# salesforce/ai-economist

Measured on AMD Instinct MI355X. Metric: agent-steps/sec, gather-trade-build 25x25 4-agent batched envs, higher is better.
Workload: dtype u8/i32 state + f64 coin/utility (f32 observations); 1 GPU; C2 BASELINE configs[1]: gather-trade-build 25x25, 4 agents + planner, Build+CDA+Gather+PeriodicBracketTax, 4096 replicas/GPU, uniform random policy, planner not counted; envs_per_gpu=4096, global_envs=4096, n_agents=4, kernel_specialisation=compile time, parallelism=single GPU

## Files before the change

ai-economist_amd/csrc/aie_capi.hip:

```cpp
#include <hip/hip_runtime.h>

#include <cstdio>
#include <cstdlib>
#include <cstring>
#include <vector>

#include "aie_kernels.hip"
#include "aie_kernels_ose.hip"
#include "aie_kernels_saez.hip"
#include "aie_kernels_ppo.hip"
#include "aie_kernels_covid.hip"
#include "aie_jit.h"

struct aie_env {
  aie_params P{};
  aie_params* d_params;
  aie_tensor_table tt;
  uint8_t* arena;
  bool owns_arena;
  size_t vmm_total, vmm_piece;
  int device;
  size_t lds;
  int spec;
  int spec_match;
  hipModule_t jit_mod;
  hipFunction_t jit_step, jit_reset;
  std::shared_ptr<aie_jit::Job> jit_job;
  int pinned_generic;
  float* rew_log;
  int32_t rew_log_slots, rew_log_epoch;
  int cv_taps_f32;
  int log_active;
  int dev_generic;
  char err[512];
};

static thread_local char g_create_err[512] = "";
static inline void aie_jit_poll(aie_env* env);
static bool aie_jit_eligible(const aie_env* env);
static int aie_jit_request(aie_env* env);

#define AIE_DEV_API __attribute__((visibility("default")))

#define AIE_HIP_CHECK(env, expr)                                                          \
  do {                                                                                    \
    hipError_t _e = (expr);                                                               \
    if (_e != hipSuccess) {                                                               \
      snprintf((env)->err, sizeof((env)->err), "%s failed: %s", #expr, hipGetErrorString(_e)); \
      return AIE_E_HIP;                                                                   \
    }                                                                                     \
  } while (0)

static uint8_t* aie_arena_alloc_pieces(int device, size_t bytes, size_t piece_mb, size_t* vmm_total, size_t* vmm_piece);
static uint8_t* aie_arena_alloc(int device, size_t bytes, size_t* vmm_total, size_t* vmm_piece) {
  const char* e_min = getenv("AIE_ARENA_VMM_MIN_MB");
  const char* e_piece = getenv("AIE_ARENA_PIECE_MB");
  const size_t min_mb = e_min ? (size_t)atol(e_min) : 1024;
  return aie_arena_alloc_pieces(device, bytes, bytes >= (min_mb << 20) ? (e_piece ? (size_t)atol(e_piece) : 64) : 0, vmm_total, vmm_piece);
}
static uint8_t* aie_arena_alloc_pieces(int device, size_t bytes, size_t piece_mb, size_t* vmm_total, size_t* vmm_piece) {
  *vmm_total = *vmm_piece = 0;
  void* p = nullptr;
  if (piece_mb > 0) {
    hipMemAllocationProp prop = {};
    prop.type = hipMemAllocationTypePinned;
    prop.location.type = hipMemLocationTypeDevice;
    prop.location.id = device;
    size_t gran = 0;
    if (hipMemGetAllocationGranularity(&gran, &prop, hipMemAllocationGranularityMinimum) == hipSuccess && gran > 0) {
      if (gran < ((size_t)2 << 20)) gran = (size_t)2 << 20;
      size_t piece = (piece_mb << 20) / gran * gran;
      if (piece < gran) piece = gran;
      const size_t total = (bytes + piece - 1) / piece * piece;
      hipDeviceptr_t va = nullptr;
      if (hipMemAddressReserve(&va, total, gran, nullptr, 0) == hipSuccess) {
        size_t off = 0;
        for (; off < total; off += piece) {
          hipMemGenericAllocationHandle_t h;
          if (hipMemCreate(&h, piece, &prop, 0) != hipSuccess) break;
          const hipError_t me = hipMemMap(static_cast<char*>(va) + off, piece, 0, h, 0);
          (void)hipMemRelease(h);
          if (me != hipSuccess) break;
        }
        hipMemAccessDesc acc = {};
        acc.location = prop.location;
        acc.flags = hipMemAccessFlagsProtReadWrite;
        if (off >= total && hipMemSetAccess(va, total, &acc, 1) == hipSuccess) {
          *vmm_total = total;
          *vmm_piece = piece;
          return static_cast<uint8_t*>(va);
        }
        for (size_t q = 0; q < off; q += piece) (void)hipMemUnmap(static_cast<char*>(va) + q, piece);
        (void)hipMemAddressFree(va, total);
      }
    }
    (void)hipGetLastError();
  }
  return hipMalloc(&p, bytes) == hipSuccess ? static_cast<uint8_t*>(p) : nullptr;
}
static void aie_arena_free(uint8_t* arena, size_t vmm_total, size_t vmm_piece) {
  if (!arena) return;
  if (vmm_total) {
    for (size_t q = 0; q < vmm_total; q += vmm_piece) (void)hipMemUnmap(arena + q, vmm_piece);
    (void)hipMemAddressFree(arena, vmm_total);
  } else {
    (void)hipFree(arena);
  }
}

__global__ void aie_init_cells_kernel(const aie_params P, uint8_t* __restrict__ arena) {
  const int64_t q = (int64_t)blockIdx.x * blockDim.x + threadIdx.x;
  if (q >= (int64_t)P.E * P.HW) return;
  const int e = (int)(q / P.HW), cell = (int)(q - (int64_t)e * P.HW);
  reinterpret_cast<uint32_t*>(arena + P.a_records + (int64_t)e * P.rec_bytes + P.o_cells)[cell] = 0x00ff0000u;
}

__global__ void aie_set_flags_kernel(const aie_params P, uint8_t* __restrict__ arena,
                                     const uint8_t* __restrict__ flags, int shared) {
  const int64_t q = (int64_t)blockIdx.x * blockDim.x + threadIdx.x;
  if (q >= (int64_t)P.E * P.HW) return;
  const int e = (int)(q / P.HW), cell = (int)(q - (int64_t)e * P.HW);
  uint32_t* w = reinterpret_cast<uint32_t*>(arena + P.a_records + (int64_t)e * P.rec_bytes + P.o_cells) + cell;
  const uint32_t fl = flags[shared ? cell : q];
  *w = (*w & 0x00ffffffu) | (fl << 24);
}

__global__ void __launch_bounds__(64) aie_src_list_kernel(const aie_params* __restrict__ params, uint8_t* __restrict__ arena) {
  const aie_params& P = *params;
  const int e = (int)blockIdx.x, lane = (int)threadIdx.x, HW = P.HW;
  if (!P.o_src_list || e >= P.E) return;
  uint8_t* rec = arena + P.a_records + (int64_t)e * P.rec_bytes;
  const uint8_t* cb = rec + P.o_cells;
  uint16_t* lst = reinterpret_cast<uint16_t*>(rec + P.o_src_list);
  for (int k = lane; k < AIE_SRC_CAP; k += 64) lst[k] = 0;
  int base = 0;
  for (int rs = 0; rs < 2; ++rs) {
    const uint32_t bit = rs == 0 ? AIE_CELL_WOOD_SRC : AIE_CELL_STONE_SRC;
    for (int q0 = 0; q0 < HW; q0 += 64) {
      const int q = q0 + lane;
      const bool on = q < HW && (cb[4 * q + 3] & bit);
      const uint64_t mask = __ballot(on);
      const int slot = base + __popcll(mask & ((1ull << lane) - 1ull));
      if (on && slot < AIE_SRC_CAP) lst[slot] = (uint16_t)(rs * HW + q);
      base += __popcll(mask);
    }
  }
  if (lane == 0) *reinterpret_cast<int32_t*>(rec + P.o_src_n) = base;
}
static int aie_rebuild_src_lists(aie_env* env) {
  if (env->P.c.scenario != AIE_SCN_GTB || !env->P.o_src_list) return AIE_OK;
  hipLaunchKernelGGL(aie_src_list_kernel, dim3((unsigned)env->P.E), dim3(64), 0, 0, env->d_params, env->arena);
  AIE_HIP_CHECK(env, hipGetLastError());
  AIE_HIP_CHECK(env, hipDeviceSynchronize());
  return AIE_OK;
}

static inline int aie_workgroups_per_cu(size_t lds) {
  const size_t granules = (lds + 1279) / 1280;
  const size_t fit = granules ? (size_t)128 / granules : 16;
  return (int)(fit < 16 ? fit : 16);
}

using aie_step_fn = void (*)(const aie_params*, uint8_t*, const int32_t*, const int32_t*, NextActions);
using aie_reset_fn = void (*)(const aie_params*, uint8_t*, const uint8_t*, int);
using aie_window_fn = void (*)(const aie_params*, uint8_t*);
template <typename Fn>
struct aie_kernel {
  Fn fn;
  const char* name;
};
#define AIE_KERNEL(...) {__VA_ARGS__, #__VA_ARGS__}
template <typename Fn>
struct aie_route {
  aie_kernel<Fn> k;
  bool module;
  unsigned block;
  size_t lds;
};

static const struct aie_spec_kernels {
  aie_kernel<aie_step_fn> step[AIE_N_SPECS], traced[AIE_N_SPECS], ose[AIE_N_SPECS];
  aie_kernel<aie_reset_fn> reset[AIE_N_SPECS];
} aie_spec_kernel = [] {
  aie_spec_kernels t{};
#define AIE_GTB_ROW(K) t.step[K] = AIE_KERNEL(aie_step_kernel_spec<K>), t.reset[K] = AIE_KERNEL(aie_reset_kernel_spec<K>);
#define AIE_OSE_ROW(K) t.ose[K] = AIE_KERNEL(aie_ose_step_kernel_spec<K>);
#define AIE_TRACED_ROW(K) t.traced[K] = AIE_KERNEL(aie_step_kernel_spec_trace<K>);
  AIE_SPEC_LIST_GTB(AIE_GTB_ROW)
  AIE_SPEC_LIST_OSE(AIE_OSE_ROW)
#ifdef AIE_DEV
  AIE_SPEC_LIST_GTB(AIE_TRACED_ROW)
#endif
  return t;
}();
#define AIE_CV_TABLE(ROW) {ROW(1), ROW(2), ROW(3), ROW(4), ROW(5), ROW(6), ROW(7), ROW(8)}
#define AIE_CV_STEP_ROW(F) {AIE_KERNEL(aie_covid_step_kernel<F, false>), AIE_KERNEL(aie_covid_step_kernel<F, true>)}
#define AIE_CV_WINDOW_ROW(F) {AIE_KERNEL(aie_covid_window_kernel<F, double>), AIE_KERNEL(aie_covid_window_kernel<F, float>)}
static const aie_kernel<aie_step_fn> aie_cv_step_kernel[AIE_COVID_MAX_FILTERS][2] = AIE_CV_TABLE(AIE_CV_STEP_ROW);
static const aie_kernel<aie_window_fn> aie_cv_window_kernel[AIE_COVID_MAX_FILTERS][2] = AIE_CV_TABLE(AIE_CV_WINDOW_ROW);

static int aie_select_step(const aie_env* env, bool full, aie_route<aie_step_fn>* out) {
  const aie_params& P = env->P;
  const int spec = env->spec;
  const bool covid = P.c.scenario == AIE_SCN_COVID, ose = P.c.scenario == AIE_SCN_ONE_STEP_ECONOMY;
  const bool jit = spec == AIE_KERNEL_INSTANCE_JIT, inst = spec >= 0 && spec < AIE_N_SPECS;
  const bool hooks = P.dev_trace != nullptr || P.dev_skip_mask != 0;
  const aie_kernel<aie_step_fn> none = {nullptr, nullptr};
  aie_kernel<aie_step_fn> k = AIE_KERNEL(aie_step_kernel_log);
  if (full) {
  } else if (covid) {
    if (P.cv_F < 1 || P.cv_F > AIE_COVID_MAX_FILTERS) return AIE_E_UNSUPPORTED;
    k = aie_cv_step_kernel[P.cv_F - 1][P.c.covid.filter_recurrence ? 1 : 0];
  } else if (ose) {
    if (jit) k = {nullptr, "aie_jit_ose_step"};
    else if (spec >= 0) k = inst ? aie_spec_kernel.ose[spec] : none;
    else k = AIE_KERNEL(aie_ose_step_kernel);
  } else if (inst && hooks && !env->dev_generic) {
    k = aie_spec_kernel.traced[spec];
  } else if (P.saez_stride || P.M > AIE_NT || P.regen_general || hooks || env->dev_generic || P.n_host_a || P.n_host_p) {
  } else if (jit) {
    k = {nullptr, "aie_jit_step"};
  } else if (spec >= 0) {
    k = inst ? aie_spec_kernel.step[spec] : none;
  } else if (aie_workgroups_per_cu(env->lds) <= 12) {
    k = AIE_KERNEL(aie_step_kernel_r6);
  } else {
    k = AIE_KERNEL(aie_step_kernel);
  }
  if (!k.name) return AIE_E_INVALID;
  *out = {k, !k.fn, (unsigned)(covid ? AIE_NT : ose ? OSE_NT : 2 * AIE_NT), env->lds};
  return AIE_OK;
}

static int aie_launch_step(aie_env* env, const aie_route<aie_step_fn>& r, unsigned grid, const int32_t* d_actions_a,
                           const int32_t* d_actions_p, const NextActions& next, hipStream_t st) {
  if (r.module) {
    const aie_params* dp = env->d_params;
    uint8_t* ar = env->arena;
    NextActions nx = next;
    void* args[] = {&dp, &ar, &d_actions_a, &d_actions_p, &nx};
    AIE_HIP_CHECK(env, hipModuleLaunchKernel(env->jit_step, grid, 1, 1, r.block, 1, 1, (unsigned)r.lds, st, args, nullptr));
  } else {
    hipLaunchKernelGGL(r.k.fn, dim3(grid), dim3(r.block), r.lds, st, env->d_params, env->arena, d_actions_a, d_actions_p, next);
  }
  return AIE_OK;
}

static unsigned aie_log_grid(const aie_env* env) {
  if (env->P.c.scenario != AIE_SCN_GTB || env->P.ev_replicas <= 0 || !env->log_active) return 0;
  const int64_t L = env->P.ev_replicas, E8 = env->P.E >> 3;
  return (env->P.E & 7) ? (unsigned)L : (L <= E8 ? (unsigned)(8 * (L - 1) + 1) : (unsigned)env->P.E);
}

static aie_route<aie_reset_fn> aie_select_reset(const aie_env* env) {
  const aie_params& P = env->P;
  if (P.c.scenario == AIE_SCN_COVID) return {AIE_KERNEL(aie_covid_reset_kernel), false, AIE_NT, 0};
  if (P.c.scenario == AIE_SCN_ONE_STEP_ECONOMY) return {{nullptr, "aie_ose_reset_kernel"}, false, OSE_NT, env->lds};
  const bool layout = P.c.layout_gen != AIE_LAYOUT_FIXED;
  aie_route<aie_reset_fn> r = {AIE_KERNEL(aie_reset_kernel), false, AIE_NT, env->lds + aie::layout_gen_lds_bytes(P)};
  if (layout) r.k = AIE_KERNEL(aie_reset_kernel_layout), r.block = LG_NW * AIE_NT;
  if (P.dev_skip_mask == 0 && !env->dev_generic) {
    if (env->spec == AIE_KERNEL_INSTANCE_JIT) r.k = {nullptr, "aie_jit_reset"}, r.module = true;
    else if (env->spec >= 0 && env->spec < AIE_N_SPECS && aie_spec_kernel.reset[env->spec].fn) r.k = aie_spec_kernel.reset[env->spec];
  }
  return r;
}

static void aie_launch_reset(aie_env* env, const uint8_t* d_mask, int keep_rewards, void* stream) {
  const aie_route<aie_reset_fn> r = aie_select_reset(env);
  const dim3 g((unsigned)env->P.E), b(r.block);
  hipStream_t st = static_cast<hipStream_t>(stream);
  if (r.module) {
    const aie_params* dp = env->d_params;
    uint8_t* ar = env->arena;
    void* args[] = {&dp, &ar, &d_mask, &keep_rewards};
    (void)hipModuleLaunchKernel(env->jit_reset, g.x, 1, 1, b.x, 1, 1, (unsigned)r.lds, st, args, nullptr);
  } else if (!r.k.fn) {
    hipLaunchKernelGGL(aie_ose_reset_kernel, g, b, r.lds, st, env->d_params, env->arena, d_mask);
  } else {
    hipLaunchKernelGGL(r.k.fn, g, b, r.lds, st, env->d_params, env->arena, d_mask, keep_rewards);
  }
  if (env->P.c.scenario == AIE_SCN_GTB && aie__layout_staged(&env->P.c)) {
    const int threshold = env->P.E >= 4 ? (int)(env->P.E / 4) : 1;
    hipLaunchKernelGGL(aie_layout_decide_kernel, dim3(1), dim3(1), 0, st, env->d_params, env->arena, threshold);
    hipLaunchKernelGGL(aie_layout_refill_kernel, g, dim3(LG_NW * AIE_NT), r.lds, st, env->d_params, env->arena);
  }
}

template <bool LOGP>
using aie_policy_fn = void (*)(const aie_sampler_args, uint8_t*, const float*, const float*, uint64_t, int64_t, int32_t*, int32_t*,
                               int, const SamplerLogp<LOGP>);
template <bool LOGP>
static aie_policy_fn<LOGP> aie_policy_sampler(const aie_sampler_args& S) {
  if (S.ragged || S.agents.len > 64 || S.planner.len > 64) return aie_sample_policy_actions_kernel<LOGP>;
  static const aie_policy_fn<LOGP> fast[3][3] = {
      {aie_sample_policy_fast_kernel<4, 4, LOGP>, aie_sample_policy_fast_kernel<4, 5, LOGP>, aie_sample_policy_fast_kernel<4, 6, LOGP>},
      {aie_sample_policy_fast_kernel<5, 4, LOGP>, aie_sample_policy_fast_kernel<5, 5, LOGP>, aie_sample_policy_fast_kernel<5, 6, LOGP>},
      {aie_sample_policy_fast_kernel<6, 4, LOGP>, aie_sample_policy_fast_kernel<6, 5, LOGP>, aie_sample_policy_fast_kernel<6, 6, LOGP>}};
  return fast[S.agents.lsh - 4][S.planner.lsh - 4];
}

template <bool LOGP>
static int aie_sample_policy_launch(aie_env* env, const float* d_logits_a, const float* d_logits_p, uint64_t seed,
                                    int64_t global_env_offset, int32_t* d_actions_a, int32_t* d_actions_p, float* d_logp_a,
                                    float* d_logp_p, void* stream) {
  if (!env) return AIE_E_INVALID;
  if ((d_actions_a && !d_logits_a) || (d_actions_p && !d_logits_p)) {
    snprintf(env->err, sizeof(env->err), "aie_sample_policy_actions: an action buffer without its logits");
    return AIE_E_INVALID;
  }
  if (LOGP && ((d_actions_a && d_logits_a && !d_logp_a) || (d_actions_p && d_logits_p && !d_logp_p))) {
    snprintf(env->err, sizeof(env->err), "aie_sample_policy_actions_logp: an action buffer without its log-probability buffer");
    return AIE_E_INVALID;
  }
  if (aie_sampler_check(&env->P, env->err, sizeof(env->err)) != AIE_OK) return AIE_E_UNSUPPORTED;
  AIE_HIP_CHECK(env, hipSetDevice(env->device));
  static const int wpr_log2 = [] {
    const char* v = getenv("AIE_SAMPLER_WAVES_LOG2");
    const int k = v ? atoi(v) : 1;
    int r = k < 0 ? 0 : (k > 2 ? 2 : k);
#ifdef AIE_DEV
    if (const char* sk = getenv("AIE_SAMPLER_DEV_SKIP")) r |= atoi(sk) << 8;
#endif
    return r;
  }();
  const int rpb = 4 >> (wpr_log2 & 255);
  const aie_sampler_args S = aie_sampler_args_of(&env->P, env->d_params);
  SamplerLogp<LOGP> LP;
  if constexpr (LOGP) LP.a = d_logp_a, LP.p = d_logp_p;
  hipLaunchKernelGGL(aie_policy_sampler<LOGP>(S), dim3((unsigned)((env->P.E + rpb - 1) / rpb)), dim3(256), 0,
                     static_cast<hipStream_t>(stream), S, env->arena, d_logits_a, d_logits_p, seed, global_env_offset, d_actions_a,
                     d_actions_p, wpr_log2, LP);
  AIE_HIP_CHECK(env, hipGetLastError());
  return AIE_OK;
}

extern "C" {

int aie_sizeof_config(void) { return (int)sizeof(aie_config); }

int aie_arena_info(const aie_env* env, int64_t* bytes, int32_t* allocator, int64_t* piece_bytes) {
  if (!env) return AIE_E_INVALID;
  if (bytes) *bytes = env->P.arena_bytes;
  if (allocator) *allocator = !env->owns_arena ? AIE_ARENA_CALLER : env->vmm_total ? AIE_ARENA_VMM : AIE_ARENA_HIPMALLOC;
  if (piece_bytes) *piece_bytes = (int64_t)env->vmm_piece;
  return AIE_OK;
}

int64_t aie_arena_bytes(const aie_config* cfg) {
  aie_params P;
  int rc = aie_build_params(cfg, &P, nullptr, g_create_err, sizeof(g_create_err));
  if (rc != AIE_OK) return rc;
  return P.arena_bytes;
}

int aie_create(const aie_config* cfg, int device, void* arena, int64_t arena_bytes, aie_env** out) {
  if (!cfg || !out) {
    snprintf(g_create_err, sizeof(g_create_err), "null argument");
    return AIE_E_INVALID;
  }
  aie_env* env = new aie_env();
  int rc = aie_build_params(cfg, &env->P, &env->tt, g_create_err, sizeof(g_create_err));
  if (rc != AIE_OK) { delete env; return rc; }
  env->device = device;
  env->spec = -1;
  env->log_active = 1;
  env->cv_taps_f32 = 1;
  if (cfg->scenario != AIE_SCN_COVID) {
    std::vector<aie_params> norm(1, env->P);
    aie_spec_normalize(&norm[0]);
    for (int k = 0; k < AIE_N_SPECS; ++k)
      if (memcmp(&norm[0], aie_spec_table[k], sizeof(aie_params)) == 0) env->spec = k;
  }
  env->spec_match = env->spec;
  const bool covid = cfg->scenario == AIE_SCN_COVID;
  const bool ose = cfg->scenario == AIE_SCN_ONE_STEP_ECONOMY || covid;
  env->lds = covid ? 0 : cfg->scenario == AIE_SCN_ONE_STEP_ECONOMY ? aie::ose_lds_bytes(env->P) : aie::lds_bytes(env->P);
  if (env->lds + (covid ? 0 : aie::layout_gen_lds_bytes(env->P)) > 160 * 1024) {
    snprintf(g_create_err, sizeof(g_create_err),
             "per-replica working set (%zu B of LDS) exceeds 160 KiB: reduce max_num_orders / world size", env->lds);
    delete env;
    return AIE_E_UNSUPPORTED;
  }
  hipError_t he = hipSetDevice(device);
  if (he != hipSuccess) {
    snprintf(g_create_err, sizeof(g_create_err), "hipSetDevice(%d): %s", device, hipGetErrorString(he));
    delete env;
    return AIE_E_HIP;
  }
  if (arena) {
    if (arena_bytes < env->P.arena_bytes || (reinterpret_cast<uintptr_t>(arena) & 255u)) {
      snprintf(g_create_err, sizeof(g_create_err), "arena too small (%lld < %lld) or not 256-byte aligned",
               (long long)arena_bytes, (long long)env->P.arena_bytes);
      delete env;
      return AIE_E_INVALID;
    }
    env->arena = static_cast<uint8_t*>(arena);
    env->owns_arena = false;
  } else {
    env->arena = aie_arena_alloc(device, (size_t)env->P.arena_bytes, &env->vmm_total, &env->vmm_piece);
    if (!env->arena) {
      snprintf(g_create_err, sizeof(g_create_err), "arena allocation of %lld bytes failed", (long long)env->P.arena_bytes);
      delete env;
      return AIE_E_NOMEM;
    }
    env->owns_arena = true;
  }
  he = hipMemset(env->arena, 0, (size_t)env->P.arena_bytes);
  if (he == hipSuccess && !ose) {
    const int64_t tot = (int64_t)env->P.E * env->P.HW;
    hipLaunchKernelGGL(aie_init_cells_kernel, dim3((unsigned)((tot + 255) / 256)), dim3(256), 0, 0, env->P, env->arena);
    he = hipDeviceSynchronize();
  }
  if (he == hipSuccess && env->P.saez_stride) {
    std::vector<double> rows((size_t)env->P.E * 2, 0.5);
    he = hipMemcpy2D(env->arena + env->P.a_saez + AIE_SAEZ_OFF_ELAS, (size_t)env->P.saez_stride, rows.data(), 16, 16,
                     (size_t)env->P.E, hipMemcpyHostToDevice);
  }
  if (he != hipSuccess) {
    snprintf(g_create_err, sizeof(g_create_err), "arena init: %s", hipGetErrorString(he));
    if (env->owns_arena) aie_arena_free(env->arena, env->vmm_total, env->vmm_piece);
    delete env;
    return AIE_E_HIP;
  }
  he = hipMalloc(reinterpret_cast<void**>(&env->d_params), sizeof(aie_params));
  if (he == hipSuccess) he = hipMemcpy(env->d_params, &env->P, sizeof(aie_params), hipMemcpyHostToDevice);
  if (he != hipSuccess) {
    snprintf(g_create_err, sizeof(g_create_err), "parameter block: %s", hipGetErrorString(he));
    if (env->owns_arena) aie_arena_free(env->arena, env->vmm_total, env->vmm_piece);
    delete env;
    return AIE_E_HIP;
  }
  for (int i = 0; i < env->tt.n; ++i) env->tt.t[i].data = env->arena + env->tt.t[i].arena_offset;
  const char* auto_jit = getenv("AIE_JIT_AUTO");
  if (env->spec < 0 && aie_jit_eligible(env) && !(auto_jit && auto_jit[0] == '0')) (void)aie_jit_request(env);
  *out = env;
  return AIE_OK;
}

int aie_destroy(aie_env* env) {
  if (!env) return AIE_OK;
  (void)hipSetDevice(env->device);
  (void)hipDeviceSynchronize();
  if (env->owns_arena && env->arena) aie_arena_free(env->arena, env->vmm_total, env->vmm_piece);
  if (env->d_params) (void)hipFree(env->d_params);
  if (env->jit_mod) (void)hipModuleUnload(env->jit_mod);
  delete env;
  return AIE_OK;
}

const char* aie_last_error(const aie_env* env) { return env ? env->err : g_create_err; }

int aie_num_tensors(const aie_env* env) { return env ? env->tt.n : AIE_E_INVALID; }

int aie_tensor_at(const aie_env* env, int index, aie_tensor_desc* out) {
  if (!env || !out || index < 0 || index >= env->tt.n) return AIE_E_INVALID;
  *out = env->tt.t[index];
  return AIE_OK;
}

static const aie_tensor_desc* find_tensor(const aie_env* env, const char* name) {
  for (int i = 0; i < env->tt.n; ++i)
    if (strcmp(env->tt.t[i].name, name) == 0) return &env->tt.t[i];
  return nullptr;
}

int aie_get_tensor(const aie_env* env, const char* name, aie_tensor_desc* out) {
  if (!env || !name || !out) return AIE_E_INVALID;
  const aie_tensor_desc* d = find_tensor(env, name);
  if (!d) {
    snprintf(const_cast<aie_env*>(env)->err, sizeof(env->err), "no tensor named '%s'", name);
    return AIE_E_NOTFOUND;
  }
  *out = *d;
  return AIE_OK;
}

static int copy_tensor(aie_env* env, const char* name, void* host, int64_t bytes, bool upload) {
  if (!env || !name || !host) return AIE_E_INVALID;
  const aie_tensor_desc* d = find_tensor(env, name);
  if (!d) {
    snprintf(env->err, sizeof(env->err), "no tensor named '%s'", name);
    return AIE_E_NOTFOUND;
  }
  const int es = aie__dtype_size(d->dtype);
  int64_t count = 1, span = es;
  for (int i = 0; i < d->ndim; ++i) {
    count *= d->shape[i];
    span += (d->shape[i] - 1) * d->stride[i];
  }
  if (bytes != count * es) {
    snprintf(env->err, sizeof(env->err), "'%s': expected %lld bytes, got %lld", name, (long long)(count * es),
             (long long)bytes);
    return AIE_E_INVALID;
  }
  AIE_HIP_CHECK(env, hipSetDevice(env->device));
  std::vector<uint8_t> tmp((size_t)span);
  uint8_t* dev = env->arena + d->arena_offset;
  AIE_HIP_CHECK(env, hipDeviceSynchronize());
  AIE_HIP_CHECK(env, hipMemcpy(tmp.data(), dev, (size_t)span, hipMemcpyDeviceToHost));
  int64_t idx[6] = {0, 0, 0, 0, 0, 0};
  uint8_t* h = static_cast<uint8_t*>(host);
  for (int64_t k = 0; k < count; ++k) {
    int64_t off = 0;
    for (int i = 0; i < d->ndim; ++i) off += idx[i] * d->stride[i];
    if (upload) memcpy(tmp.data() + off, h + k * es, (size_t)es);
    else memcpy(h + k * es, tmp.data() + off, (size_t)es);
    for (int i = d->ndim - 1; i >= 0; --i) {
      if (++idx[i] < d->shape[i]) break;
      idx[i] = 0;
    }
  }
  if (upload) AIE_HIP_CHECK(env, hipMemcpy(dev, tmp.data(), (size_t)span, hipMemcpyHostToDevice));
  return AIE_OK;
}

int aie_upload(aie_env* env, const char* name, const void* host, int64_t bytes) {
  const int rc = copy_tensor(env, name, const_cast<void*>(host), bytes, true);
  if (rc == AIE_OK && env->P.o_obs_valid && strcmp(name, "obs_valid") != 0) {
    const aie_tensor_desc* d = find_tensor(env, name);
    const int64_t r0 = env->P.a_records, r1 = r0 + (int64_t)env->P.E * env->P.rec_bytes;
    if (d->arena_offset >= r0 && d->arena_offset < r1)
      AIE_HIP_CHECK(env, hipMemset2DAsync(env->arena + r0 + env->P.o_obs_valid, (size_t)env->P.rec_bytes, 0, 4,
                                          (size_t)env->P.E, nullptr));
  }
  if (rc == AIE_OK && (strcmp(name, "cells") == 0 || strcmp(name, "cell_flags") == 0))
    return aie_rebuild_src_lists(env);
  if (rc == AIE_OK && env->P.c.scenario == AIE_SCN_COVID && strcmp(name, "model_unemp_conv_filters") == 0) {
    const double* taps = static_cast<const double*>(host);
    env->cv_taps_f32 = 1;
    for (int64_t q = 0; q < bytes / 8; ++q)
      if ((double)(float)taps[q] != taps[q]) env->cv_taps_f32 = 0;
  }
  if (rc == AIE_OK && env->P.c.scenario == AIE_SCN_COVID &&
      (strcmp(name, "model_stringency_level_history_0") == 0 || strcmp(name, "model_unemp_conv_filters") == 0)) {
    hipLaunchKernelGGL(aie_covid_prepare_kernel, dim3(1), dim3(AIE_NT), 0, 0, env->d_params, env->arena);
    AIE_HIP_CHECK(env, hipGetLastError());
    AIE_HIP_CHECK(env, hipDeviceSynchronize());
  }
  return rc;
}
int aie_download(aie_env* env, const char* name, void* host, int64_t bytes) {
  return copy_tensor(env, name, host, bytes, false);
}

int aie_set_layout(aie_env* env, const uint8_t* stone_src, const uint8_t* wood_src, const uint8_t* water) {
  if (!env) return AIE_E_INVALID;
  if (env->P.c.scenario != AIE_SCN_GTB) return AIE_OK;
  if (!stone_src || !wood_src) return AIE_E_INVALID;
  const aie_params& P = env->P;
  const int shared = P.c.shared_layout ? 1 : 0;
  const int64_t cnt = (shared ? 1 : (int64_t)P.E) * P.HW;
  std::vector<uint8_t> fl((size_t)cnt);
  for (int64_t q = 0; q < cnt; ++q)
    fl[(size_t)q] = (uint8_t)(((water && water[q]) ? AIE_CELL_WATER : 0u) | (stone_src[q] ? AIE_CELL_STONE_SRC : 0u) |
                              (wood_src[q] ? AIE_CELL_WOOD_SRC : 0u));
  AIE_HIP_CHECK(env, hipSetDevice(env->device));
  uint8_t* dfl = nullptr;
  AIE_HIP_CHECK(env, hipMalloc(reinterpret_cast<void**>(&dfl), (size_t)cnt));
  AIE_HIP_CHECK(env, hipMemcpy(dfl, fl.data(), (size_t)cnt, hipMemcpyHostToDevice));
  const int64_t tot = (int64_t)P.E * P.HW;
  hipLaunchKernelGGL(aie_set_flags_kernel, dim3((unsigned)((tot + 255) / 256)), dim3(256), 0, 0, P, env->arena, dfl, shared);
  AIE_HIP_CHECK(env, hipGetLastError());
  AIE_HIP_CHECK(env, hipDeviceSynchronize());
  AIE_HIP_CHECK(env, hipFree(dfl));
  if (const int rc = aie_rebuild_src_lists(env)) return rc;
  if (aie__shared_src_list(&P.c)) {
    struct { int32_t count, pad[3]; uint16_t d[AIE_SRC_CAP]; } lst;
    memset(&lst, 0, sizeof(lst));
    for (int r = 0; r < 2; ++r) {
      const uint8_t* plane = r == 0 ? wood_src : stone_src;
      for (int cell = 0; cell < P.HW; ++cell)
        if (plane[cell]) {
          if (lst.count < AIE_SRC_CAP) lst.d[lst.count] = (uint16_t)(r * P.HW + cell);
          lst.count += 1;
        }
    }
    AIE_HIP_CHECK(env, hipMemcpy(env->arena + P.a_src_list, &lst, sizeof(lst), hipMemcpyHostToDevice));
  }
  return AIE_OK;
}

static int aie_seed_impl(aie_env* env, uint64_t base_seed, void* stream) {
  if (env->P.c.scenario == AIE_SCN_COVID) return AIE_OK;
  AIE_HIP_CHECK(env, hipSetDevice(env->device));
  hipLaunchKernelGGL(aie_seed_kernel, dim3((unsigned)((env->P.E + 63) / 64)), dim3(64), 0,
                     static_cast<hipStream_t>(stream), env->P, env->arena, base_seed);
  AIE_HIP_CHECK(env, hipGetLastError());
// ... 439 lines not shown
               "stats, with values also values_old, returns and grad_values (and no grad_values without), and clip > 0 (%g)",
               c ? "planner's" : "agents'", (double)k->clip);
      return AIE_E_INVALID;
    }
  }
  aie_policy_eval_args E;
  const int rc = aie_policy_eval_args_of(env, "aie_ppo_loss", B, agents ? agents->logits : nullptr, planner ? planner->logits : nullptr,
                                         agents ? agents->masks : nullptr, planner ? planner->masks : nullptr, &E);
  if (rc != AIE_OK) return rc;
  if (!E.items) return AIE_OK;
  aie_ppo_args A;
  memset(&A, 0, sizeof(A));
  const aie_policy_eval_group* eg[2] = {&E.agents, &E.planner};
  aie_ppo_group* pg[2] = {&A.agents, &A.planner};
  const int width[2] = {env->P.act_a_width, env->P.act_p_width};
  for (int c = 0; c < 2; ++c) {
    const aie_ppo_class* k = cls[c];
    if (!k) continue;
    const aie_policy_eval_group& e = *eg[c];
    aie_ppo_group& G = *pg[c];
    G.lg = k->logits;
    G.val = k->values;
    G.mk = k->masks;
    G.act = k->actions;
    G.lp_old = k->logp_old;
    G.adv = k->adv;
    G.val_old = k->values_old;
    G.ret = k->returns;
    G.mom = k->adv_moments;
    G.grad = k->grad_logits;
    G.grad_v = k->grad_values;
    G.stats = k->stats;
    G.lg_bstride = e.lg_bstride;
    G.len = e.len;
    G.lrs = e.lrs;
    G.lsh = e.lsh;
    G.rows = e.rows;
    G.w = width[c] > 0 ? width[c] : 1;
    G.actors = e.rows / G.w;
    if (G.w > 64 || G.actors * G.w != e.rows) {
      snprintf(env->err, sizeof(env->err), "aie_ppo_loss: %d action slots per actor (%d rows) are more than a wavefront holds", G.w, e.rows);
      return AIE_E_UNSUPPORTED;
    }
    G.generic = e.generic || G.w > 1;
    const int rpw = G.generic ? 1 : 64 >> e.lsh;
    G.items = G.generic ? G.actors : (e.rows + rpw - 1) / rpw;
    G.clip = k->clip;
    G.vf_clip = k->vf_clip;
    G.vf_coef = k->vf_coef;
    G.ent_coef = k->ent_coef;
    G.scale = aie_ppo_scale(B * (int64_t)G.actors);
    G.g_H = -aie_ppo_product(G.scale, k->ent_coef);
    G.kv = aie_ppo_product(G.scale, k->vf_coef);
  }
  A.params = env->d_params;
  A.index = d_index;
  A.ws = static_cast<double*>(d_workspace);
  A.B = (uint32_t)B;
  A.items = (uint32_t)(A.agents.items + A.planner.items);
  A.act_a_width = E.act_a_width;
  A.ragged = E.ragged;
  const int64_t work = B * (int64_t)A.items;
  if (work > 0x7fffff00ll) {
    snprintf(env->err, sizeof(env->err), "aie_ppo_loss: B = %lld is more than one call takes (%u work items per batch element)",
             (long long)B, A.items);
    return AIE_E_INVALID;
  }
  AIE_HIP_CHECK(env, hipSetDevice(env->device));
  A.waves = aie_ppo_waves(work, AIE_PPO_MAX_WAVES);
  const int64_t need = (int64_t)A.waves * AIE_PPO_RECORD * (int64_t)sizeof(double);
  if (!d_workspace || (reinterpret_cast<uintptr_t>(d_workspace) & 7u) || workspace_bytes < need) {
    snprintf(env->err, sizeof(env->err), "aie_ppo_loss: the workspace (%p, %lld bytes) must be device memory, 8-byte aligned, of at "
             "least %lld bytes (aie_ppo_workspace_bytes)", d_workspace, (long long)workspace_bytes, (long long)need);
    return AIE_E_INVALID;
  }
  hipLaunchKernelGGL(aie_ppo_loss_kernel, dim3((A.waves + 3u) / 4u), dim3(256), 0, static_cast<hipStream_t>(stream), A);
  hipLaunchKernelGGL(aie_ppo_reduce_kernel, dim3(1), dim3(1024), 0, static_cast<hipStream_t>(stream), A);
  AIE_HIP_CHECK(env, hipGetLastError());
  return AIE_OK;
}

int aie_trajectory_store(aie_env* env, const aie_traj_segment* segs, int32_t n_segs, int32_t n_slots, int32_t* d_slot, void* stream) {
  if (!env) return AIE_E_INVALID;
  static_assert(AIE_TRAJ_SEGMENTS == AIE_TRAJ_MAX_SEGMENTS, "aie_layout.h and aie.h disagree on the segment count");
  if (!segs || n_segs < 1 || n_segs > AIE_TRAJ_MAX_SEGMENTS || n_slots < 1 || !d_slot) {
    snprintf(env->err, sizeof(env->err), "aie_trajectory_store: %d segments (1 .. %d), %d slots (>= 1), segments and slot counters "
             "not NULL", n_segs, AIE_TRAJ_MAX_SEGMENTS, n_slots);
    return AIE_E_INVALID;
  }
  aie_traj_args A;
  memset(&A, 0, sizeof(A));
  for (int g = 0; g < n_segs; ++g) {
    const aie_traj_segment& s = segs[g];
    const uintptr_t sp = reinterpret_cast<uintptr_t>(s.src), dp = reinterpret_cast<uintptr_t>(s.dst);
    const int64_t count = s.bytes / 4;
    if (!s.src || !s.dst || s.bytes < 4 || (s.bytes & 3) || (s.src_stride & 3) || (sp & 3) || (dp & 3) || s.rows < 0 ||
        s.rows > 32767 || (s.rows > 1 && count % s.rows)) {
      snprintf(env->err, sizeof(env->err), "aie_trajectory_store: segment %d (%d bytes per replica, source stride %lld, rows %d): "
               "pointers not NULL and 4-byte aligned, sizes and strides multiples of 4, rows dividing the element count", g,
               s.bytes, (long long)s.src_stride, s.rows);
      return AIE_E_INVALID;
    }
    aie_traj_seg_k& k = A.seg[g];
    k.src = static_cast<const uint8_t*>(s.src);
    k.dst = static_cast<uint8_t*>(s.dst);
    k.src_stride = s.src_stride;
    k.bytes = s.bytes;
    k.rows = (int16_t)s.rows;
    k.wide = (int16_t)(s.rows <= 1 && !((sp | dp | (uintptr_t)s.src_stride | (uintptr_t)s.bytes) & 15));
  }
  A.slot = d_slot;
  A.n_segs = n_segs;
  A.n_slots = n_slots;
  A.E = env->P.E;
  AIE_HIP_CHECK(env, hipSetDevice(env->device));
  hipLaunchKernelGGL(aie_trajectory_store_kernel, dim3((unsigned)env->P.E), dim3(256), 0, static_cast<hipStream_t>(stream), A);
  AIE_HIP_CHECK(env, hipGetLastError());
  return AIE_OK;
}

int aie_step_kernel_instance(aie_env* env) { return env ? env->spec : -2; }

static bool aie_jit_eligible(const aie_env* env) {
  const aie_params& P = env->P;
  const bool ose = P.c.scenario == AIE_SCN_ONE_STEP_ECONOMY;
  return !(P.c.scenario == AIE_SCN_COVID || P.saez_stride || P.n_host_a || P.n_host_p || (!ose && (P.M > AIE_NT || P.regen_general)));
}
static int aie_jit_request(aie_env* env) {
  if (env->jit_job && env->jit_job->pid == (long)getpid()) return AIE_OK;
  env->jit_job.reset();
  hipDeviceProp_t prop;
  AIE_HIP_CHECK(env, hipGetDeviceProperties(&prop, env->device));
  std::string arch = prop.gcnArchName;
  arch = arch.substr(0, arch.find(':'));
  std::vector<aie_params> norm(1, env->P);
  aie_spec_normalize(&norm[0]);
  const bool ose = env->P.c.scenario == AIE_SCN_ONE_STEP_ECONOMY;
  const int wg = aie_workgroups_per_cu(env->lds);
  const int waves = ose ? (wg >= 16 ? 4 : wg >= 12 ? 3 : 2) : ((2 * wg + 3) / 4 < 8 ? (2 * wg + 3) / 4 : 8);
  env->jit_job = aie_jit::start_job(&norm[0], sizeof(aie_params), waves, arch.c_str(), ose);
  return AIE_OK;
}
static bool aie_jit_load(aie_env* env, const std::string& code, bool ose) {
  hipModule_t mod = nullptr;
  hipFunction_t fs = nullptr, fr = nullptr;
  if (hipModuleLoadData(&mod, code.data()) != hipSuccess ||
      hipModuleGetFunction(&fs, mod, ose ? "aie_jit_ose_step" : "aie_jit_step") != hipSuccess ||
      (!ose && hipModuleGetFunction(&fr, mod, "aie_jit_reset") != hipSuccess)) {
    if (mod) (void)hipModuleUnload(mod);
    (void)hipGetLastError();
    return false;
  }
  env->jit_mod = mod;
  env->jit_step = fs;
  env->jit_reset = fr;
  return true;
}
static int aie_jit_adopt(aie_env* env, bool wait) {
  if (!env->jit_job) return env->spec_match == AIE_KERNEL_INSTANCE_JIT ? AIE_OK : AIE_E_UNSUPPORTED;
  std::shared_ptr<aie_jit::Job> job = env->jit_job;
  if (wait) aie_jit::run_job_now_if_queued(job);
  int st = job->state.load(std::memory_order_acquire);
  while (wait && st == 0) {
    usleep(2000);
    st = job->state.load(std::memory_order_acquire);
  }
  if (st == 0) return AIE_E_UNSUPPORTED;
  env->jit_job.reset();
  if (st < 0) {
    snprintf(env->err, sizeof(env->err), "aie_specialize: %s", job->err.c_str());
    return AIE_E_UNSUPPORTED;
  }
  (void)hipSetDevice(env->device);
  bool ok = aie_jit_load(env, job->code, job->ose);
  if (!ok) {
    std::string code, err;
    if (aie_jit::code_object(job->image.data(), job->image.size(), job->waves, job->arch.c_str(), job->ose, code, err, nullptr,
                             true))
      ok = aie_jit_load(env, code, job->ose);
  }
  if (!ok) {
    snprintf(env->err, sizeof(env->err), "aie_specialize: the compiled code object could not be loaded");
    return AIE_E_UNSUPPORTED;
  }
  env->spec_match = AIE_KERNEL_INSTANCE_JIT;
  if (!env->pinned_generic) env->spec = AIE_KERNEL_INSTANCE_JIT;
  return AIE_OK;
}
static inline void aie_jit_poll(aie_env* env) {
  if (env->jit_job && env->jit_job->pid != (long)getpid()) env->jit_job.reset();
  if (env->jit_job && env->jit_job->state.load(std::memory_order_acquire) != 0) (void)aie_jit_adopt(env, false);
}

int aie_select_step_kernel(aie_env* env, int which) {
  if (!env) return AIE_E_INVALID;
  if (which != AIE_KERNEL_AUTO && which != AIE_KERNEL_GENERIC) {
    snprintf(env->err, sizeof(env->err), "aie_select_step_kernel: unknown kernel %d", which);
    return AIE_E_INVALID;
  }
  env->pinned_generic = which == AIE_KERNEL_GENERIC;
  env->spec = which == AIE_KERNEL_GENERIC ? -1 : env->spec_match;
  return AIE_OK;
}

int aie_specialize(aie_env* env) {
  if (!env) return AIE_E_INVALID;
  if (env->spec_match >= 0 && !(getenv("AIE_JIT_FORCE") && env->spec_match != AIE_KERNEL_INSTANCE_JIT)) {
    if (!env->pinned_generic) env->spec = env->spec_match;
    return AIE_OK;
  }
  if (!aie_jit_eligible(env)) {
    snprintf(env->err, sizeof(env->err), "aie_specialize: this configuration runs the full-featured step kernel (tax_model "
             "\"saez\", order books beyond a wavefront, general regeneration) or is the COVID scenario");
    return AIE_E_UNSUPPORTED;
  }
  AIE_HIP_CHECK(env, hipSetDevice(env->device));
  const int rc = aie_jit_request(env);
  if (rc != AIE_OK) return rc;
  return aie_jit_adopt(env, true);
}

#ifdef AIE_DEV

__global__ void aie_test_glibc_math_kernel(int fn, const double* __restrict__ x, const double* __restrict__ y,
                                           double* __restrict__ out, int64_t n) {
  const int64_t i = (int64_t)blockIdx.x * blockDim.x + threadIdx.x;
  if (i >= n) return;
  double r;
  switch (fn) {
    case 0: r = aie_pow_glibc(x[i], y[i]); break;
    case 1: r = aie_exp_glibc(x[i]); break;
    case 2: r = aie_log_glibc(x[i]); break;
    case 3: r = (double)aie::cv_powf((float)x[i], (float)y[i]); break;
    case 4: r = aie::cv_exp(x[i]); break;
    default: r = aie::cv_log(x[i]); break;
  }
  out[i] = r;
}
AIE_DEV_API int aie_test_glibc_math(int fn, const void* d_x, const void* d_y, void* d_out, int64_t n, void* stream) {
  if (n <= 0 || !d_x || !d_out || ((fn == 0 || fn == 3) && !d_y) || fn < 0 || fn > 5) return AIE_E_INVALID;
  hipLaunchKernelGGL(aie_test_glibc_math_kernel, dim3((unsigned)((n + 255) / 256)), dim3(256), 0,
                     static_cast<hipStream_t>(stream), fn, static_cast<const double*>(d_x),
                     static_cast<const double*>(d_y), static_cast<double*>(d_out), n);
  return hipGetLastError() == hipSuccess ? AIE_OK : AIE_E_HIP;
}

AIE_DEV_API int aie_dev_lds_bytes(aie_env* env, int64_t* out) {
  if (!env || !out) return AIE_E_INVALID;
  out[0] = (int64_t)env->lds;
  out[5] = aie_workgroups_per_cu(env->lds);
  out[1] = env->P.o_mt;
  out[2] = env->P.HW;
  out[3] = env->P.c.scenario == AIE_SCN_ONE_STEP_ECONOMY || env->P.c.scenario == AIE_SCN_COVID ? 0 : (int64_t)aie::fscr_doubles(env->P) * 8;
  out[4] = env->P.c.scenario == AIE_SCN_ONE_STEP_ECONOMY || env->P.c.scenario == AIE_SCN_COVID ? 0 : (int64_t)aie::stage_bytes(env->P);
  return AIE_OK;
}

static int aie_dev_push_params(aie_env* env) {
  AIE_HIP_CHECK(env, hipSetDevice(env->device));
  AIE_HIP_CHECK(env, hipDeviceSynchronize());
  AIE_HIP_CHECK(env, hipMemcpy(env->d_params, &env->P, sizeof(aie_params), hipMemcpyHostToDevice));
  return AIE_OK;
}

AIE_DEV_API int aie_dev_set_trace(aie_env* env, void* d_buf) {
  if (!env) return AIE_E_INVALID;
  env->P.dev_trace = static_cast<uint64_t*>(d_buf);
  return aie_dev_push_params(env);
}

AIE_DEV_API int aie_dev_set_lds_pad(aie_env* env, int bytes) {
  if (!env || bytes < 0) return AIE_E_INVALID;
  env->lds += (size_t)bytes;
  return AIE_OK;
}

AIE_DEV_API int aie_dev_set_draw_window(aie_env* env, int words) {
  if (!env || words < 0) return AIE_E_INVALID;
  env->P.dev_draw_window = words;
  env->dev_generic = words ? 1 : 0;
  return aie_dev_push_params(env);
}

AIE_DEV_API int aie_dev_set_skip_mask(aie_env* env, int mask) {
  if (!env) return AIE_E_INVALID;
  env->P.dev_skip_mask = mask;
  return aie_dev_push_params(env);
}
AIE_DEV_API int aie_dev_step_route(aie_env* env, char* buf, int n) {
  if (!env || !buf || n < 1) return AIE_E_INVALID;
  const aie_params& P = env->P;
  const int lo = aie_log_grid(env) ? P.ev_replicas : 0;
  std::string s = P.saez_stride ? "aie_saez_kernel + " : "";
  aie_route<aie_step_fn> r;
  int rc = AIE_OK;
  if (lo && (rc = aie_select_step(env, true, &r)) == AIE_OK)
    s += std::string(r.k.name) + "[0," + std::to_string(lo) + ")x" + std::to_string(aie_log_grid(env)) + (lo < P.E ? " + " : "");
  if (rc == AIE_OK && lo < P.E && (rc = aie_select_step(env, false, &r)) == AIE_OK) {
    s += r.k.name + (lo ? "[" + std::to_string(lo) + "," + std::to_string(P.E) + ")" : std::string());
    if (P.c.scenario == AIE_SCN_COVID && !P.c.covid.filter_recurrence)
      s += std::string(" + ") + aie_cv_window_kernel[P.cv_F - 1][env->cv_taps_f32 ? 1 : 0].name;
  }
  if (rc != AIE_OK) s = "error " + std::to_string(rc);
  snprintf(buf, (size_t)n, "%s | %s", s.c_str(), aie_select_reset(env).k.name);
  return AIE_OK;
}
#endif

}
```

ai-economist_amd/csrc/aie_kernels.hip:

```cpp
#pragma once
#include <hip/hip_runtime.h>
#include <stdint.h>

#include "aie_layout.h"
#include "aie_glibc_math.h"

#pragma clang fp contract(off)

#ifdef AIE_JIT
#include "aie_jit_image.h"
#else
#include "aie_spec_generated.h"
#endif
template <int SPEC>
__device__ __forceinline__ const aie_params& aie_spec_params(const aie_params* run_time) {
  if constexpr (SPEC < 0) return *run_time;
  else return *reinterpret_cast<const aie_params*>(aie_spec_image<SPEC>::bytes);
}

#define AIE_NT 64
#define AIE_DIRTY_CAP 64

namespace aie {

// ... 1601 lines not shown
      const int a_idx = 64 * J + lane;
      const int q = done + (a_idx - pos);
      const uint32_t t = mt_word(m, m.r[J]);
      uint32_t tn = lane_get(t, (lane + 1) & 63);
      if (J < 9) tn = (lane == 63) ? mt_word(m, bcast(m.r[J + 1], 0)) : tn;
      const bool first = a_idx >= pos && a_idx < AIE_MT_N - 1 && (q & 1) == 0 && q < total;
      if (first) regen_cell(c, t, tn, q >> 1);
    }
    const int avail = AIE_MT_N - pos;
    const int take = (total - done) < avail ? (total - done) : avail;
    if (take == avail) {
      const int q623 = done + (AIE_MT_N - 1 - pos);
      if ((q623 & 1) == 0 && q623 < total) {
        carry = true;
        carry_t = mt_word(m, bcast(m.r[9], 47));
        carry_d = q623 >> 1;
      }
    }
    done += take;
    m.pos = pos + take;
    if (done >= total) break;
  }
}

__device__ __forceinline__ uint32_t mt_window_word(const MT& m, int idx) {
  const int row = idx >> 6, ln = idx & 63;
  uint32_t v = 0;
#pragma unroll
  for (int r = 0; r < 10; ++r) {
    const uint32_t t = lane_get(m.r[r], ln);
    v = (row == r) ? t : v;
  }
  return v;
}
struct SrcList {
  int S;
  int d[AIE_SRC_CAP / AIE_NT];
};
__device__ __forceinline__ SrcList src_list_from_record(const Ctx& c, const uint8_t* __restrict__ arena) {
  SrcList L;
  const uint8_t* g = arena + (int64_t)c.e * c.P.rec_bytes;
  L.S = uni(*reinterpret_cast<const int32_t*>(g + c.P.o_src_n));
  const uint16_t* lst = reinterpret_cast<const uint16_t*>(g + c.P.o_src_list);
#pragma unroll
  for (int k = 0; k < AIE_SRC_CAP / AIE_NT; ++k) L.d[k] = (int)lst[k * AIE_NT + c.tid];
  return L;
}
__device__ __forceinline__ SrcList src_list_from_arena(const Ctx& c, const uint8_t* __restrict__ arena) {
  SrcList L;
  const uint8_t* g = arena + c.R.a_src_list;
  L.S = uni(*reinterpret_cast<const int32_t*>(g));
  const uint16_t* lst = reinterpret_cast<const uint16_t*>(g + 16);
#pragma unroll
  for (int k = 0; k < AIE_SRC_CAP / AIE_NT; ++k) L.d[k] = (int)lst[k * AIE_NT + c.tid];
  return L;
}
__device__ __forceinline__ void scenario_step_regen(const Ctx& c, MT& m, const SrcList& src) {
  if (c.full && c.snap) {
    const int HW = c.P.HW, stride = (HW + 15) / 16 * 16;
    const uint8_t* cb = reinterpret_cast<const uint8_t*>(R_CELLS(c));
    for (int q = c.tid; q < HW; q += AIE_NT) {
      const uint32_t fl = cb[4 * q + 3];
      const uint8_t s0 = cb[4 * q], s1 = cb[4 * q + 1];
      c.snap[q] = (fl & AIE_CELL_STONE_SRC) ? (s0 > 1 ? s0 : 1) : s0;
      c.snap[stride + q] = (fl & AIE_CELL_WOOD_SRC) ? (s1 > 1 ? s1 : 1) : s1;
    }
    AIE_WSYNC();
  }
  const int S = src.S;
  if (S > AIE_SRC_CAP) {
    if (m.fast && m.pos < AIE_MT_N) mt_fast_rows(m, c.tid);
    scenario_step_regen_rows(c, m);
    return;
  }
  const int lane = c.tid;
  const int total = 4 * c.P.HW;
  const int pos0 = m.pos;
  const int nchunk = (S + AIE_NT - 1) / AIE_NT;
  if (m.fast) {
    const int odd = pos0 & 1;
#pragma unroll
    for (int k = 0; k < AIE_SRC_CAP / AIE_NT; ++k) {
      if (k >= nchunk) continue;
      const int j = k * AIE_NT + lane;
      const int d = j < S ? src.d[k] : 0;
      const int h = (pos0 >> 1) + d;
      uint32_t a0, a1, b0 = 0, b1 = 0;
      fast_pair(m.fkey, m.fblk, m.fsalt, h, a0, a1);
      if (odd) fast_pair(m.fkey, m.fblk, m.fsalt, h + 1, b0, b1);
      if (j < S) regen_cell(c, odd ? a1 : a0, odd ? b0 : a1, d);
    }
    const int last_win = (pos0 + total - 1) / AIE_MT_N;
    m.pos = pos0 + total - last_win * AIE_MT_N;
    m.fblk += (uint32_t)last_win;
    AIE_WSYNC();
    return;
  }
  int off_a[AIE_SRC_CAP / AIE_NT];
  uint32_t wa[AIE_SRC_CAP / AIE_NT], wb[AIE_SRC_CAP / AIE_NT];
#pragma unroll
  for (int k = 0; k < AIE_SRC_CAP / AIE_NT; ++k) {
    const int j = k * AIE_NT + lane;
    off_a[k] = (k < nchunk && j < S) ? pos0 + 2 * src.d[k] : -16;
    wa[k] = wb[k] = 0;
  }
  const int last_win = (pos0 + total - 1) / AIE_MT_N;
  for (int w = 0; w <= last_win; ++w) {
    if (w > 0) mt_twist_body(m, lane);
    const int lo = w * AIE_MT_N;
    if (c.mtwin) {
#pragma unroll
      for (int j = 0; j < 10; ++j) c.mtwin[64 * j + lane] = m.r[j];
#pragma unroll
      for (int k = 0; k < AIE_SRC_CAP / AIE_NT; ++k) {
        if (k >= nchunk) continue;
        const int ia = off_a[k] - lo;
        const bool ha = (unsigned)ia < (unsigned)AIE_MT_N, hb = (unsigned)(ia + 1) < (unsigned)AIE_MT_N;
        if (__ballot(ha || hb) == 0) continue;
        const int at = ia < 0 ? 0 : (ia > AIE_MT_N - 1 ? AIE_MT_N - 1 : ia);
        const uint32_t x0 = c.mtwin[at], x1 = c.mtwin[at + 1];
        if (ha) wa[k] = x0;
        if (hb) wb[k] = ia < 0 ? x0 : x1;
      }
      continue;
    }
#pragma unroll
    for (int k = 0; k < AIE_SRC_CAP / AIE_NT; ++k) {
      if (k >= nchunk) continue;
      const int ia = off_a[k] - lo, ib = ia + 1;
      const bool ha = ia >= 0 && ia < AIE_MT_N, hb = off_a[k] >= 0 && ib >= 0 && ib < AIE_MT_N;
      if (__ballot(ha || hb) == 0) continue;
      const uint32_t va = mt_window_word(m, ha ? ia : 0), vb = mt_window_word(m, hb ? ib : 0);
      if (ha) wa[k] = va;
      if (hb) wb[k] = vb;
    }
  }
  m.pos = pos0 + total - last_win * AIE_MT_N;
#pragma unroll
  for (int k = 0; k < AIE_SRC_CAP / AIE_NT; ++k)
    if (k < nchunk && off_a[k] >= 0) regen_cell(c, mt_temper(wa[k]), mt_temper(wb[k]), (off_a[k] - pos0) >> 1);
  AIE_WSYNC();
}

__device__ __forceinline__ double energy_weight(const Ctx& c) {
  if (!c.P.sh_energy_warmup) return 1.0;
  const int v = c.P.c.energy_warmup_method == AIE_WARMUP_DECAY ? *R_I32(c, o_completions) : *R_I32(c, o_auto_warmup);
  return 1.0 - aie_exp_glibc(-(double)v / c.R.c.energy_warmup_constant);
}

__device__ __forceinline__ void current_metrics(const Ctx& c) {
  const int n = c.P.n, i = c.tid;
  double* coin = scr_coin(c);
  double* out = scr_part(c);
  double* tmp = scr_gini_sort(c);
  const double lcf = energy_weight(c) * c.R.c.energy_cost;
  const double eta = c.R.c.isoelastic_eta;
  if (i < n) {
    const double ci = R_F64(c, o_inv_coin)[i] + R_F64(c, o_esc_coin)[i];
    coin[i] = ci;
    double util_c;
    if (c.P.sh_eta_is_one) util_c = aie_log_glibc(ci > 1 ? ci : 1);
    else util_c = (aie_pow_glibc(ci, 1 - eta) - 1) / (1 - eta);
    out[i] = util_c - R_F64(c, o_labor)[i] * lcf;
  }
  AIE_WSYNC();
  const int prt = c.P.c.planner_reward_type;
  if (prt == AIE_PLANNER_REW_COIN_EQ_TIMES_PROD) {
    double gini;
    const double tot = np_sum_small(coin, n);
    if (n < 30) {
      const double diff = np_sum_seq<3>(coin, n, 1, 65536u / (uint32_t)n + 1u, 0, n * n, i);
      const double unscaled = diff / (2 * n * tot + 1e-10);
      gini = unscaled / ((double)(n - 1) / (double)n);
    } else {
      double* s = scr_gini_sort(c);
      if (i == 0) {
        for (int j = 0; j < n; ++j) s[j] = coin[j];
        for (int a = 1; a < n; ++a) {
          double x = s[a]; int b = a - 1;
          while (b >= 0 && s[b] > x) { s[b + 1] = s[b]; --b; }
          s[b + 1] = x;
        }
        const double tots = np_sum_small(s, n) + 1e-10;
        double run = 0;
        for (int j = 0; j < n; ++j) { run += s[j]; s[j] = run / tots; }
      }
      AIE_WSYNC();
      gini = 1 - (2.0 / (n + 1)) * np_sum_small(s, n);
    }
    if (i == 0) {
      const double ew = 1 - c.R.c.mixing_weight_gini_vs_coin;
      out[n] = (ew * (1 - gini) + (1 - ew)) * (tot / n);
    }
  } else {
    if (i < n) tmp[i] = 1 / (coin[i] > 1 ? coin[i] : 1);
    AIE_WSYNC();
    const double sw = np_sum_small(tmp, n);
    AIE_WSYNC();
    if (i < n) tmp[i] = (prt == AIE_PLANNER_REW_INV_INCOME_COIN ? coin[i] : out[i]) * (tmp[i] / sw);
    AIE_WSYNC();
    if (i == 0) out[n] = np_sum_small(tmp, n);
  }
}

__device__ __forceinline__ void compute_rewards(const Ctx& c, uint8_t* __restrict__ arena, float* rew_log = nullptr) {
  const int n = c.P.n, i = c.tid;
  current_metrics(c);
  AIE_WSYNC();
  double* cur = scr_part(c);
  double* util = R_F64(c, o_util);
  double* rew = scr_coin(c);
  if (i <= n) {
    const double r = cur[i] - util[i];
    util[i] = cur[i];
    rew[i] = r;
    if (i < n) reinterpret_cast<float*>(arena + c.R.a_rew_a)[(int64_t)c.e * n + i] = (float)r;
    else reinterpret_cast<float*>(arena + c.R.a_rew_p)[c.e] = (float)r;
    if (rew_log) rew_log[(int64_t)c.e * (n + 2) + i] = (float)r;
  }
  AIE_WSYNC();
  if (i == 0) {
    if (np_sum_small(rew, n) / n > 0) *R_I32(c, o_auto_warmup) += 1;
  }
}

template <bool WATER>
__device__ __forceinline__ void cell_channels(uint32_t w, float* ch) {
  const uint32_t fl = w >> 24;
  ch[0] = (float)AIE_CELL_STONE(w);
  ch[1] = (float)AIE_CELL_WOOD(w);
  ch[2] = (((w >> 16) & 0xffu) != 0xffu) ? 1.0f : 0.0f;
  int k = 3;
  if (WATER) ch[k++] = (fl & AIE_CELL_WATER) ? 1.0f : 0.0f;
  ch[k++] = (fl & AIE_CELL_STONE_SRC) ? 1.0f : 0.0f;
  ch[k++] = (fl & AIE_CELL_WOOD_SRC) ? 1.0f : 0.0f;
}

struct SpatialOut {
  BufRsrc amap, aidx, pmap, pidx;
};
template <bool WATER>
__device__ __forceinline__ SpatialOut spatial_out(const Ctx& c, uint8_t* __restrict__ arena) {
  constexpr int CM = WATER ? 6 : 5;
  const int n = c.P.n, HW = c.P.HW, WV2 = c.P.WV * c.P.WV;
  (void)WV2;
  const int plane = c.P.am_h * c.P.am_w;
  const uint32_t amap_bytes = (uint32_t)(n * c.P.am_ch * plane * 4), aidx_bytes = (uint32_t)(n * 2 * plane * 2);
  SpatialOut o;
  o.amap = make_rsrc(arena + c.R.a_obs_a_map + (int64_t)c.e * amap_bytes, amap_bytes);
  o.aidx = make_rsrc(arena + c.R.a_obs_a_idx + (int64_t)c.e * aidx_bytes, aidx_bytes);
  const bool pl = c.P.c.planner_gets_spatial_info != 0;
  o.pmap = make_rsrc(arena + c.R.a_obs_p_map + (int64_t)c.e * CM * HW * 4, pl ? (uint32_t)(CM * HW * 4) : 0u);
  o.pidx = make_rsrc(arena + c.R.a_obs_p_idx + (int64_t)c.e * 2 * HW * 2, pl ? (uint32_t)(2 * HW * 2) : 0u);
  return o;
}

template <bool WATER>
__device__ __forceinline__ void crop_item(const Ctx& c, const SpatialOut& o, int i, int d, int r, int col) {
  constexpr int CM = WATER ? 6 : 5;
  const int H = c.P.H, W = c.P.W, WV2 = c.P.WV * c.P.WV;
  const int so = i * (CM + 1) * WV2 * 4, si = i * 2 * WV2 * 2;
  const bool in = (r >= 0) & (r < H) & (col >= 0) & (col < W);
  const int cell = in ? r * W + col : 0;
  const uint32_t cw = in ? R_CELLS(c)[cell] : 0x00ff0000u;
  float ch[6];
  cell_channels<WATER>(cw, ch);
#pragma unroll
  for (int k = 0; k < CM; ++k) buf_store_f32(o.amap, ch[k], 4 * d, so + k * WV2 * 4);
  buf_store_f32(o.amap, in ? 1.0f : 0.0f, 4 * d, so + CM * WV2 * 4);
  const int own = AIE_CELL_OWNER(cw);
  int v0 = own >= 0 ? own + 2 : 0;
  int v1 = in ? (int)c.locmap[cell] : 0;
  v1 = v1 ? v1 + 1 : 0;
  if (v0 == i + 2) v0 = 1;
  if (v1 == i + 2) v1 = 1;
  buf_store_i16(o.aidx, v0, 2 * d, si);
  buf_store_i16(o.aidx, v1, 2 * d, si + WV2 * 2);
}
template <bool WATER>
__device__ __forceinline__ void crop_agent(const Ctx& c, const SpatialOut& o, int i) {
  const int WV = c.P.WV, WV2 = WV * WV, w = c.P.c.obs_range;
  const int r0 = R_I32(c, o_loc_r)[i] - w, c0 = R_I32(c, o_loc_c)[i] - w;
  for (int d = c.tid; d < WV2; d += AIE_NT) {
    const int dr = udiv(d, WV, c.P.mg_WV), dc = d - dr * WV;
    crop_item<WATER>(c, o, i, d, r0 + dr, c0 + dc);
  }
}
template <bool WATER>
__device__ __forceinline__ void planner_cell(const Ctx& c, const SpatialOut& o, int cell) {
  constexpr int CM = WATER ? 6 : 5;
  const int HW = c.P.HW;
  float ch[6];
  const uint32_t cw = R_CELLS(c)[cell];
  cell_channels<WATER>(cw, ch);
#pragma unroll
  for (int k = 0; k < CM; ++k) buf_store_f32(o.pmap, ch[k], 4 * cell, k * HW * 4);
  const int own = AIE_CELL_OWNER(cw);
  const int occ = c.locmap[cell];
  buf_store_i16(o.pidx, own >= 0 ? own + 2 : 0, 2 * cell, 0);
  buf_store_i16(o.pidx, occ ? occ + 1 : 0, 2 * cell, HW * 2);
}

template <bool WATER>
__device__ __forceinline__ void write_spatial_observations_t(const Ctx& c, uint8_t* __restrict__ arena) {
  constexpr int CM = WATER ? 6 : 5;
  const int n = c.P.n, HW = c.P.HW;
  const uint32_t* cells = R_CELLS(c);
  const SpatialOut o = spatial_out<WATER>(c, arena);
  if (c.P.c.full_observability) {
    const uint32_t* lm4f = reinterpret_cast<const uint32_t*>(c.locmap);
    for (int i = 0; i < n; ++i) {
      const int so = i * CM * HW * 4, si = i * 2 * HW * 2;
      for (int q = c.tid; q < (HW >> 2); q += AIE_NT) {
        const uint4 cw = reinterpret_cast<const uint4*>(cells)[q];
        const uint32_t cws[4] = {cw.x, cw.y, cw.z, cw.w};
        float ch[4][6];
#pragma unroll
        for (int u = 0; u < 4; ++u) cell_channels<WATER>(cws[u], ch[u]);
#pragma unroll
        for (int k = 0; k < CM; ++k) buf_store_f32x4(o.amap, ch[0][k], ch[1][k], ch[2][k], ch[3][k], 16 * q, so + k * HW * 4);
        const uint32_t occ4 = lm4f[q];
#pragma unroll
        for (int u = 0; u < 4; ++u) {
          const int own = AIE_CELL_OWNER(cws[u]);
          int v0 = own >= 0 ? own + 2 : 0;
          const int occ = (int)((occ4 >> (8 * u)) & 0xffu);
          int v1 = occ ? occ + 1 : 0;
          if (v0 == i + 2) v0 = 1;
          if (v1 == i + 2) v1 = 1;
          buf_store_i16(o.aidx, v0, 8 * q + 2 * u, si);
          buf_store_i16(o.aidx, v1, 8 * q + 2 * u, si + HW * 2);
        }
      }
      for (int cell = 4 * (HW >> 2) + c.tid; cell < HW; cell += AIE_NT) {
        float ch[6];
        const uint32_t cw = cells[cell];
        cell_channels<WATER>(cw, ch);
#pragma unroll
        for (int k = 0; k < CM; ++k) buf_store_f32(o.amap, ch[k], 4 * cell, so + k * HW * 4);
        const int own = AIE_CELL_OWNER(cw);
        int v0 = own >= 0 ? own + 2 : 0;
        const int occ = c.locmap[cell];
        int v1 = occ ? occ + 1 : 0;
        if (v0 == i + 2) v0 = 1;
        if (v1 == i + 2) v1 = 1;
        buf_store_i16(o.aidx, v0, 2 * cell, si);
        buf_store_i16(o.aidx, v1, 2 * cell, si + HW * 2);
      }
    }
  } else {
    for (int i = 0; i < n; ++i) crop_agent<WATER>(c, o, i);
  }
  if (c.P.c.planner_gets_spatial_info) {
    const int nq4 = HW >> 2;
    const uint32_t* lm4 = reinterpret_cast<const uint32_t*>(c.locmap);
    for (int q = c.tid; q < nq4; q += AIE_NT) {
      const uint4 cw = reinterpret_cast<const uint4*>(cells)[q];
      const uint32_t cws[4] = {cw.x, cw.y, cw.z, cw.w};
      float ch[4][6];
#pragma unroll
      for (int u = 0; u < 4; ++u) cell_channels<WATER>(cws[u], ch[u]);
#pragma unroll
      for (int k = 0; k < CM; ++k) buf_store_f32x4(o.pmap, ch[0][k], ch[1][k], ch[2][k], ch[3][k], 16 * q, k * HW * 4);
      const uint32_t occ4 = lm4[q];
      uint32_t ow[2], oc[2];
#pragma unroll
      for (int u = 0; u < 4; ++u) {
        const int own = AIE_CELL_OWNER(cws[u]);
        const uint32_t vo = (uint32_t)(own >= 0 ? own + 2 : 0);
        const uint32_t occ = (occ4 >> (8 * u)) & 0xffu;
        const uint32_t vc = occ ? occ + 1 : 0;
        if (u & 1) { ow[u >> 1] |= vo << 16; oc[u >> 1] |= vc << 16; }
        else { ow[u >> 1] = vo; oc[u >> 1] = vc; }
      }
      buf_store_u32x2(o.pidx, ow[0], ow[1], 8 * q, 0);
      if ((HW & 1) == 0) {
        buf_store_u32x2(o.pidx, oc[0], oc[1], 8 * q, HW * 2);
      } else {
#pragma unroll
        for (int u = 0; u < 4; ++u) buf_store_i16(o.pidx, (int)((oc[u >> 1] >> (16 * (u & 1))) & 0xffffu), 8 * q + 2 * u, HW * 2);
      }
    }
    for (int cell = 4 * nq4 + c.tid; cell < HW; cell += AIE_NT) planner_cell<WATER>(c, o, cell);
  }
}

template <bool WATER>
__device__ __forceinline__ void agent_full_cell(const Ctx& c, const SpatialOut& o, int i, int cell) {
  constexpr int CM = WATER ? 6 : 5;
  const int HW = c.P.HW;
  const int so = i * CM * HW * 4, si = i * 2 * HW * 2;
  float ch[6];
  const uint32_t cw = R_CELLS(c)[cell];
  cell_channels<WATER>(cw, ch);
#pragma unroll
  for (int k = 0; k < CM; ++k) buf_store_f32(o.amap, ch[k], 4 * cell, so + k * HW * 4);
  const int own = AIE_CELL_OWNER(cw);
  int v0 = own >= 0 ? own + 2 : 0;
  const int occ = c.locmap[cell];
  int v1 = occ ? occ + 1 : 0;
  if (v0 == i + 2) v0 = 1;
  if (v1 == i + 2) v1 = 1;
  buf_store_i16(o.aidx, v0, 2 * cell, si);
  buf_store_i16(o.aidx, v1, 2 * cell, si + HW * 2);
}

template <bool WATER>
__device__ __forceinline__ void update_spatial_observations_t(const Ctx& c, uint8_t* __restrict__ arena) {
  const int n = c.P.n, W = c.P.W, WV = c.P.WV, w = c.P.c.obs_range;
  const int cnt = uni(c.dirty[0]);
  if (cnt > AIE_DIRTY_CAP) {
    write_spatial_observations_t<WATER>(c, arena);
    return;
  }
  const SpatialOut o = spatial_out<WATER>(c, arena);
  const uint32_t mv0 = (uint32_t)uni(c.dirty[1]), mv1 = (uint32_t)uni(c.dirty[2]);
  const uint16_t* dl = dirty_list(c);
  const int cell = c.tid < cnt ? (int)dl[c.tid] : -1;
  const int r = cell >= 0 ? udiv(cell, W, c.P.mg_W) : 0, col = cell - r * W;
  for (int i = 0; i < n; ++i) {
    if (c.P.c.full_observability) {
      if (cell >= 0) agent_full_cell<WATER>(c, o, i, cell);
      continue;
    }
    const bool moved = ((i < 32 ? mv0 >> i : mv1 >> (i - 32)) & 1u) != 0;
    if (moved) {
      crop_agent<WATER>(c, o, i);
    } else if (cell >= 0) {
      const int dr = r - (R_I32(c, o_loc_r)[i] - w), dc = col - (R_I32(c, o_loc_c)[i] - w);
      if (dr >= 0 && dr < WV && dc >= 0 && dc < WV) crop_item<WATER>(c, o, i, dr * WV + dc, r, col);
    }
  }
  if (c.P.c.planner_gets_spatial_info && cell >= 0) planner_cell<WATER>(c, o, cell);
}
__device__ __forceinline__ void write_spatial_observations(const Ctx& c, uint8_t* __restrict__ arena) {
  if (c.P.c.has_water) write_spatial_observations_t<true>(c, arena);
  else write_spatial_observations_t<false>(c, arena);
}
__device__ __forceinline__ void update_spatial_observations(const Ctx& c, uint8_t* __restrict__ arena) {
  if (c.P.c.has_water) update_spatial_observations_t<true>(c, arena);
  else update_spatial_observations_t<false>(c, arena);
}

__device__ __forceinline__ void flat_a(const BufRsrc& aflat, int idx, float v) { buf_store_f32(aflat, v, 4 * idx, 0); }

__device__ __forceinline__ float flat_time_value(const Ctx& c) {
  const int t = *R_I32(c, o_timestep);
  return (float)((double)t / (c.P.c.allow_observation_scaling ? (double)c.R.c.episode_length : 1.0));
}

struct AgentScalars {
  double coin; int inv0, inv1, lr, lc;
  __device__ __forceinline__ AgentScalars(const Ctx& c, int i)
      : coin(R_F64(c, o_inv_coin)[i]), inv0(R_I32(c, o_inv_res)[i]), inv1(R_I32(c, o_inv_res)[c.P.n + i]),
        lr(R_I32(c, o_loc_r)[i]), lc(R_I32(c, o_loc_c)[i]) {}
  __device__ __forceinline__ void write(const Ctx& c, uint8_t* __restrict__ arena, const BufRsrc& aflat, float* q, int i,
                                        float tval, double isc) const {
    const aie_params& P = c.P;
    const int f0 = i * P.FA;
    flat_a(aflat, f0 + P.fa_time, tval);
    const float w0 = (float)(coin * isc);
    const float w1 = (float)((double)inv0 * isc);
    const float w2 = (float)((double)inv1 * isc);
    const float w3 = (float)((double)lc / (double)P.W);
    const float w4 = (float)((double)lr / (double)P.H);
    flat_a(aflat, f0 + P.fa_world + 0, w0); flat_a(aflat, f0 + P.fa_world + 1, w1); flat_a(aflat, f0 + P.fa_world + 2, w2);
    if (!P.c.full_observability) {
      flat_a(aflat, f0 + P.fa_world + 3, w3); flat_a(aflat, f0 + P.fa_world + 4, w4);
      q[P.fpa_world + 0] = w0; q[P.fpa_world + 1] = w1; q[P.fpa_world + 2] = w2;
      if (P.c.planner_gets_spatial_info) { q[P.fpa_world + 3] = w3; q[P.fpa_world + 4] = w4; }
    }
    reinterpret_cast<float*>(arena + c.R.a_obs_a_time)[(int64_t)c.e * P.n + i] = tval;
  }
  __device__ __forceinline__ void write_marginal_rate(const Ctx& c, const BufRsrc& aflat, float* q, int i) const {
    const double cmr = tax_marginal_rate(c, (coin + R_F64(c, o_esc_coin)[i]) - R_F64(c, o_tax_last_coin)[i]);
    flat_a(aflat, i * c.P.FA + c.P.fa_tax + AIE_FA_TAX_MARGINAL_RATE(c.P.NB, c.P.n), (float)cmr);
    q[c.P.fpa_tax + AIE_FPA_TAX_CURR_MARGINAL_RATE] = (float)cmr;
  }
};
template <class Row>
__device__ __forceinline__ double price_history_column(const Ctx& c, int r, int k, Row row) {
  double s = 0;
  for (int i = 0; i < c.P.n; ++i) {
    const int at = (r * c.P.n + i) * c.P.P + k;
    const double v = R_F64(c, o_cda_price_history)[at];
    s = (i == 0) ? v : s + v;
    row(at);
  }
  return s;
}
__device__ __forceinline__ float cda_market_rate(const Ctx& c, int r, double& tot) {
  const double* a = scr_net_ph(c) + r * c.P.P;
  double dot = 0;
  for (int k = 0; k < c.P.P; ++k) dot += (double)k * a[k];
  tot = np_sum_small(a, c.P.P);
  return (float)(dot / (tot > 0.001 ? tot : 0.001));
}
struct TaxCalendar { float is_tax_day, is_first_day, tax_phase; };
__device__ __forceinline__ TaxCalendar tax_calendar(const Ctx& c) {
  const int pos = *R_I32(c, o_tax_cycle_pos);
  return {pos >= c.R.c.tax_period ? 1.0f : 0.0f, pos == 1 ? 1.0f : 0.0f, (float)((double)pos / (double)c.R.c.tax_period)};
}

__device__ __forceinline__ void write_flat_observations(const Ctx& c, uint8_t* __restrict__ arena) {
  const aie_params& P = c.P;
  const int n = P.n, tid = c.tid, Pp = P.P, NB = P.NB;
  const double isc = P.c.allow_observation_scaling ? 0.01 : 1.0;
  float* s_pag = c.stage + stage_window_words(P);
  float* s_pflat = s_pag + pad4(n * P.FPA);
  const BufRsrc aflat = make_rsrc(arena + c.R.a_obs_a_flat + (int64_t)c.e * n * P.FA * 4, (uint32_t)(n * P.FA * 4));
  auto AF = [&](int idx, float v) { flat_a(aflat, idx, v); };
  const float tval = flat_time_value(c);

  const int skip = c.skipm;
  if (P.has_cda && !(skip & AIE_DEV_SKIP_FLAT_STAGE_A)) {
    double* net_ph = scr_net_ph(c);
    for (int q = tid; q < 2 * Pp; q += AIE_NT) {
      const int r = q >= Pp ? 1 : 0, k = q - r * Pp;
      int fa = 0, fb = 0;
      const double s = price_history_column(
          c, r, k, [&](int at) { fa += R_U8(c, o_cda_ask_hist)[at], fb += R_U8(c, o_cda_bid_hist)[at]; });
      net_ph[q] = s;
      float* g = s_pflat + P.fp_cda;
      g[AIE_FP_CDA_FULL_ASKS(Pp) + q] = (float)fa;
      g[AIE_FP_CDA_FULL_BIDS(Pp) + q] = (float)fb;
      g[AIE_FP_CDA_PRICE_HISTORY(Pp) + q] = (float)(s * isc);
    }
  }
  if (tid < n && !(skip & AIE_DEV_SKIP_FLAT_STAGE_A)) {
    const int i = tid;
    const int f0 = i * P.FA;
    const AgentScalars a(c, i);
    if (P.has_build) {
      AF(f0 + P.fa_build + 0, (float)(R_F64(c, o_build_payment)[i] / (double)c.R.c.build_payment));
      AF(f0 + P.fa_build + 1, (float)R_F64(c, o_build_skill)[i]);
    }
    if (P.has_gather) AF(f0 + P.fa_gather, (float)R_F64(c, o_bonus_gather_prob)[i]);
    float* q = s_pag + i * P.FPA;
    a.write(c, arena, aflat, q, i, tval, isc);
    if (P.has_tax) {
      const double per = (double)c.R.c.tax_period;
      const double x = R_F64(c, o_tax_last_income)[i] / per;
      double* xs = scr_cmr(c);
      xs[i] = x;
      AIE_WSYNC();
      int rank = 0;
      for (int j = 0; j < n; ++j) {
        const double y = xs[j];
        rank += (y < x || (y == x && j < i)) ? 1 : 0;
      }
      scr_sorted_inc(c)[rank] = x;
      a.write_marginal_rate(c, aflat, q, i);
      q[P.fpa_tax + AIE_FPA_TAX_LAST_INCOME] = (float)x;
      q[P.fpa_tax + AIE_FPA_TAX_LAST_MARGINAL_RATE] = (float)R_F64(c, o_tax_last_marginal_rate)[i];
    }
  }
  if (tid == 0) {
    s_pflat[P.fp_time] = tval;
    s_pflat[P.fp_world + 0] = 0.0f;
    s_pflat[P.fp_world + 1] = 0.0f;
    s_pflat[P.fp_world + 2] = 0.0f;
    reinterpret_cast<float*>(arena + c.R.a_obs_p_time)[c.e] = tval;
  }
  AIE_WSYNC();

  if (P.has_cda && !(skip & AIE_DEV_SKIP_FLAT_CDA)) {
    if (tid < 2) {
      const int r = tid;
      double tot;
      const float mr = cda_market_rate(c, r, tot);
      s_pflat[P.fp_cda + AIE_FP_CDA_MARKET_RATE(Pp) + r] = mr;
      for (int i = 0; i < n; ++i) AF(i * P.FA + P.fa_cda + AIE_FA_CDA_MARKET_RATE(Pp) + r, mr);
    }
    const float* g = s_pflat + P.fp_cda;
    for (int it = tid; it < n * 2 * Pp; it += AIE_NT) {
      const int i = udiv(it, 2 * Pp, P.mg_2P);
      const int q = it - i * 2 * Pp;
      const int r = q >= Pp ? 1 : 0, k = q - r * Pp;
      const float mya = (float)R_U8(c, o_cda_ask_hist)[(r * n + i) * Pp + k];
      const float myb = (float)R_U8(c, o_cda_bid_hist)[(r * n + i) * Pp + k];
      const int fc = i * P.FA + P.fa_cda;
      AF(fc + AIE_FA_CDA_AVAILABLE_ASKS(Pp) + q, g[AIE_FP_CDA_FULL_ASKS(Pp) + q] - mya);
      AF(fc + AIE_FA_CDA_AVAILABLE_BIDS(Pp) + q, g[AIE_FP_CDA_FULL_BIDS(Pp) + q] - myb);
      AF(fc + AIE_FA_CDA_MY_ASKS(Pp) + q, mya);
      AF(fc + AIE_FA_CDA_MY_BIDS(Pp) + q, myb);
      AF(fc + AIE_FA_CDA_PRICE_HISTORY(Pp) + q, g[AIE_FP_CDA_PRICE_HISTORY(Pp) + q]);
    }
  }
  if (P.has_tax && !(skip & AIE_DEV_SKIP_FLAT_TAX)) {
    const TaxCalendar cal = tax_calendar(c);
    const int fragA = AIE_FA_TAX_LEN(NB, n);
    for (int q = tid; q < (n + 1) * fragA; q += AIE_NT) {
      const int i = udiv(q, fragA, P.mg_taxA);
      const int j = q - i * fragA;
      const bool planner = i == n;
      if (j == AIE_FA_TAX_MARGINAL_RATE(NB, n)) {
        if (planner) s_pflat[P.fp_tax + AIE_FP_TAX_PHASE(NB, n)] = cal.tax_phase;
        continue;
      }
      if (planner && j == AIE_FA_TAX_PHASE(NB, n)) continue;
      float v;
      if (j < AIE_F_TAX_IS_FIRST_DAY(NB)) v = (float)tax_rate_obs(c, j - AIE_F_TAX_CURR_RATES);
      else if (j == AIE_F_TAX_IS_FIRST_DAY(NB)) v = cal.is_first_day;
      else if (j == AIE_F_TAX_IS_TAX_DAY(NB)) v = cal.is_tax_day;
      else if (j < AIE_FA_TAX_MARGINAL_RATE(NB, n)) v = (float)scr_sorted_inc(c)[j - AIE_F_TAX_LAST_INCOMES(NB)];
      else v = cal.tax_phase;
      if (planner) s_pflat[P.fp_tax + j] = v;
      else AF(i * P.FA + P.fa_tax + j, v);
    }
  }

  AIE_WSYNC();

  if (!(skip & AIE_DEV_SKIP_PLANNER_COPY_OUT)) {
    stream_out(s_pag, reinterpret_cast<float*>(arena + c.R.a_obs_p_agents) + (int64_t)c.e * n * P.FPA, n * P.FPA, tid);
    stream_out(s_pflat, reinterpret_cast<float*>(arena + c.R.a_obs_p_flat) + (int64_t)c.e * P.FP, P.FP, tid);
  }
}

__device__ __forceinline__ void update_flat_observations(const Ctx& c, uint8_t* __restrict__ arena, uint64_t hist_dirty) {
  const aie_params& P = c.P;
  const int n = P.n, tid = c.tid, Pp = P.P, NB = P.NB;
  const double isc = P.c.allow_observation_scaling ? 0.01 : 1.0;
  const BufRsrc aflat = make_rsrc(arena + c.R.a_obs_a_flat + (int64_t)c.e * n * P.FA * 4, (uint32_t)(n * P.FA * 4));
  auto AF = [&](int idx, float v) { flat_a(aflat, idx, v); };
  float* const pflat = reinterpret_cast<float*>(arena + c.R.a_obs_p_flat) + (int64_t)c.e * P.FP;
  float* const pag = reinterpret_cast<float*>(arena + c.R.a_obs_p_agents) + (int64_t)c.e * n * P.FPA;
  const float tval = flat_time_value(c);
  const int skip = c.skipm;
  if (P.has_cda && !(skip & AIE_DEV_SKIP_FLAT_STAGE_A)) {
    double* net_ph = scr_net_ph(c);
    for (int q = tid; q < 2 * Pp; q += AIE_NT) {
      const int r = q >= Pp ? 1 : 0, k = q - r * Pp;
      const double s = price_history_column(c, r, k, [](int) {});
      net_ph[q] = s;
      if (s != 0 && !(skip & AIE_DEV_SKIP_FLAT_CDA)) {
        const float v = (float)(s * isc);
        pflat[P.fp_cda + AIE_FP_CDA_PRICE_HISTORY(Pp) + q] = v;
        for (int i = 0; i < n; ++i) AF(i * P.FA + P.fa_cda + AIE_FA_CDA_PRICE_HISTORY(Pp) + q, v);
      }
#pragma unroll
      for (int side = 0; side < 2; ++side) {
        if (!hist_col_dirty(P, hist_dirty, r, side, k) || (skip & AIE_DEV_SKIP_FLAT_CDA)) continue;
        const uint8_t* h = side ? R_U8(c, o_cda_bid_hist) : R_U8(c, o_cda_ask_hist);
        int f = 0;
        for (int i = 0; i < n; ++i) f += h[(r * n + i) * Pp + k];
        const float full = (float)f;
        pflat[P.fp_cda + (side ? AIE_FP_CDA_FULL_BIDS(Pp) : AIE_FP_CDA_FULL_ASKS(Pp)) + q] = full;
        for (int i = 0; i < n; ++i) {
          const float my = (float)h[(r * n + i) * Pp + k];
          const int fc = i * P.FA + P.fa_cda;
          AF(fc + (side ? AIE_FA_CDA_AVAILABLE_BIDS(Pp) : AIE_FA_CDA_AVAILABLE_ASKS(Pp)) + q, full - my);
          AF(fc + (side ? AIE_FA_CDA_MY_BIDS(Pp) : AIE_FA_CDA_MY_ASKS(Pp)) + q, my);
        }
      }
    }
  }
  if (tid < n && !(skip & AIE_DEV_SKIP_FLAT_STAGE_A)) {
    const int i = tid;
    const AgentScalars a(c, i);
    float* q = pag + i * P.FPA;
    a.write(c, arena, aflat, q, i, tval, isc);
    if (P.has_tax) a.write_marginal_rate(c, aflat, q, i);
  }
  if (tid == 0) {
    pflat[P.fp_time] = tval;
    reinterpret_cast<float*>(arena + c.R.a_obs_p_time)[c.e] = tval;
  }
  if (P.has_tax && !(skip & AIE_DEV_SKIP_FLAT_TAX)) {
    const TaxCalendar cal = tax_calendar(c);
    for (int i = tid; i <= n; i += AIE_NT) {
      if (i == n) {
        pflat[P.fp_tax + AIE_F_TAX_IS_FIRST_DAY(NB)] = cal.is_first_day;
        pflat[P.fp_tax + AIE_F_TAX_IS_TAX_DAY(NB)] = cal.is_tax_day;
        pflat[P.fp_tax + AIE_FP_TAX_PHASE(NB, n)] = cal.tax_phase;
      } else {
        AF(i * P.FA + P.fa_tax + AIE_F_TAX_IS_FIRST_DAY(NB), cal.is_first_day);
        AF(i * P.FA + P.fa_tax + AIE_F_TAX_IS_TAX_DAY(NB), cal.is_tax_day);
        AF(i * P.FA + P.fa_tax + AIE_FA_TAX_PHASE(NB, n), cal.tax_phase);
      }
    }
  }
  if (P.has_cda && !(skip & AIE_DEV_SKIP_FLAT_CDA)) {
    AIE_WSYNC();
    if (tid < 2) {
      const int r = tid;
      double tot;
      const float mr = cda_market_rate(c, r, tot);
      if (tot != 0) {
        pflat[P.fp_cda + AIE_FP_CDA_MARKET_RATE(Pp) + r] = mr;
        for (int i = 0; i < n; ++i) AF(i * P.FA + P.fa_cda + AIE_FA_CDA_MARKET_RATE(Pp) + r, mr);
      }
    }
  }
}


__device__ __forceinline__ void write_action_masks(const Ctx& c, uint8_t* __restrict__ arena, bool all = true) {
  const aie_params& P = c.P;
  const int n = P.n, tid = c.tid, Pp = P.P;
  const int skip = c.skipm;
  if (skip & AIE_DEV_SKIP_MASKS) return;
  if (!P.o_mask_bits) all = true;
  if (tid < n) {
    const int i = tid;
    const double coin = R_F64(c, o_inv_coin)[i];
    const int inv0 = R_I32(c, o_inv_res)[i], inv1 = R_I32(c, o_inv_res)[n + i];
    const int lr = R_I32(c, o_loc_r)[i], lc = R_I32(c, o_loc_c)[i];
    uint32_t mf = 0;
    if (P.has_build) mf |= agent_can_build(c, i) ? 1u : 0u;
    if (P.has_gather) {
      mf |= can_agent_occupy(c, lr, lc - 1, i) ? 2u : 0u;
      mf |= can_agent_occupy(c, lr, lc + 1, i) ? 4u : 0u;
      mf |= can_agent_occupy(c, lr - 1, lc, i) ? 8u : 0u;
      mf |= can_agent_occupy(c, lr + 1, lc, i) ? 16u : 0u;
    }
    if (P.has_cda) {
      int kmax = coin >= (double)(Pp - 1) ? Pp - 1 : (int)coin;
#pragma unroll
      for (int r = 0; r < 2; ++r) {
        const bool quota = R_I32(c, o_cda_n_orders)[r * n + i] < P.c.cda_max_num_orders;
        if (quota && (r ? inv1 : inv0) > 0) mf |= 32u << r;
        if (quota) mf |= (uint32_t)(kmax + 1) << (8 + 8 * r);
      }
    }
    const bool changed = all || (int32_t)mf != R_I32(c, o_mask_bits)[i];
    if (P.o_mask_bits) R_I32(c, o_mask_bits)[i] = (int32_t)mf;
    c.mflags[i] = (int32_t)(mf | (changed ? 0x80000000u : 0u));
  }
  AIE_WSYNC();
  {
    float* dst = reinterpret_cast<float*>(arena + c.R.a_obs_a_mask) + (int64_t)c.e * n * P.MA;
    const int count = n * P.MA;
    auto elem = [&](int idx) -> float {
      const int i = udiv(idx, P.MA, P.mg_MA), m = idx - i * P.MA;
      const uint32_t t = c.mtab[m];
      const uint32_t sh = t & 31u, msk = (t >> 8) & 0xffu, thr = t >> 16;
      return (((uint32_t)c.mflags[i] >> sh) & msk) >= thr ? 1.0f : 0.0f;
    };
    auto dirty = [&](int idx) -> bool { return c.mflags[udiv(idx, P.MA, P.mg_MA)] < 0; };
// ... 536 lines not shown
      const uint64_t mw = (uint64_t)sh->am[par][w][0] | ((uint64_t)sh->am[par][w][1] << 32);
      const int cw = __popcll(mw);
      if (w == wave) before_wave = total;
      if (!found && total + cw >= pairs) {
        used = w * AIE_NT + lg_kth_bit(mw, pairs - total, lane) + 1;
        found = true;
      }
      total += cw;
    }
    par ^= 1;
    if (acc && a < used) {
      const double f = sqrt(-2.0 * aie_log_glibc(r2) / r2);
      const int k = produced + 2 * (before_wave + __popcll(am & lanemask_lt(lane)));
      emit(k, f * x2);
      if (k + 1 < count) emit(k + 1, f * x1);
      else {
        *cache = f * x1;
        *has = 1;
      }
    }
    produced += 2 * (found ? pairs : total);
    mt3_consume(s, 4 * used, lane);
  }
  __syncthreads();
}

template <typename Planes>
__device__ __forceinline__ void layout_install(const Ctx& c, int gtid, int nthreads, Planes planes) {
  const aie_params& P = c.P;
  const aie_config& g = P.c;
  const int H = P.H, W = P.W, HW = P.HW;
  uint8_t* cb = reinterpret_cast<uint8_t*>(R_CELLS(c));
  for (int cell = gtid; cell < HW; cell += nthreads) {
    const int r = cell / W, col = cell - r * W;
    const uint32_t bits = planes(cell);
    bool st = (bits & 1u) != 0, wd = (bits & 2u) != 0;
    if (g.layout_checker && ((r & 1) + (col & 1)) != 1) st = wd = false;
    if (g.layout_gen == AIE_LAYOUT_QUADRANT && (col == H / 2 || r == W / 2)) st = wd = false;
    cb[4 * cell + 3] = (uint8_t)((cb[4 * cell + 3] & AIE_CELL_WATER) | (st ? AIE_CELL_STONE_SRC : 0) | (wd ? AIE_CELL_WOOD_SRC : 0));
  }
}
__device__ __forceinline__ void layout_generate(const Ctx& c, MT& m, const uint8_t* __restrict__ arena, uint8_t* extra, int gtid,
                                                int32_t* ghas, double* gcache, uint8_t* __restrict__ stage_out = nullptr) {
  const aie_params& P = c.P;
  const aie_config& g = P.c;
  const int H = P.H, W = P.W, HW = P.HW, lane = gtid & 63, wave = gtid >> 6;
  constexpr int NT = LG_NW * AIE_NT;
  const int hwp = (HW + 15) / 16 * 16;
  double* tmp = reinterpret_cast<double*>(extra);
  double* x = tmp + hwp;
  uint8_t* mbp[2] = {reinterpret_cast<uint8_t*>(x + hwp), reinterpret_cast<uint8_t*>(x + hwp) + hwp};
  int32_t* grid = reinterpret_cast<int32_t*>(mbp[1] + hwp);
  LgShared* sh = reinterpret_cast<LgShared*>(grid + 256);
  int par = 0, gpar = 0;
  const double* shared_prob = reinterpret_cast<const double*>(arena + c.R.a_layout_prob);
  const bool mz = g.layout_gen == AIE_LAYOUT_MULTI_ZONE;
  double mz_scale[2] = {0.0, 0.0};
  int size_r = 1, size_c = 1;
  if (mz) {
    const int regions = g.mz_rows * g.mz_cols;
    for (int k = gtid; k < regions; k += NT) {
      int z = -1;
      if (k < g.mz_zones[0]) z = 0;
      else if (k < g.mz_zones[0] + g.mz_zones[1]) z = 1;
      else if (k < g.mz_zones[0] + g.mz_zones[1] + g.mz_zones[2]) z = 2;
      grid[k] = z;
    }
    __syncthreads();
    for (int i = regions - 1; i >= 1; --i) {
      const int j = (int)rng_interval(m, lane, (uint32_t)i);
      if (gtid == 0) { const int t = grid[i]; grid[i] = grid[j]; grid[j] = t; }
      AIE_WSYNC();
    }
    __syncthreads();
    size_r = (H + g.mz_rows - 1) / g.mz_rows;
    size_c = (W + g.mz_cols - 1) / g.mz_cols;
    for (int rs = 0; rs < 2; ++rs) {
      const int own = rs == 1 ? 0 : 1;
      int cnt = 0;
      for (int base = 0; base < HW; base += NT) {
        const int cell = base + gtid;
        bool in = false;
        if (cell < HW) {
          const int r = cell / W, col = cell - r * W;
          const int z = grid[(r / size_r) * g.mz_cols + col / size_c];
          in = z == own || z == 2;
        }
        cnt += lg_block_count(in, sh, par, wave, lane);
      }
      mz_scale[rs] = (1.0 / ((double)cnt / (double)HW)) * c.R.c.layout_coverage[1];
    }
  }
  auto source_prob = [&](int rs, int cell, double clump) -> double {
    double v;
    if (mz) {
      const int r = cell / W, col = cell - r * W;
      const int z = grid[(r / size_r) * g.mz_cols + col / size_c];
      v = (z == (rs == 1 ? 0 : 1) || z == 2) ? mz_scale[rs] : 0.0;
    } else {
      v = shared_prob[rs * HW + cell];
    }
    return v * 0.1 * clump;
  };
#ifdef AIE_DEV
  uint64_t lg_acc[8] = {0, 0, 0, 0, 0, 0, 0, 0};
  const uint64_t lg_start = wall_clock64();
#endif
  MT3 s3;
  mt_copy(s3.w[0], m);
  s3.pos = m.pos;
  s3.have = 1;
  bool happy = false;
  for (int tries = 0; tries < 100 && !happy; ++tries) {
    LG_CNT(5);
    for (int q = 0; q < 2; ++q) {
      const int rs = q == 0 ? 1 : 0;
      const double cov = c.R.c.layout_coverage[rs], clump = c.R.c.layout_clump[rs];
      uint8_t* mb = mbp[rs];
      const uint8_t* other = q == 0 ? nullptr : mbp[1];
      { LG_T0();
      for (int base = 0; base < HW; base += NT) {
        const int nb = HW - base < NT ? HW - base : NT;
        mt3_need(s3, (s3.pos + 2 * nb - 1) / AIE_MT_N, lane);
        const int o = s3.pos + 2 * (gtid < nb ? gtid : nb - 1);
        const uint32_t a = mt3_word(s3, o), b = mt3_word(s3, o + 1);
        if (gtid < nb) tmp[base + gtid] = u53(a, b);
        mt3_consume(s3, 2 * nb, lane);
      }
      __syncthreads();
      LG_ACC(1); }
      int count = 0;
      for (int base = 0; base < HW; base += NT) {
        const int cell = base + gtid;
        bool on = false;
        if (cell < HW) {
          on = (tmp[cell] < source_prob(rs, cell, clump)) && !(other && other[cell]);
          mb[cell] = on ? 1 : 0;
        }
        count += lg_block_count(on, sh, par, wave, lane);
      }
      int n_tries = 0;
      if (HW <= NT) {
        const int cell = gtid < HW ? gtid : HW - 1;
        double t = tmp[cell];
        const double sp = source_prob(rs, cell, clump);
        const bool free_tile = gtid < HW && !(other && other[cell]);
        while ((double)count / (double)HW < cov * clump && n_tries <= 200) {
          LG_T0();
          LG_CNT(7);
          const int B = 201 - n_tries < 32 ? 201 - n_tries : 32;
          if (gtid < 32) sh->thr[gtid] = 0;
          __syncthreads();
          int first_on = 32;
          {
            double tk = t;
#pragma unroll
            for (int k = 0; k < 32; ++k) {
              tk = tk * 0.9;
              first_on = (first_on == 32 && (tk < sp) && k < B) ? k : first_on;
            }
            t = tk;
          }
          if (!free_tile) first_on = 32;
          if (first_on < 32) atomicAdd(&sh->thr[first_on], 1);
          __syncthreads();
          int mine = lane < 32 ? sh->thr[lane] : 0;
#pragma unroll
          for (int d = 1; d < 32; d <<= 1) {
            const int up = __shfl_up(mine, d, 64);
            mine += lane >= d ? up : 0;
          }
          const uint64_t reached = __ballot(lane < B && !((double)mine / (double)HW < cov * clump));
          const int stop = reached ? __ffsll((unsigned long long)reached) - 1 : B - 1;
          count = bcast(mine, stop);
          const uint32_t bits = first_on <= stop ? ~0u : 0u;
          n_tries += stop + 1;
          if (gtid < HW) mb[gtid] = (bits >> stop) & 1u;
          __syncthreads();
          LG_ACC(2);
        }
      } else
      while ((double)count / (double)HW < cov * clump && n_tries <= 200) {
        LG_T0();
        LG_CNT(7);
        const int B = 201 - n_tries < 8 ? 201 - n_tries : 8;
        if (gtid < 8) sh->thr[gtid] = 0;
        __syncthreads();
        for (int base = 0; base < HW; base += NT) {
          const int cell = base + gtid;
          uint32_t bits = 0;
          if (cell < HW) {
            double t = tmp[cell];
            const double sp = source_prob(rs, cell, clump);
            const bool free_tile = !(other && other[cell]);
#pragma unroll
            for (int k = 0; k < 8; ++k) {
              t = t * 0.9;
              bits |= ((t < sp) && free_tile && k < B) ? (1u << k) : 0u;
            }
            tmp[cell] = t;
            mb[cell] = (uint8_t)bits;
          }
#pragma unroll
          for (int k = 0; k < 8; ++k) {
            const int ck = __popcll(__ballot((bits >> k) & 1u));
            if (lane == 0 && ck) atomicAdd(&sh->thr[k], ck);
          }
        }
        __syncthreads();
        int stop = B - 1;
        for (int k = B - 1; k >= 0; --k)
          if (!((double)sh->thr[k] / (double)HW < cov * clump)) stop = k;
        stop = uni(stop);
        count = uni(sh->thr[stop]);
        n_tries += stop + 1;
        for (int base = 0; base < HW; base += NT) {
          const int cell = base + gtid;
          if (cell < HW) mb[cell] = (mb[cell] >> stop) & 1u;
        }
        __syncthreads();
        LG_ACC(2);
      }
      while ((double)count / (double)HW < cov) {
        LG_CNT(6);
        if (gtid < 2) sh->kbits[gtid] = 0;
        { LG_T0();
        lg_gauss(s3, 49 + HW, sh, gpar, wave, lane, ghas, gcache, [&](int k, double gs) {
          if (k < 49) {
            if (gs > 0) atomicOr(&sh->kbits[k >> 5], 1u << (k & 31));
          } else {
            const int cell = k - 49;
            x[cell] = ((double)mb[cell] + (0.2 * gs)) - 0.25;
          }
        });
        LG_ACC(3); }
        LG_T0();
        const uint64_t kmask = (uint64_t)sh->kbits[0] | ((uint64_t)sh->kbits[1] << 32);
        count = 0;
        for (int base = 0; base < HW; base += NT) {
          const int cell = base + gtid;
          bool on = false;
          if (cell < HW) {
            const int r0 = cell / W, c0 = cell - r0 * W;
            double win[49];
            uint32_t rowok = 0, colok = 0;
#pragma unroll
            for (int j = 0; j < 7; ++j) {
              rowok |= (r0 + 3 - j >= 0 && r0 + 3 - j < H) ? (1u << j) : 0u;
              colok |= (c0 + 3 - j >= 0 && c0 + 3 - j < W) ? (1u << j) : 0u;
            }
#pragma unroll
            for (int t = 0; t < 49; ++t) {
              const int j = t / 7, k = t - 7 * j;
              const bool inb = ((rowok >> j) & 1u) && ((colok >> k) & 1u);
              win[t] = inb ? x[cell + (3 - j) * W + (3 - k)] : 0.0;
            }
            double sum = 0.0;
#pragma unroll
            for (int t = 0; t < 49; ++t) {
              const int j = t / 7, k = t - 7 * j;
              if ((kmask >> t) & 1ull) {
                const bool inb = ((rowok >> j) & 1u) && ((colok >> k) & 1u);
                sum = inb ? sum + win[t] : sum;
              }
            }
            on = ((sum > 0) || mb[cell]) && !(other && other[cell]);
            mb[cell] = on ? 1 : 0;
          }
          count += lg_block_count(on, sh, par, wave, lane);
        }
        LG_ACC(4);
      }
    }
    happy = true;
    for (int q = 0; q < 2; ++q) {
      const int rs = q == 0 ? 1 : 0;
      int count = 0;
      for (int base = 0; base < HW; base += NT) {
        const int cell = base + gtid;
        count += lg_block_count(cell < HW && mbp[rs][cell], sh, par, wave, lane);
      }
      const double ratio = ((double)count / (double)HW) / c.R.c.layout_coverage[rs];
      if (!((1 / 1.4) <= ratio && ratio <= 1.4)) happy = false;
    }
  }
  mt_copy(m, s3.w[0]);
  m.pos = s3.pos;
  if (stage_out) {
    for (int cell = gtid; cell < HW; cell += NT) stage_out[cell] = (uint8_t)((mbp[0][cell] ? 1u : 0u) | (mbp[1][cell] ? 2u : 0u));
  } else {
    layout_install(c, gtid, NT, [&](int cell) -> uint32_t { return (mbp[0][cell] ? 1u : 0u) | (mbp[1][cell] ? 2u : 0u); });
  }
  __syncthreads();
#ifdef AIE_DEV
  if (c.R.dev_trace && gtid == 0) {
    lg_acc[0] = wall_clock64() - lg_start;
    for (int k = 0; k < 8; ++k) c.R.dev_trace[12 * c.e + k] = lg_acc[k];
  }
#endif
}
}

namespace aie {
template <int SPEC, bool LAYOUT = true>
__device__ __forceinline__ void reset_body(const aie_params* __restrict__ params, uint8_t* __restrict__ arena,
                                           const uint8_t* __restrict__ mask, int keep_rewards, uint8_t* lds) {
  const aie_params& R = *params;
  const aie_params& P = aie_spec_params<SPEC>(params);
  const int e = replica_of_block((int)blockIdx.x, R.E);
  if (mask && !mask[e]) return;
  const int gtid = (int)threadIdx.x, wave = gtid >> 6, nwaves = (int)blockDim.x >> 6;
  const Ctx c = make_ctx(P, R, lds, e, gtid & 63, arena);
  const int n = P.n, HW = P.HW, tid = c.tid;
  if (wave == 0) {
    for (int q = tid; q < (P.met_bytes >> 2); q += AIE_NT) reinterpret_cast<uint32_t*>(C_MET(c))[q] = 0u;
    if (c.ev && tid == 0) c.ev[0] = 0;
  }
  MT m;
  mt_init(m, P);
  load_record(c, arena, m, wave, nwaves, wave);
  __syncthreads();
  m.pos = uni(*R_I32(c, o_mt_pos));
  mt_fast_attach(c, m);
  if (LAYOUT && P.c.layout_gen != AIE_LAYOUT_FIXED) {
    if (aie__layout_staged(&P.c)) {
      uint32_t st[4];
#pragma unroll
      for (int k = 0; k < 4; ++k) st[k] = (uint32_t)uni((int)R_U32(c, o_mt)[k]);
      const uint64_t tag = aie_layout_tag(st);
      const uint64_t* tags = reinterpret_cast<const uint64_t*>(arena + R.a_layout_tag);
      int32_t* ctl = reinterpret_cast<int32_t*>(arena + R.a_layout_ctl);
      const uint64_t have = tags[e];
      const bool staged = (uint32_t)uni((int)(uint32_t)have) == (uint32_t)tag && (uint32_t)uni((int)(uint32_t)(have >> 32)) == (uint32_t)(tag >> 32);
      __syncthreads();
      if (staged) {
        const uint8_t* sp = arena + R.a_layout_stage + (int64_t)e * R.layout_stage_stride;
        layout_install(c, gtid, LG_NW * AIE_NT, [&](int cell) -> uint32_t { return sp[cell]; });
        __syncthreads();
      } else {
        LgShared* sh = lg_shared(lds + lds_bytes(P), P);
        if (gtid == 0) {
          sh->lhas = 0;
          sh->lcache = 0.0;
        }
        __syncthreads();
        uint32_t ks[2];
        aie_layout_stream(st, ks);
        MT ml;
        mt_init(ml, P);
        ml.fkey = ks[0];
        ml.fblk = 0xffffffffu;
        ml.fsalt = ks[1];
        layout_generate(c, ml, arena, lds + lds_bytes(P), gtid, &sh->lhas, &sh->lcache);
      }
      if (gtid == 0) {
        R_U32(c, o_mt)[3] = st[3] + 1u;
        atomicAdd(&ctl[0], 1);
        atomicAdd(&ctl[staged ? 2 : 3], 1);
      }
    } else {
      layout_generate(c, m, arena, lds + lds_bytes(P), gtid, R_I32(c, o_mt_has_gauss), R_F64(c, o_mt_gauss));
    }
    if (wave != 0) return;
  }
  {
    uint32_t* cells = R_CELLS(c);
    for (int q = tid; q < HW; q += AIE_NT) {
      const uint32_t fl = cells[q] >> 24;
      cells[q] = AIE_CELL_PACK((fl & AIE_CELL_STONE_SRC) ? 1 : 0, (fl & AIE_CELL_WOOD_SRC) ? 1 : 0, 0xff, fl);
    }
    if (tid < n) {
      R_I32(c, o_inv_res)[tid] = 0; R_I32(c, o_inv_res)[n + tid] = 0;
      R_I32(c, o_esc_res)[tid] = 0; R_I32(c, o_esc_res)[n + tid] = 0;
      R_F64(c, o_inv_coin)[tid] = c.R.c.starting_agent_coin;
      R_F64(c, o_esc_coin)[tid] = 0;
      R_F64(c, o_labor)[tid] = 0;
      R_I32(c, o_loc_r)[tid] = -1;
      R_I32(c, o_loc_c)[tid] = -1;
      if (!P.has_build) { R_F64(c, o_build_payment)[tid] = 0; R_F64(c, o_build_skill)[tid] = 0; }
      if (!P.has_gather) R_F64(c, o_bonus_gather_prob)[tid] = 0;
    }
    if (P.has_cda) {
      for (int q = tid; q < 2 * P.M; q += AIE_NT) { R_I32(c, o_cda_bids)[q] = 0; R_I32(c, o_cda_asks)[q] = 0; }
      for (int q = tid; q < 2 * n * P.P; q += AIE_NT) {
        R_U8(c, o_cda_bid_hist)[q] = 0; R_U8(c, o_cda_ask_hist)[q] = 0;
        R_F64(c, o_cda_price_history)[q] = 0;
      }
      for (int q = tid; q < 2 * n; q += AIE_NT) R_I32(c, o_cda_n_orders)[q] = 0;
      if (tid < 2) { R_I32(c, o_cda_n_bids)[tid] = 0; R_I32(c, o_cda_n_asks)[tid] = 0; }
    }
  }
  __syncthreads();
  build_src_list(c, arena);
  if (P.regen_conv) {
    const uint8_t* cb = reinterpret_cast<const uint8_t*>(R_CELLS(c));
    for (int q = tid; q < AIE_N_RES * HW; q += AIE_NT) {
      const int rs = q >= HW ? 1 : 0, cell = q - rs * HW, r0 = cell / P.W, c0 = cell - r0 * P.W;
      const int hw = P.c.regen_halfwidth[rs];
      const uint32_t bit = rs ? AIE_CELL_WOOD_SRC : AIE_CELL_STONE_SRC;
      int cnt = 0;
      for (int r = max(r0 - hw, 0); r <= min(r0 + hw, P.H - 1); ++r)
        for (int cc = max(c0 - hw, 0); cc <= min(c0 + hw, P.W - 1); ++cc)
          cnt += (cb[4 * (r * P.W + cc) + 3] & bit) ? 1 : 0;
      R_U8(c, o_regen_count)[q] = (uint8_t)cnt;
    }
  }
  rebuild_locmap(c);
  *R_I32(c, o_timestep) = 0;
  *R_I32(c, o_error_flags) = 0;
  const int place_perm = P.c.reset_random_order ? rng_permutation(m, tid, n) : tid;
  for (int k = 0; k < n; ++k) {
    const int i = bcast(place_perm, k);
    int r = (int)rng_interval(m, tid, (uint32_t)(P.H - 1)), col = (int)rng_interval(m, tid, (uint32_t)(P.W - 1)), tries = 0;
    while (!can_agent_occupy(c, r, col, i)) {
      r = (int)rng_interval(m, tid, (uint32_t)(P.H - 1));
      col = (int)rng_interval(m, tid, (uint32_t)(P.W - 1));
      if (++tries > 200) {
        *R_I32(c, o_error_flags) |= AIE_ERR_RESET_PLACEMENT;
        break;
      }
    }
    R_I32(c, o_loc_r)[i] = r;
    R_I32(c, o_loc_c)[i] = col;
    c.locmap[r * P.W + col] = (uint8_t)(i + 1);
  }
  for (int k = 0; k < P.c.n_components; ++k) {
    switch (P.c.components[k]) {
      case AIE_COMP_BUILD:
        for (int i = 0; i < n; ++i) {
          double skill = 1, pay = 1;
          const double pm = (double)c.R.c.build_payment_max_skill_multiplier;
          if (P.c.build_skill_dist == AIE_SKILL_PARETO) {
            skill = rng_pareto(m, tid, 4.0);
            pay = (pm - 1) * skill + 1; if (pm < pay) pay = pm;
          } else if (P.c.build_skill_dist == AIE_SKILL_LOGNORMAL) {
            skill = rng_lognormal(c, m, -1.0, 0.5);
            pay = (pm - 1) * skill + 1; if (pm < pay) pay = pm;
          }
          R_F64(c, o_build_payment)[i] = pay * (double)c.R.c.build_payment;
          R_F64(c, o_build_skill)[i] = skill;
        }
        break;
      case AIE_COMP_GATHER:
        for (int i = 0; i < n; ++i) {
          double b = 0.0;
          if (P.c.gather_skill_dist == AIE_SKILL_PARETO) { b = rng_pareto(m, tid, 3.0); b = (b < 2 ? b : 2) / 2; }
          else if (P.c.gather_skill_dist == AIE_SKILL_LOGNORMAL) { b = rng_lognormal(c, m, -2.022, 0.938); b = (b < 2 ? b : 2) / 2; }
          R_F64(c, o_bonus_gather_prob)[i] = b;
        }
        break;
      case AIE_COMP_TAX:
        for (int b = 0; b < P.NB; ++b) R_I32(c, o_tax_rate_idx)[b] = 0;
        *R_I32(c, o_tax_cycle_pos) = 1;
        for (int i = 0; i < n; ++i) {
          R_F64(c, o_tax_last_coin)[i] = R_F64(c, o_inv_coin)[i] + R_F64(c, o_esc_coin)[i];
          R_F64(c, o_tax_last_income)[i] = 0;
          R_F64(c, o_tax_last_marginal_rate)[i] = 0;
        }
        *R_F64(c, o_tax_total_collected) = 0;
        if (P.c.tax_model == AIE_TAX_SAEZ) {
          for (int b = 0; b < P.NB; ++b) R_F64(c, o_tax_saez_obs_rates)[b] = tax_rate(c, b);
          AIE_WSYNC();
          for (int b = 0; b < P.NB; ++b)
            R_F64(c, o_tax_saez_rates)[b] = reinterpret_cast<const double*>(saez_block(c) + AIE_SAEZ_OFF_AVG)[b];
        }
        break;
      default: break;
    }
  }
  if (P.c.fixed_four_skill_and_loc) {
    for (int i = 0; i < n; ++i) {
      c.locmap[R_I32(c, o_loc_r)[i] * P.W + R_I32(c, o_loc_c)[i]] = 0;
      R_I32(c, o_loc_r)[i] = -1;
      R_I32(c, o_loc_c)[i] = -1;
    }
    const int perm = rng_permutation(m, tid, n);
    for (int k = 0; k < n; ++k) {
      const int i = bcast(perm, k);
      const int r = c.R.c.ranked_locs[k][0], col = c.R.c.ranked_locs[k][1];
      if (can_agent_occupy(c, r, col, i)) {
        R_I32(c, o_loc_r)[i] = r;
        R_I32(c, o_loc_c)[i] = col;
        c.locmap[r * P.W + col] = (uint8_t)(i + 1);
      }
      R_F64(c, o_build_payment)[i] = c.R.c.avg_ranked_skill[k];
    }
  }
  if (P.c.split_water_line > 0) {
    for (int i = 0; i < n; ++i) {
      c.locmap[R_I32(c, o_loc_r)[i] * P.W + R_I32(c, o_loc_c)[i]] = 0;
      R_I32(c, o_loc_r)[i] = -1;
      R_I32(c, o_loc_c)[i] = -1;
    }
    const int perm = rng_permutation(m, tid, n);
    const int wl = P.c.split_water_line;
    for (int k = 0; k < n; ++k) {
      const int i = bcast(perm, k);
      R_F64(c, o_build_payment)[i] = c.R.c.avg_ranked_skill[k];
      const bool top = (c.R.c.split_top_ranks[k >> 5] >> (k & 31)) & 1u;
      const int r_min = top ? 0 : wl + 1, r_max = top ? wl : P.H;
      int r = r_min + (int)rng_interval(m, tid, (uint32_t)(r_max - r_min - 1));
      int col = (int)rng_interval(m, tid, (uint32_t)(P.W - 1)), tries = 0;
      while (!can_agent_occupy(c, r, col, i)) {
        r = r_min + (int)rng_interval(m, tid, (uint32_t)(r_max - r_min - 1));
        col = (int)rng_interval(m, tid, (uint32_t)(P.W - 1));
        if (++tries > 200) {
          *R_I32(c, o_error_flags) |= AIE_ERR_RESET_PLACEMENT;
          break;
        }
      }
      R_I32(c, o_loc_r)[i] = r;
      R_I32(c, o_loc_c)[i] = col;
      c.locmap[r * P.W + col] = (uint8_t)(i + 1);
    }
  }
  *R_I32(c, o_mt_pos) = m.pos;
  mt_fast_detach(c, m);
  __syncthreads();
  current_metrics(c);
  __syncthreads();
  if (tid <= n) R_F64(c, o_util)[tid] = scr_part(c)[tid];
  __syncthreads();
  write_spatial_observations(c, arena);
  if (tid == 0) *R_I32(c, o_obs_valid) = 1;
  write_flat_observations(c, arena);
  AIE_WSYNC();
  if (P.has_tax && P.c.tax_annealing && tid == 0) *R_I32(c, o_tax_last_completions) = *R_I32(c, o_completions);
  AIE_WSYNC();
  write_action_masks(c, arena);
  if (!keep_rewards) {
    if (tid < n) reinterpret_cast<float*>(arena + R.a_rew_a)[(int64_t)e * n + tid] = 0.0f;
    if (tid == 0) {
      reinterpret_cast<float*>(arena + R.a_rew_p)[e] = 0.0f;
      (arena + R.a_done)[e] = 0;
    }
  }
  __syncthreads();
  store_record(c, arena, m);
}
}

#ifndef AIE_JIT
extern "C" __global__ void __launch_bounds__(AIE_NT)
aie_reset_kernel(const aie_params* __restrict__ params, uint8_t* __restrict__ arena,
                 const uint8_t* __restrict__ mask, int keep_rewards) {
  extern __shared__ __attribute__((aligned(16))) uint8_t lds[];
  aie::reset_body<-1, false>(params, arena, mask, keep_rewards, lds);
}
extern "C" __global__ void __launch_bounds__(LG_NW * AIE_NT)
aie_reset_kernel_layout(const aie_params* __restrict__ params, uint8_t* __restrict__ arena,
                        const uint8_t* __restrict__ mask, int keep_rewards) {
  extern __shared__ __attribute__((aligned(16))) uint8_t lds[];
  aie::reset_body<-1, true>(params, arena, mask, keep_rewards, lds);
}
extern "C" __global__ void aie_layout_decide_kernel(const aie_params* __restrict__ params, uint8_t* __restrict__ arena, int threshold) {
  int32_t* ctl = reinterpret_cast<int32_t*>(arena + params->a_layout_ctl);
  const bool go = ctl[0] >= threshold;
  ctl[1] = go ? 1 : 0;
  if (go) ctl[0] = 0;
}
extern "C" __global__ void __launch_bounds__(LG_NW * AIE_NT)
aie_layout_refill_kernel(const aie_params* __restrict__ params, uint8_t* __restrict__ arena) {
  extern __shared__ __attribute__((aligned(16))) uint8_t lds[];
  const aie_params& P = *params;
  const int32_t* ctl = reinterpret_cast<const int32_t*>(arena + P.a_layout_ctl);
  if (!ctl[1]) return;
  const int e = (int)blockIdx.x, gtid = (int)threadIdx.x;
  const uint32_t* stg = reinterpret_cast<const uint32_t*>(arena + P.a_records + (int64_t)e * P.rec_bytes + P.o_mt);
  uint32_t st[4];
#pragma unroll
  for (int k = 0; k < 4; ++k) st[k] = (uint32_t)aie::uni((int)stg[k]);
  const uint64_t tag = aie_layout_tag(st);
  uint64_t* tags = reinterpret_cast<uint64_t*>(arena + P.a_layout_tag);
  const uint64_t have = tags[e];
  if ((uint32_t)aie::uni((int)(uint32_t)have) == (uint32_t)tag && (uint32_t)aie::uni((int)(uint32_t)(have >> 32)) == (uint32_t)(tag >> 32)) return;
  const aie::Ctx c = aie::make_ctx(P, P, lds, e, gtid & 63, arena);
  aie::LgShared* sh = aie::lg_shared(lds + aie::lds_bytes(P), P);
  if (gtid == 0) {
    sh->lhas = 0;
    sh->lcache = 0.0;
  }
  __syncthreads();
  uint32_t ks[2];
  aie_layout_stream(st, ks);
  aie::MT ml;
  aie::mt_init(ml, P);
  ml.fkey = ks[0];
  ml.fblk = 0xffffffffu;
  ml.fsalt = ks[1];
  aie::layout_generate(c, ml, arena, lds + aie::lds_bytes(P), gtid, &sh->lhas, &sh->lcache,
                       arena + P.a_layout_stage + (int64_t)e * P.layout_stage_stride);
  if (gtid == 0) tags[e] = tag;
}
template <int SPEC>
__global__ void __launch_bounds__(LG_NW * AIE_NT)
aie_reset_kernel_spec(const aie_params* __restrict__ params, uint8_t* __restrict__ arena,
                      const uint8_t* __restrict__ mask, int keep_rewards) {
  extern __shared__ __attribute__((aligned(16))) uint8_t lds[];
  aie::reset_body<SPEC>(params, arena, mask, keep_rewards, lds);
}

extern "C" __global__ void aie_seed_kernel(const aie_params P, uint8_t* __restrict__ arena, uint64_t base_seed) {
  const int e = (int)(blockIdx.x * blockDim.x + threadIdx.x);
  if (e >= P.E) return;
  uint8_t* rec = arena + P.a_records + (int64_t)e * P.rec_bytes;
  uint32_t* mt = reinterpret_cast<uint32_t*>(rec + P.o_mt);
  if (aie::rng_fast(P)) {
    const uint64_t s = base_seed + (uint64_t)e;
    mt[0] = (uint32_t)s;
    mt[1] = 0u;
    mt[2] = ((uint32_t)(s >> 32) & 0xffffu) << 16;
    mt[3] = 0u;
  } else {
    uint32_t x = (uint32_t)base_seed + (uint32_t)e;
    mt[0] = x;
    for (int i = 1; i < AIE_MT_N; ++i) {
      x = 1812433253u * (x ^ (x >> 30)) + (uint32_t)i;
      mt[i] = x;
    }
  }
  *reinterpret_cast<int32_t*>(rec + P.o_mt_pos) = AIE_MT_N;
  *reinterpret_cast<int32_t*>(rec + P.o_mt_has_gauss) = 0;
  *reinterpret_cast<double*>(rec + P.o_mt_gauss) = 0.0;
}

extern "C" __global__ void aie_sample_actions_kernel(const aie_params P, const uint8_t* __restrict__ arena, uint64_t seed,
                                                     int64_t env_offset, int32_t* __restrict__ act_a,
                                                     int32_t* __restrict__ act_p) {
  const int64_t q = (int64_t)blockIdx.x * blockDim.x + threadIdx.x;
  const int per_env = P.n * P.act_a_width + P.act_p_width;
  if (q >= (int64_t)P.E * per_env) return;
  const int e = (int)(q / per_env);
  const int64_t t = *reinterpret_cast<const int32_t*>(arena + P.a_records + (int64_t)e * P.rec_bytes + P.o_sample_t);
  aie::sample_action_slot(P, seed, env_offset, t, e, (int)(q - (int64_t)e * per_env), act_a, act_p);
}
extern "C" __global__ void aie_sample_advance_kernel(uint8_t* __restrict__ arena, int64_t a_records, int rec_bytes,
                                                     int o_sample_t, int E) {
  const int e = (int)(blockIdx.x * blockDim.x + threadIdx.x);
  if (e < E) *reinterpret_cast<int32_t*>(arena + a_records + (int64_t)e * rec_bytes + o_sample_t) += 1;
}

extern "C" __global__ void aie_sample_masked_actions_kernel(const aie_params P, const uint8_t* __restrict__ arena,
                                                            uint64_t seed, int64_t env_offset,
                                                            int32_t* __restrict__ act_a, int32_t* __restrict__ act_p) {
  const int64_t q = (int64_t)blockIdx.x * blockDim.x + threadIdx.x;
  const int per_env = P.n * P.act_a_width + P.act_p_width;
  if (q >= (int64_t)P.E * per_env) return;
  const int e = (int)(q / per_env);
  const int j = (int)(q - (int64_t)e * per_env);
  const int64_t t = *reinterpret_cast<const int32_t*>(arena + P.a_records + (int64_t)e * P.rec_bytes + P.o_sample_t);
  const uint32_t u = aie_counter_rng(seed, (uint64_t)(env_offset + e), (uint64_t)t, (uint64_t)j);
  const float* mask;
  int lo, len, stride = 1;
  int32_t* dst;
  const bool covid = P.c.scenario == AIE_SCN_COVID;
  if (j < P.n * P.act_a_width) {
    if (!act_a) return;
    const int i = j / P.act_a_width, s = j - i * P.act_a_width;
    if (covid) {
      mask = reinterpret_cast<const float*>(arena + P.a_cv_obs_a) + ((int64_t)e * P.cv_nrow_obs + AIE_CV_OB_MASK) * P.n + i;
      stride = P.n;
    } else {
      mask = reinterpret_cast<const float*>(arena + P.a_obs_a_mask) + ((int64_t)e * P.n + i) * P.MA;
    }
    if (P.c.multi_action_mode_agents) {
      lo = 0;
      for (int k = 0; k < s; ++k) lo += 1 + P.sub_a_dim[k];
      len = P.n_sub_a ? 1 + P.sub_a_dim[s] : 1;
    } else {
      lo = 0;
      len = covid ? 1 + P.cv_NL : P.MA;
    }
    dst = act_a + (int64_t)e * P.n * P.act_a_width + j;
  } else {
    if (!act_p) return;
    const int s = j - P.n * P.act_a_width;
    if (covid) mask = reinterpret_cast<const float*>(arena + P.a_cv_obs_p) + (int64_t)e * (4 + P.MP) + 4;
    else mask = reinterpret_cast<const float*>(arena + P.a_obs_p_mask) + (int64_t)e * P.MP;
    if (P.c.multi_action_mode_planner) {
      lo = s * (1 + P.p_row_dim);
      len = 1 + P.p_row_dim;
    } else {
      lo = 0;
      len = P.MP;
    }
    dst = act_p + (int64_t)e * P.act_p_width + s;
  }
  int count = 0;
  for (int k = 0; k < len; ++k) count += mask[(lo + k) * stride] > 0.5f ? 1 : 0;
  if (count == 0) { *dst = 0; return; }
  int pick = (int)(((uint64_t)u * (uint64_t)count) >> 32);
  int chosen = 0;
  for (int k = 0; k < len; ++k) {
    if (mask[(lo + k) * stride] > 0.5f) {
      if (pick == 0) { chosen = k; break; }
      --pick;
    }
  }
  *dst = chosen;
}

__device__ __forceinline__ float sampler_row16_max(float m) {
  asm("s_nop 4\n\t"
      "v_max_f32_dpp %0, %0, %0 row_ror:1 row_mask:0xf bank_mask:0xf\n\ts_nop 1\n\t"
      "v_max_f32_dpp %0, %0, %0 row_ror:2 row_mask:0xf bank_mask:0xf\n\ts_nop 1\n\t"
      "v_max_f32_dpp %0, %0, %0 row_ror:4 row_mask:0xf bank_mask:0xf\n\ts_nop 1\n\t"
      "v_max_f32_dpp %0, %0, %0 row_ror:8 row_mask:0xf bank_mask:0xf\n\ts_nop 1"
      : "+v"(m));
  return m;
}
__device__ __forceinline__ float sampler_max_raw(float a, float b) {
  float r;
  asm("v_max_f32 %0, %1, %2" : "=v"(r) : "v"(a), "v"(b));
  return r;
}
__device__ __forceinline__ float sampler_segment_max(float m, int seg) {
  m = sampler_row16_max(m);
  if (seg >= 32) {
    const auto r = __builtin_amdgcn_permlane16_swap(__float_as_uint(m), __float_as_uint(m), false, false);
    m = sampler_max_raw(__uint_as_float(r[0]), __uint_as_float(r[1]));
  }
  if (seg >= 64) {
    const auto r = __builtin_amdgcn_permlane32_swap(__float_as_uint(m), __float_as_uint(m), false, false);
    m = sampler_max_raw(__uint_as_float(r[0]), __uint_as_float(r[1]));
  }
  return m;
}
__device__ __forceinline__ float sampler_scan(float v, int seg) {
  asm("s_nop 4\n\t"
      "v_add_f32_dpp %0, %0, %0 row_shr:1 row_mask:0xf bank_mask:0xf bound_ctrl:1\n\ts_nop 1\n\t"
      "v_add_f32_dpp %0, %0, %0 row_shr:2 row_mask:0xf bank_mask:0xf bound_ctrl:1\n\ts_nop 1\n\t"
      "v_add_f32_dpp %0, %0, %0 row_shr:4 row_mask:0xf bank_mask:0xf bound_ctrl:1\n\ts_nop 1\n\t"
      "v_add_f32_dpp %0, %0, %0 row_shr:8 row_mask:0xf bank_mask:0xf bound_ctrl:1\n\ts_nop 1"
      : "+v"(v));
  if (seg >= 32) asm("s_nop 4\n\tv_add_f32_dpp %0, %0, %0 row_bcast:15 row_mask:0xa bank_mask:0xf\n\ts_nop 1" : "+v"(v));
  if (seg >= 64) asm("s_nop 4\n\tv_add_f32_dpp %0, %0, %0 row_bcast:31 row_mask:0xc bank_mask:0xf\n\ts_nop 1" : "+v"(v));
  return v;
}
template <bool LOGP>
struct SamplerLogp {
  float *a, *p;
};
template <>
struct SamplerLogp<false> {};
template <bool LOGP>
__device__ __forceinline__ float* sampler_logp_of(const SamplerLogp<LOGP>& lp, bool planner) {
  if constexpr (LOGP) return planner ? lp.p : lp.a;
  else return nullptr;
}
struct SamplerItem {
  const float *lg, *mk;
  int32_t* dst;
  int len, lrs, mrs, mks;
  int rows, lsh;
  uint32_t j0;
};
struct SamplerGroup {
  const float *lg, *mk;
  int32_t* dst;
  int len, lrs, mrs, mks, rpw, lsh, rows, items, slot0;
};
__device__ __forceinline__ SamplerGroup sampler_group(const aie_sampler_group& g, const uint8_t* __restrict__ arena,
                                                      const float* __restrict__ logits, int32_t* __restrict__ act, int e, int slot0) {
  SamplerGroup G;
  G.lg = logits + (uint64_t)(uint32_t)e * g.lg_estride;
  G.mk = reinterpret_cast<const float*>(arena + g.mk_off) + (uint64_t)(uint32_t)e * g.mk_estride;
  G.dst = act + (uint64_t)(uint32_t)e * (uint32_t)g.rows;
  G.len = g.len;
  G.lrs = g.lrs;
  G.mrs = g.mrs;
  G.mks = g.mks;
  G.lsh = g.lsh;
  G.rpw = 64 >> g.lsh;
  G.rows = g.rows;
  G.items = (act && logits) ? (g.rows + G.rpw - 1) >> (6 - g.lsh) : 0;
  G.slot0 = slot0;
  return G;
}
__device__ __forceinline__ SamplerItem sampler_item(const aie_sampler_args& S, const SamplerGroup& A, const SamplerGroup& Q, int it) {
  SamplerItem d;
  const bool ag = it < A.items;
  const int rpw = ag ? A.rpw : Q.rpw, r0 = (ag ? it : it - A.items) * rpw, rows = ag ? A.rows : Q.rows;
  const float* lg = ag ? A.lg : Q.lg;
  const float* mk = ag ? A.mk : Q.mk;
  d.lrs = ag ? A.lrs : Q.lrs;
  d.mrs = ag ? A.mrs : Q.mrs;
  d.mks = ag ? A.mks : Q.mks;
  d.lsh = ag ? A.lsh : Q.lsh;
  d.len = ag ? A.len : Q.len;
  d.dst = (ag ? A.dst : Q.dst) + r0;
  d.j0 = (uint32_t)(r0 + (ag ? A.slot0 : Q.slot0));
  d.rows = rows - r0 < rpw ? rows - r0 : rpw;
  if (ag && S.ragged) {
    const int i = r0 / S.act_a_width, s = r0 - i * S.act_a_width;
    int lo = 0;
    for (int k = 0; k < s; ++k) lo += 1 + S.params->sub_a_dim[k];
    d.len = S.params->n_sub_a ? 1 + S.params->sub_a_dim[s] : 1;
    d.lg = lg + (int64_t)i * d.lrs + lo;
    d.mk = mk + (int64_t)i * d.mrs + lo;
  } else {
    d.lg = lg + (int64_t)r0 * d.lrs;
    d.mk = mk + (int64_t)r0 * d.mrs;
  }
  return d;
}
__device__ __forceinline__ void sampler_item_load(const SamplerItem& d, int lane, float& x, float& mv) {
  const int sub = lane >> d.lsh, kk = lane & ((1 << d.lsh) - 1);
  const bool inb = sub < d.rows && kk < d.len;
  x = d.lg[inb ? __mul24(sub, d.lrs) + kk : 0];
  mv = d.mk[inb ? __mul24(sub, d.mrs) + __mul24(kk, d.mks) : 0];
}
template <bool LOGP>
__device__ __forceinline__ void sampler_item_run(const SamplerItem& d, int lane, const float x0, const float mv0, uint32_t base,
                                                 float* __restrict__ lp) {
  const int lsh = d.lsh, segw = 1 << lsh, rpw = 64 >> lsh, len = d.len;
  const int sub = lane >> lsh, kk = lane & (segw - 1);
  const int nch = rpw > 1 ? 1 : (len + 63) >> 6;
  const int seg = rpw > 1 ? segw : (len > 32 ? 64 : aie_sampler_segment(len));
  const int lgo = __mul24(sub, d.lrs) + kk, mko = __mul24(sub, d.mrs) + __mul24(kk, d.mks);
  const bool ok0 = sub < d.rows && kk < len && mv0 > 0.5f && x0 == x0;
  float m = ok0 ? x0 : -INFINITY;
  for (int ch = 1; ch < nch; ++ch)
    if (64 * ch + kk < len) {
      const float x = d.lg[lgo + 64 * ch];
      if (d.mk[mko + 64 * ch * d.mks] > 0.5f && x > m) m = x;
    }
  const float M = sampler_segment_max(m, seg);
  uint32_t rnd = 0u;
  for (int s = 0; s < rpw; ++s) {
    const uint32_t h = aie_sampler_entry_rng(base, d.j0 + (uint32_t)s);
    rnd = sub == s ? h : rnd;
  }
  const float u = aie_sampler_uniform(rnd);
  int choice = -1, last_ok = -1, outv = 0;
  float T = 0.0f;
  bool had_ok = false;
  for (int pass = (nch > 1 ? 0 : 1); pass < 2; ++pass) {
    float carry = 0.0f;
    for (int ch = 0; ch < nch; ++ch) {
      float x = x0;
      bool ok = ok0;
      if (ch > 0) {
        ok = false;
        if (64 * ch + kk < len) {
          x = d.lg[lgo + 64 * ch];
          ok = d.mk[mko + 64 * ch * d.mks] > 0.5f && x == x;
        }
      }
      const float w = ok ? aie_sampler_expf(x - M) : 0.0f;
      const float c = carry + sampler_scan(w, seg);
      if (rpw == 1) {
        const float tot = __builtin_bit_cast(float, __builtin_amdgcn_readlane(__builtin_bit_cast(int, c), seg - 1));
        if (pass == 0) {
          carry = tot;
          continue;
        }
        if (nch == 1) T = tot;
        const uint64_t oks = __ballot(ok), hits = __ballot(ok && c > u * T);
        if (choice < 0 && hits) choice = 64 * ch + (__ffsll((unsigned long long)hits) - 1);
        if (oks) last_ok = 64 * ch + (63 - __clzll((long long)oks));
        carry = tot;
      } else {
        float Ts = 0.0f;
        for (int s = 0; s < rpw; ++s) {
          const float tot = __builtin_bit_cast(float, __builtin_amdgcn_readlane(__builtin_bit_cast(int, c), (s << lsh) + segw - 1));
          Ts = sub == s ? tot : Ts;
        }
        if (LOGP) T = Ts;
        const uint64_t oks = __ballot(ok), hits = __ballot(ok && c > u * Ts);
        const uint64_t sm = (1ull << segw) - 1ull;
        for (int s = 0; s < rpw; ++s) {
          const uint64_t h = (hits >> (s << lsh)) & sm, o = (oks >> (s << lsh)) & sm;
          const int pick = h ? __ffsll((unsigned long long)h) - 1 : (o ? 63 - __clzll((long long)o) : 0);
          outv = sub == s ? pick : outv;
          if (LOGP) had_ok = sub == s ? o != 0ull : had_ok;
        }
      }
    }
    if (pass == 0) T = carry;
  }
  if (rpw == 1) outv = choice < 0 ? (last_ok < 0 ? 0 : last_ok) : choice;
  if (sub < d.rows && kk == 0) d.dst[sub] = outv;
  if constexpr (LOGP) {
    if (rpw == 1) had_ok = last_ok >= 0;
    if (sub < d.rows && kk == 0) {
      float lpv = 0.0f;
      if (had_ok && T > 0.0f) lpv = (d.lg[__mul24(sub, d.lrs) + outv] - M) - aie_sampler_logf(T);
      lp[sub] = lpv;
    }
  }
}
#ifdef AIE_DEV
__device__ __forceinline__ int sampler_dev_skip(int& wpr_log2) {
  const int bits = wpr_log2 >> 8;
  wpr_log2 &= 255;
  return bits;
}
#else
__device__ constexpr int sampler_dev_skip(int&) { return 0; }
#endif
#define AIE_SAMPLER_GROUP 4
template <bool LOGP>
// ... 206 lines not shown
    }
  }
  __syncthreads();
  if (e < S.E && w_in == 0 && lane == 0 && !(dev_skip & AIE_SAMPLER_SKIP_DRAW_INDEX)) {
    int32_t* tfield = reinterpret_cast<int32_t*>(arena + S.t_off + (int64_t)e * S.rec_bytes);
    *tfield = *tfield + 1;
  }
}
#define AIE_SAMPLER_FAST(LA, LQ) \
  template __global__ void aie_sample_policy_fast_kernel<LA, LQ, false>(const aie_sampler_args, uint8_t*, const float*, const float*, \
                                                                        uint64_t, int64_t, int32_t*, int32_t*, int, const SamplerLogp<false>); \
  template __global__ void aie_sample_policy_fast_kernel<LA, LQ, true>(const aie_sampler_args, uint8_t*, const float*, const float*, \
                                                                       uint64_t, int64_t, int32_t*, int32_t*, int, const SamplerLogp<true>);
AIE_SAMPLER_FAST(4, 4) AIE_SAMPLER_FAST(4, 5) AIE_SAMPLER_FAST(4, 6)
AIE_SAMPLER_FAST(5, 4) AIE_SAMPLER_FAST(5, 5) AIE_SAMPLER_FAST(5, 6)
AIE_SAMPLER_FAST(6, 4) AIE_SAMPLER_FAST(6, 5) AIE_SAMPLER_FAST(6, 6)

template <int LSH>
__device__ __forceinline__ float policy_segment_total(float c) {
  if (LSH == 6) return __builtin_bit_cast(float, __builtin_amdgcn_readlane(__builtin_bit_cast(int, c), 63));
  return __builtin_bit_cast(float, __builtin_amdgcn_ds_swizzle(__builtin_bit_cast(int, c), LSH == 5 ? 0x3E0 : 0x1F0));
}
template <int LSH, bool BWD>
__device__ __forceinline__ void policy_eval_fast(const aie_policy_eval_group& G, uint32_t b, uint32_t gi, int lane) {
  constexpr int SEG = 1 << LSH, RPW = 64 >> LSH;
  const int sub = lane >> LSH, kk = lane & (SEG - 1);
  const uint32_t r0 = gi << (6 - LSH);
  const int rows = (int)((uint32_t)G.rows - r0) < RPW ? (int)((uint32_t)G.rows - r0) : RPW;
  const bool in = sub < rows && kk < G.len;
  const float* lgb = G.lg + ((uint64_t)b * G.lg_bstride + (uint64_t)r0 * (uint32_t)G.lrs);
  const float* mkb = G.mk + ((uint64_t)b * G.mk_bstride + (uint64_t)r0 * (uint32_t)G.mrs);
  const uint64_t row0 = (uint64_t)b * (uint32_t)G.rows + r0;
  const uint32_t lgo = in ? (uint32_t)(__mul24(sub, G.lrs) + kk) : 0u;
  const uint32_t mko = in ? (uint32_t)(__mul24(sub, G.mrs) + __mul24(kk, G.mks)) : 0u;
  const uint32_t ro = sub < rows ? (uint32_t)sub : 0u;
  const float x = lgb[lgo];
  const float mv = mkb[mko];
  int a = 0;
  if (G.act) a = G.act[row0 + ro];
  float gl = 0.0f, gh = 0.0f;
  if (BWD) {
    if (G.g_logp) gl = G.g_logp[row0 + ro];
    if (G.g_ent) gh = G.g_ent[row0 + ro];
  }
  const bool ok = in && mv > 0.5f && x == x;
  const float M = sampler_segment_max(ok ? x : -INFINITY, SEG);
  const float y = x - M;
  const float w = ok ? aie_sampler_expf(y) : 0.0f;
  const bool live = ok && y > -80.0f;
  const float v = live ? w * y : 0.0f;
  const float T = policy_segment_total<LSH>(sampler_scan(w, SEG));
  const float S = policy_segment_total<LSH>(sampler_scan(v, SEG));
  const bool any = T > 0.0f;
  const float Ts = any ? T : 1.0f;
  const float L = aie_sampler_logf(Ts);
  const float H = any ? L - __fdiv_rn(S, Ts) : 0.0f;
  const bool a_in = a >= 0 && a < G.len;
  if (!BWD) {
    if (G.logp && sub < rows && kk == (a_in ? a : 0))
      G.logp[row0 + sub] = !any ? 0.0f : (a_in && ok) ? y - L : -INFINITY;
    if (G.ent && sub < rows && kk == 0) G.ent[row0 + sub] = H;
  } else {
    const uint64_t hit = __ballot(ok && kk == a);
    const bool a_ok = LSH == 6 ? hit != 0ull : ((hit >> (lane & ~(SEG - 1))) & ((1ull << (SEG & 63)) - 1ull)) != 0ull;
    float g = 0.0f;
    if (ok && any) g = aie_policy_entry_grad(y, w, Ts, L, H, kk == a, a_ok ? gl : 0.0f, gh);
    if (in) (G.grad + ((uint64_t)b * G.lg_bstride + (uint64_t)r0 * (uint32_t)G.lrs))[lgo] = g;
  }
}
template <bool BWD>
__device__ __forceinline__ void policy_eval_generic(const aie_policy_eval_args& A, const aie_policy_eval_group& G, bool agents,
                                                    uint32_t b, uint32_t row, int lane) {
  int len = G.len;
  uint32_t lo = row * (uint32_t)G.lrs, mlo = row * (uint32_t)G.mrs;
  if (agents && A.ragged) {
    const int i = (int)row / A.act_a_width, s = (int)row - i * A.act_a_width;
    int off = 0;
    for (int k = 0; k < s; ++k) off += 1 + A.params->sub_a_dim[k];
    len = A.params->n_sub_a ? 1 + A.params->sub_a_dim[s] : 1;
    lo = (uint32_t)(i * G.lrs + off);
    mlo = (uint32_t)(i * G.mrs + off * G.mks);
  }
  const float* lg = G.lg + ((uint64_t)b * G.lg_bstride + lo);
  const float* mk = G.mk + ((uint64_t)b * G.mk_bstride + mlo);
  const uint64_t ri = (uint64_t)b * (uint32_t)G.rows + row;
  const int nch = (len + 63) >> 6, seg = nch > 1 ? 64 : aie_sampler_segment(len);
  const int a = G.act ? G.act[ri] : 0;
  const bool a_in = a >= 0 && a < len;
  const float xa = lg[a_in ? a : 0], ma = mk[(a_in ? a : 0) * G.mks];
  const bool a_ok = a_in && ma > 0.5f && xa == xa;
  float m = -INFINITY;
  for (int ch = 0; ch < nch; ++ch) {
    const int k = 64 * ch + lane;
    if (k < len) {
      const float x = lg[k];
      if (mk[k * G.mks] > 0.5f && x > m) m = x;
    }
  }
  const float M = sampler_segment_max(m, 64);
  float T = 0.0f, S = 0.0f;
  for (int ch = 0; ch < nch; ++ch) {
    const int k = 64 * ch + lane;
    float w = 0.0f, v = 0.0f;
    if (k < len) {
      const float x = lg[k];
      if (mk[k * G.mks] > 0.5f && x == x) {
        const float y = x - M;
        w = aie_sampler_expf(y);
        v = y > -80.0f ? w * y : 0.0f;
      }
    }
    const float c = T + sampler_scan(w, seg), cs = S + sampler_scan(v, seg);
    T = __builtin_bit_cast(float, __builtin_amdgcn_readlane(__builtin_bit_cast(int, c), seg - 1));
    S = __builtin_bit_cast(float, __builtin_amdgcn_readlane(__builtin_bit_cast(int, cs), seg - 1));
  }
  const bool any = T > 0.0f;
  const float Ts = any ? T : 1.0f;
  const float L = aie_sampler_logf(Ts);
  const float H = any ? L - __fdiv_rn(S, Ts) : 0.0f;
  if (!BWD) {
    if (lane == 0) {
      if (G.logp) G.logp[ri] = !any ? 0.0f : a_ok ? (xa - M) - L : -INFINITY;
      if (G.ent) G.ent[ri] = H;
    }
  } else {
    const float gl = (G.g_logp && a_ok) ? G.g_logp[ri] : 0.0f, gh = G.g_ent ? G.g_ent[ri] : 0.0f;
    float* gr = G.grad + ((uint64_t)b * G.lg_bstride + lo);
    for (int ch = 0; ch < nch; ++ch) {
      const int k = 64 * ch + lane;
      if (k < len) {
        const float x = lg[k];
        float g = 0.0f;
        if (any && mk[k * G.mks] > 0.5f && x == x) {
          const float y = x - M;
          g = aie_policy_entry_grad(y, aie_sampler_expf(y), Ts, L, H, k == a, gl, gh);
        }
        gr[k] = g;
      }
    }
  }
}
template <bool BWD>
__device__ __forceinline__ void policy_eval_body(const aie_policy_eval_args& A) {
  const int lane = (int)threadIdx.x & 63;
  const uint32_t wv = (uint32_t)aie::uni((int)(blockIdx.x * 4u + (threadIdx.x >> 6)));
  asm volatile("" ::"s"(A.agents.lg), "s"(A.agents.mk), "s"(A.agents.act), "s"(A.agents.logp), "s"(A.agents.ent), "s"(A.agents.grad),
               "s"(A.agents.g_logp), "s"(A.agents.g_ent), "s"(A.agents.lg_bstride), "s"(A.agents.mk_bstride), "s"(A.agents.len),
               "s"(A.agents.lrs), "s"(A.agents.mrs), "s"(A.agents.mks), "s"(A.agents.lsh), "s"(A.agents.rows), "s"(A.agents.items),
               "s"(A.agents.generic));
  asm volatile("" ::"s"(A.planner.lg), "s"(A.planner.mk), "s"(A.planner.act), "s"(A.planner.logp), "s"(A.planner.ent),
               "s"(A.planner.grad), "s"(A.planner.g_logp), "s"(A.planner.g_ent), "s"(A.planner.lg_bstride), "s"(A.planner.mk_bstride),
               "s"(A.planner.len), "s"(A.planner.lrs), "s"(A.planner.mrs), "s"(A.planner.mks), "s"(A.planner.lsh), "s"(A.planner.rows),
               "s"(A.planner.items), "s"(A.planner.generic), "s"(A.B), "s"(A.items));
  const uint32_t b = wv / A.items, it = wv - b * A.items;
  if (b >= A.B) return;
  const bool ag = it < (uint32_t)A.agents.items;
  const aie_policy_eval_group G = ag ? A.agents : A.planner;
  const uint32_t gi = ag ? it : it - (uint32_t)A.agents.items;
  if (G.generic) policy_eval_generic<BWD>(A, G, ag, b, gi, lane);
  else if (G.lsh == 4) policy_eval_fast<4, BWD>(G, b, gi, lane);
  else if (G.lsh == 5) policy_eval_fast<5, BWD>(G, b, gi, lane);
  else policy_eval_fast<6, BWD>(G, b, gi, lane);
}
extern "C" __global__ void __launch_bounds__(256) aie_policy_eval_kernel(const aie_policy_eval_args A) { policy_eval_body<false>(A); }
extern "C" __global__ void __launch_bounds__(256) aie_policy_eval_bwd_kernel(const aie_policy_eval_args A) { policy_eval_body<true>(A); }

#define AIE_GAE_U 8
struct GaeLane {
  const float *r, *d, *v;
  float *adv, *ret;
  uint32_t row, vstride;
};
__device__ __forceinline__ void gae_load(const GaeLane& L, int t0, int slot0, int slots, float (&r)[AIE_GAE_U], float (&d)[AIE_GAE_U],
                                         float (&v)[AIE_GAE_U]) {
#pragma unroll
  for (int k = 0; k < AIE_GAE_U; ++k) {
    const int t = t0 - k;
    r[k] = d[k] = v[k] = 0.0f;
    if (t >= 0) {
      const int s = slot0 - k < 0 ? slot0 - k + slots : slot0 - k;
      r[k] = L.r[(size_t)s * L.row];
      d[k] = L.d[(size_t)s * L.row];
      v[k] = L.v[(size_t)t * L.vstride];
    }
  }
}
__device__ __forceinline__ void gae_chunk(const GaeLane& L, int t0, const float (&r)[AIE_GAE_U], const float (&d)[AIE_GAE_U],
                                          const float (&v)[AIE_GAE_U], float gamma, float gl, float& v_next, float& a_next) {
#pragma unroll
  for (int k = 0; k < AIE_GAE_U; ++k) {
    const int t = t0 - k;
    if (t >= 0) {
      const float a = aie_gae_step(r[k], v[k], v_next, a_next, d[k] > 0.5f, gamma, gl);
      if (L.adv) L.adv[(size_t)t * L.vstride] = a;
      if (L.ret) L.ret[(size_t)t * L.vstride] = aie_gae_return(a, v[k]);
      a_next = a;
      v_next = v[k];
    }
  }
}
extern "C" __global__ void __launch_bounds__(64) aie_gae_kernel(const aie_gae_args A) {
  asm volatile("" ::"s"(A.log), "s"(A.va), "s"(A.vp), "s"(A.adv_a), "s"(A.adv_p), "s"(A.ret_a), "s"(A.ret_p), "s"(A.T), "s"(A.slots),
               "s"(A.first), "s"(A.E), "s"(A.n), "s"(A.gamma), "s"(A.gl));
  const uint32_t W = (uint32_t)A.n + 2u, row = (uint32_t)A.E * W;
  const uint32_t c = blockIdx.x * 64u + threadIdx.x;
  if (c >= row) return;
  const uint32_t e = c / W, j = c - e * W;
  const bool agent = j < (uint32_t)A.n;
  const float* vals = agent ? A.va : A.vp;
  if (j > (uint32_t)A.n || !vals) return;
  GaeLane L;
  L.row = row;
  L.vstride = agent ? (uint32_t)A.E * (uint32_t)A.n : (uint32_t)A.E;
  const uint32_t vo = agent ? e * (uint32_t)A.n + j : e;
  L.r = A.log + c;
  L.d = A.log + (e * W + (uint32_t)A.n + 1u);
  L.v = vals + vo;
  L.adv = agent ? A.adv_a : A.adv_p;
  L.ret = agent ? A.ret_a : A.ret_p;
  if (L.adv) L.adv += vo;
  if (L.ret) L.ret += vo;
  const int T = A.T, slots = A.slots;
  float v_next = L.v[(size_t)T * L.vstride], a_next = 0.0f;
  int t0 = T - 1;
  int slot0 = (int)((uint32_t)A.first + (uint32_t)t0);
  if (slot0 < 0 || slot0 >= slots) slot0 = (int)((uint32_t)slot0 - (uint32_t)slots);
  float r0[AIE_GAE_U], d0[AIE_GAE_U], v0[AIE_GAE_U], r1[AIE_GAE_U], d1[AIE_GAE_U], v1[AIE_GAE_U];
  gae_load(L, t0, slot0, slots, r0, d0, v0);
  while (t0 >= 0) {
    int sn = slot0 - AIE_GAE_U;
    if (sn < 0) sn += slots;
    gae_load(L, t0 - AIE_GAE_U, sn, slots, r1, d1, v1);
    gae_chunk(L, t0, r0, d0, v0, A.gamma, A.gl, v_next, a_next);
    t0 -= AIE_GAE_U;
    slot0 = sn - AIE_GAE_U;
    if (slot0 < 0) slot0 += slots;
    if (t0 < 0) break;
    gae_load(L, t0 - AIE_GAE_U, slot0, slots, r0, d0, v0);
    gae_chunk(L, t0, r1, d1, v1, A.gamma, A.gl, v_next, a_next);
    t0 -= AIE_GAE_U;
  }
}

extern "C" __global__ void __launch_bounds__(256) aie_trajectory_store_kernel(const aie_traj_args A) {
  const uint32_t e = blockIdx.x;
  int32_t s = A.slot[e];
  __syncthreads();
  if (threadIdx.x == 0) A.slot[e] = (uint32_t)s + 1u < (uint32_t)A.n_slots ? s + 1 : 0;
  if ((uint32_t)s >= (uint32_t)A.n_slots) s = 0;
  const int lane = (int)threadIdx.x & 63;
  for (int g = aie::uni((int)(threadIdx.x >> 6)); g < A.n_segs; g += 4) {
    const uint8_t* src = A.seg[g].src + (int64_t)e * A.seg[g].src_stride;
    const int32_t bytes = A.seg[g].bytes, rows = A.seg[g].rows;
    uint8_t* dst = A.seg[g].dst + ((int64_t)s * A.E + e) * bytes;
    if (rows > 1) {
      const uint32_t* s32 = reinterpret_cast<const uint32_t*>(src);
      uint32_t* d32 = reinterpret_cast<uint32_t*>(dst);
      const uint32_t count = (uint32_t)bytes >> 2, cols = count / (uint32_t)rows;
      for (uint32_t i = (uint32_t)lane; i < count; i += 64u) {
        const uint32_t cc = i / (uint32_t)rows, rr = i - cc * (uint32_t)rows;
        d32[i] = s32[rr * cols + cc];
      }
    } else if (A.seg[g].wide) {
      const uint4* s128 = reinterpret_cast<const uint4*>(src);
      uint4* d128 = reinterpret_cast<uint4*>(dst);
      for (uint32_t i = (uint32_t)lane; i < ((uint32_t)bytes >> 4); i += 64u) d128[i] = s128[i];
    } else {
      const uint32_t* s32 = reinterpret_cast<const uint32_t*>(src);
      uint32_t* d32 = reinterpret_cast<uint32_t*>(dst);
      for (uint32_t i = (uint32_t)lane; i < ((uint32_t)bytes >> 2); i += 64u) d32[i] = s32[i];
    }
  }
}
#endif

#if defined(AIE_JIT) && !defined(AIE_JIT_OSE)
#ifdef AIE_JIT_PAD_NOPS
extern "C" __global__ void aie_jit_pad() {
#define AIE_STR2(x) #x
#define AIE_STR(x) AIE_STR2(x)
  asm volatile(".rept " AIE_STR(AIE_JIT_PAD_NOPS) "\n s_nop 0\n .endr");
}
#endif
extern "C" __global__ void aie_jit_keep_helpers_generic(const double* a, int n, uint32_t M, int o, int m, uint32_t* gkey,
                                                        uint32_t* w, int cap, int pos, double* out) {
  const int lane = (int)threadIdx.x & 63;
  out[0] = aie::np_sum_leaf(a, n, 1, M, o, m, lane);
  const aie::Refill r = aie::rng_refill(gkey, w, cap, pos, lane);
  const aie::Refill rf = aie::rng_refill_fast(gkey, w, cap, pos, lane);
  out[1] = (double)(r.pos + r.avail + r.twisted + rf.pos + rf.avail + rf.twisted);
  aie::MTRows t;
  for (int j = 0; j < 10; ++j) t.r[j] = gkey[64 * j + lane];
  t = aie::mt_twist_rows(t, lane);
  const aie::MTRows f = aie::mt_fast_rows_of(gkey[0], gkey[1], gkey[2], lane);
  for (int j = 0; j < 10; ++j) gkey[64 * j + lane] = t.r[j] ^ f.r[j];
}
extern "C" __global__ void __launch_bounds__(2 * AIE_NT)
__attribute__((amdgpu_waves_per_eu(aie_spec_image<0>::waves, aie_spec_image<0>::waves)))
aie_jit_step(const aie_params* __restrict__ params, uint8_t* __restrict__ arena,
             const int32_t* __restrict__ act_a, const int32_t* __restrict__ act_p, NextActions next) {
  extern __shared__ __attribute__((aligned(16))) uint8_t lds[];
  step_body<false, 0>(params, arena, act_a, act_p, lds, next);
}
extern "C" __global__ void __launch_bounds__(LG_NW * AIE_NT)
aie_jit_reset(const aie_params* __restrict__ params, uint8_t* __restrict__ arena,
              const uint8_t* __restrict__ mask, int keep_rewards) {
  extern __shared__ __attribute__((aligned(16))) uint8_t lds[];
  aie::reset_body<0>(params, arena, mask, keep_rewards, lds);
}
#endif
```

Baseline: 734.3 million agent-steps/s.

## Restructure reset: per-wave work split, grouped masked resets, single-wave full reset

Reset work is now split across waves: wave 0 handles placement and skills, one side wave builds source lists and action masks, another computes utility, and the spatial observation writes are spread over the remaining waves. Masked resets gather 8 replicas per block and, when enough LDS is available, run several replicas at once with one wave each, so blocks for unmasked replicas are not launched. Unmasked full resets use a new single-wave kernel, and occupancy hints are added. The aim is to shorten the serial reset critical path and cut idle blocks, at the cost of more complex synchronisation and more LDS per block.

```diff
diff --git a/ai-economist_amd/csrc/aie_capi.hip b/ai-economist_amd/csrc/aie_capi.hip
--- a/ai-economist_amd/csrc/aie_capi.hip
+++ b/ai-economist_amd/csrc/aie_capi.hip
@@ -176,14 +176,16 @@
   bool module;
   unsigned block;
   size_t lds;
+  unsigned grid;
 };
 
 static const struct aie_spec_kernels {
   aie_kernel<aie_step_fn> step[AIE_N_SPECS], traced[AIE_N_SPECS], ose[AIE_N_SPECS];
-  aie_kernel<aie_reset_fn> reset[AIE_N_SPECS];
+  aie_kernel<aie_reset_fn> reset[AIE_N_SPECS], reset_all[AIE_N_SPECS];
 } aie_spec_kernel = [] {
   aie_spec_kernels t{};
-#define AIE_GTB_ROW(K) t.step[K] = AIE_KERNEL(aie_step_kernel_spec<K>), t.reset[K] = AIE_KERNEL(aie_reset_kernel_spec<K>);
+#define AIE_GTB_ROW(K) t.step[K] = AIE_KERNEL(aie_step_kernel_spec<K>), t.reset[K] = AIE_KERNEL(aie_reset_kernel_spec<K>), \
+                       t.reset_all[K] = AIE_KERNEL(aie_reset_all_kernel_spec<K>);
 #define AIE_OSE_ROW(K) t.ose[K] = AIE_KERNEL(aie_ose_step_kernel_spec<K>);
 #define AIE_TRACED_ROW(K) t.traced[K] = AIE_KERNEL(aie_step_kernel_spec_trace<K>);
   AIE_SPEC_LIST_GTB(AIE_GTB_ROW)
@@ -252,23 +254,31 @@
   return (env->P.E & 7) ? (unsigned)L : (L <= E8 ? (unsigned)(8 * (L - 1) + 1) : (unsigned)env->P.E);
 }
 
-static aie_route<aie_reset_fn> aie_select_reset(const aie_env* env) {
+static aie_route<aie_reset_fn> aie_select_reset(const aie_env* env, bool masked) {
   const aie_params& P = env->P;
-  if (P.c.scenario == AIE_SCN_COVID) return {AIE_KERNEL(aie_covid_reset_kernel), false, AIE_NT, 0};
-  if (P.c.scenario == AIE_SCN_ONE_STEP_ECONOMY) return {{nullptr, "aie_ose_reset_kernel"}, false, OSE_NT, env->lds};
+  const unsigned E = (unsigned)P.E;
+  if (P.c.scenario == AIE_SCN_COVID) return {AIE_KERNEL(aie_covid_reset_kernel), false, AIE_NT, 0, E};
+  if (P.c.scenario == AIE_SCN_ONE_STEP_ECONOMY) return {{nullptr, "aie_ose_reset_kernel"}, false, OSE_NT, env->lds, E};
   const bool layout = P.c.layout_gen != AIE_LAYOUT_FIXED;
-  aie_route<aie_reset_fn> r = {AIE_KERNEL(aie_reset_kernel), false, AIE_NT, env->lds + aie::layout_gen_lds_bytes(P)};
-  if (layout) r.k = AIE_KERNEL(aie_reset_kernel_layout), r.block = LG_NW * AIE_NT;
+  aie_route<aie_reset_fn> r = {AIE_KERNEL(aie_reset_kernel), false, LG_NW * AIE_NT, env->lds + aie::layout_gen_lds_bytes(P), E};
+  aie_kernel<aie_reset_fn> all = AIE_KERNEL(aie_reset_all_kernel);
+  if (layout) r.k = AIE_KERNEL(aie_reset_kernel_layout);
   if (P.dev_skip_mask == 0 && !env->dev_generic) {
     if (env->spec == AIE_KERNEL_INSTANCE_JIT) r.k = {nullptr, "aie_jit_reset"}, r.module = true;
-    else if (env->spec >= 0 && env->spec < AIE_N_SPECS && aie_spec_kernel.reset[env->spec].fn) r.k = aie_spec_kernel.reset[env->spec];
-  }
+    else if (env->spec >= 0 && env->spec < AIE_N_SPECS && aie_spec_kernel.reset[env->spec].fn)
+      r.k = aie_spec_kernel.reset[env->spec], all = aie_spec_kernel.reset_all[env->spec];
+  }
+  if (masked && !layout) {
+    r.grid = (E + AIE_RESET_GROUP - 1) / AIE_RESET_GROUP;
+    if (env->lds * LG_NW <= AIE_RESET_DENSE_LDS_MAX) r.lds = env->lds * LG_NW;
+  }
+  if (!masked && !layout && !r.module) r.k = all, r.block = AIE_NT;
   return r;
 }
 
 static void aie_launch_reset(aie_env* env, const uint8_t* d_mask, int keep_rewards, void* stream) {
-  const aie_route<aie_reset_fn> r = aie_select_reset(env);
-  const dim3 g((unsigned)env->P.E), b(r.block);
+  const aie_route<aie_reset_fn> r = aie_select_reset(env, d_mask != nullptr);
+  const dim3 ge((unsigned)env->P.E), g(r.grid), b(r.block);
   hipStream_t st = static_cast<hipStream_t>(stream);
   if (r.module) {
     const aie_params* dp = env->d_params;
@@ -283,7 +293,7 @@
   if (env->P.c.scenario == AIE_SCN_GTB && aie__layout_staged(&env->P.c)) {
     const int threshold = env->P.E >= 4 ? (int)(env->P.E / 4) : 1;
     hipLaunchKernelGGL(aie_layout_decide_kernel, dim3(1), dim3(1), 0, st, env->d_params, env->arena, threshold);
-    hipLaunchKernelGGL(aie_layout_refill_kernel, g, dim3(LG_NW * AIE_NT), r.lds, st, env->d_params, env->arena);
+    hipLaunchKernelGGL(aie_layout_refill_kernel, ge, dim3(LG_NW * AIE_NT), r.lds, st, env->d_params, env->arena);
   }
 }
 
@@ -1329,7 +1339,7 @@
       s += std::string(" + ") + aie_cv_window_kernel[P.cv_F - 1][env->cv_taps_f32 ? 1 : 0].name;
   }
   if (rc != AIE_OK) s = "error " + std::to_string(rc);
-  snprintf(buf, (size_t)n, "%s | %s", s.c_str(), aie_select_reset(env).k.name);
+  snprintf(buf, (size_t)n, "%s | %s", s.c_str(), aie_select_reset(env, true).k.name);
   return AIE_OK;
 }
 #endif
diff --git a/ai-economist_amd/csrc/aie_kernels.hip b/ai-economist_amd/csrc/aie_kernels.hip
--- a/ai-economist_amd/csrc/aie_kernels.hip
+++ b/ai-economist_amd/csrc/aie_kernels.hip
@@ -1927,14 +1927,15 @@
 }
 
 template <bool WATER>
-__device__ __forceinline__ void write_spatial_observations_t(const Ctx& c, uint8_t* __restrict__ arena) {
+__device__ __forceinline__ void write_spatial_observations_t(const Ctx& c, uint8_t* __restrict__ arena, int part = 0,
+                                                             int nparts = 1) {
   constexpr int CM = WATER ? 6 : 5;
   const int n = c.P.n, HW = c.P.HW;
   const uint32_t* cells = R_CELLS(c);
   const SpatialOut o = spatial_out<WATER>(c, arena);
   if (c.P.c.full_observability) {
     const uint32_t* lm4f = reinterpret_cast<const uint32_t*>(c.locmap);
-    for (int i = 0; i < n; ++i) {
+    for (int i = part; i < n; i += nparts) {
       const int so = i * CM * HW * 4, si = i * 2 * HW * 2;
       for (int q = c.tid; q < (HW >> 2); q += AIE_NT) {
         const uint4 cw = reinterpret_cast<const uint4*>(cells)[q];
@@ -1974,12 +1975,12 @@
       }
     }
   } else {
-    for (int i = 0; i < n; ++i) crop_agent<WATER>(c, o, i);
+    for (int i = part; i < n; i += nparts) crop_agent<WATER>(c, o, i);
   }
   if (c.P.c.planner_gets_spatial_info) {
     const int nq4 = HW >> 2;
     const uint32_t* lm4 = reinterpret_cast<const uint32_t*>(c.locmap);
-    for (int q = c.tid; q < nq4; q += AIE_NT) {
+    for (int q = part * AIE_NT + c.tid; q < nq4; q += nparts * AIE_NT) {
       const uint4 cw = reinterpret_cast<const uint4*>(cells)[q];
       const uint32_t cws[4] = {cw.x, cw.y, cw.z, cw.w};
       float ch[4][6];
@@ -2006,7 +2007,8 @@
         for (int u = 0; u < 4; ++u) buf_store_i16(o.pidx, (int)((oc[u >> 1] >> (16 * (u & 1))) & 0xffffu), 8 * q + 2 * u, HW * 2);
       }
     }
-    for (int cell = 4 * nq4 + c.tid; cell < HW; cell += AIE_NT) planner_cell<WATER>(c, o, cell);
+    if (part == 0)
+      for (int cell = 4 * nq4 + c.tid; cell < HW; cell += AIE_NT) planner_cell<WATER>(c, o, cell);
   }
 }
 
@@ -2058,9 +2060,10 @@
   }
   if (c.P.c.planner_gets_spatial_info && cell >= 0) planner_cell<WATER>(c, o, cell);
 }
-__device__ __forceinline__ void write_spatial_observations(const Ctx& c, uint8_t* __restrict__ arena) {
-  if (c.P.c.has_water) write_spatial_observations_t<true>(c, arena);
-  else write_spatial_observations_t<false>(c, arena);
+__device__ __forceinline__ void write_spatial_observations(const Ctx& c, uint8_t* __restrict__ arena, int part = 0,
+                                                           int nparts = 1) {
+  if (c.P.c.has_water) write_spatial_observations_t<true>(c, arena, part, nparts);
+  else write_spatial_observations_t<false>(c, arena, part, nparts);
 }
 __device__ __forceinline__ void update_spatial_observations(const Ctx& c, uint8_t* __restrict__ arena) {
   if (c.P.c.has_water) update_spatial_observations_t<true>(c, arena);
@@ -3203,27 +3206,45 @@
 }
 
 namespace aie {
-template <int SPEC, bool LAYOUT = true>
+#ifdef AIE_DEV
+#define RS_STAMP(k) do { if (!fresh_layout && R.dev_trace && tid == 0) R.dev_trace[12 * e + (k)] = wall_clock64(); } while (0)
+#else
+#define RS_STAMP(k) do {} while (0)
+#endif
+#define RS_SYNC() do { if constexpr (alone) AIE_WSYNC(); else __syncthreads(); } while (0)
+template <int SPEC, bool LAYOUT = true, int NW = LG_NW>
 __device__ __forceinline__ void reset_body(const aie_params* __restrict__ params, uint8_t* __restrict__ arena,
-                                           const uint8_t* __restrict__ mask, int keep_rewards, uint8_t* lds) {
+                                           int keep_rewards, uint8_t* lds, int e) {
   const aie_params& R = *params;
   const aie_params& P = aie_spec_params<SPEC>(params);
-  const int e = replica_of_block((int)blockIdx.x, R.E);
-  if (mask && !mask[e]) return;
-  const int gtid = (int)threadIdx.x, wave = gtid >> 6, nwaves = (int)blockDim.x >> 6;
+  static_assert(NW == 1 || NW == LG_NW, "one wave, or the layout generator's count");
+  constexpr int nwaves = NW, NT = NW * AIE_NT;
+  constexpr bool alone = NW == 1;
+  const int gtid = alone ? (int)threadIdx.x & (AIE_NT - 1) : (int)threadIdx.x, wave = alone ? 0 : gtid >> 6;
+  const bool fresh_layout = LAYOUT && P.c.layout_gen != AIE_LAYOUT_FIXED;
+  const bool solo = alone || fresh_layout;
+  const int w_side = solo ? 0 : 1, w_util = solo ? 0 : nwaves - 1;
+  const int regen_w0 = w_side, regen_nw = solo ? 1 : 2;
+  const int map_part = solo ? 0 : wave - 1, map_parts = solo ? 1 : nwaves - 1;
+  const bool maps_here = solo ? wave == 0 : wave != 0;
   const Ctx c = make_ctx(P, R, lds, e, gtid & 63, arena);
   const int n = P.n, HW = P.HW, tid = c.tid;
-  if (wave == 0) {
-    for (int q = tid; q < (P.met_bytes >> 2); q += AIE_NT) reinterpret_cast<uint32_t*>(C_MET(c))[q] = 0u;
-    if (c.ev && tid == 0) c.ev[0] = 0;
-  }
+  const bool replaces = P.c.fixed_four_skill_and_loc || P.c.split_water_line > 0;
+  const bool skill_draws = (P.has_build && P.c.build_skill_dist != AIE_SKILL_NONE) ||
+                           (P.has_gather && P.c.gather_skill_dist != AIE_SKILL_NONE);
+  const bool maps_early = skill_draws && !replaces;
+  const bool latch = P.has_tax && P.c.tax_annealing;
+  if (wave == 0) RS_STAMP(0);
+  for (int q = gtid; q < (P.met_bytes >> 2); q += NT) reinterpret_cast<uint32_t*>(C_MET(c))[q] = 0u;
+  if (c.ev && gtid == 0) c.ev[0] = 0;
   MT m;
   mt_init(m, P);
-  load_record(c, arena, m, wave, nwaves, wave);
-  __syncthreads();
+  load_record(c, arena, m, wave, nwaves, (fresh_layout && !aie__layout_staged(&P.c)) ? wave : 0);
+  RS_SYNC();
+  if (wave == 0) RS_STAMP(1);
   m.pos = uni(*R_I32(c, o_mt_pos));
-  mt_fast_attach(c, m);
-  if (LAYOUT && P.c.layout_gen != AIE_LAYOUT_FIXED) {
+  if (wave == 0 || fresh_layout) mt_fast_attach(c, m);
+  if (fresh_layout) {
     if (aie__layout_staged(&P.c)) {
       uint32_t st[4];
 #pragma unroll
@@ -3262,40 +3283,42 @@
     } else {
       layout_generate(c, m, arena, lds + lds_bytes(P), gtid, R_I32(c, o_mt_has_gauss), R_F64(c, o_mt_gauss));
     }
-    if (wave != 0) return;
   }
   {
     uint32_t* cells = R_CELLS(c);
-    for (int q = tid; q < HW; q += AIE_NT) {
+    for (int q = gtid; q < HW; q += NT) {
       const uint32_t fl = cells[q] >> 24;
       cells[q] = AIE_CELL_PACK((fl & AIE_CELL_STONE_SRC) ? 1 : 0, (fl & AIE_CELL_WOOD_SRC) ? 1 : 0, 0xff, fl);
     }
-    if (tid < n) {
-      R_I32(c, o_inv_res)[tid] = 0; R_I32(c, o_inv_res)[n + tid] = 0;
-      R_I32(c, o_esc_res)[tid] = 0; R_I32(c, o_esc_res)[n + tid] = 0;
-      R_F64(c, o_inv_coin)[tid] = c.R.c.starting_agent_coin;
-      R_F64(c, o_esc_coin)[tid] = 0;
-      R_F64(c, o_labor)[tid] = 0;
-      R_I32(c, o_loc_r)[tid] = -1;
-      R_I32(c, o_loc_c)[tid] = -1;
-      if (!P.has_build) { R_F64(c, o_build_payment)[tid] = 0; R_F64(c, o_build_skill)[tid] = 0; }
-      if (!P.has_gather) R_F64(c, o_bonus_gather_prob)[tid] = 0;
+    uint32_t* lm = reinterpret_cast<uint32_t*>(c.locmap);
+    for (int q = gtid; q < ((HW + 3) >> 2); q += NT) lm[q] = 0;
+    if (gtid < n) {
+      R_I32(c, o_inv_res)[gtid] = 0; R_I32(c, o_inv_res)[n + gtid] = 0;
+      R_I32(c, o_esc_res)[gtid] = 0; R_I32(c, o_esc_res)[n + gtid] = 0;
+      R_F64(c, o_inv_coin)[gtid] = c.R.c.starting_agent_coin;
+      R_F64(c, o_esc_coin)[gtid] = 0;
+      R_F64(c, o_labor)[gtid] = 0;
+      R_I32(c, o_loc_r)[gtid] = -1;
+      R_I32(c, o_loc_c)[gtid] = -1;
+      if (!P.has_build) { R_F64(c, o_build_payment)[gtid] = 0; R_F64(c, o_build_skill)[gtid] = 0; }
+      if (!P.has_gather) R_F64(c, o_bonus_gather_prob)[gtid] = 0;
     }
     if (P.has_cda) {
-      for (int q = tid; q < 2 * P.M; q += AIE_NT) { R_I32(c, o_cda_bids)[q] = 0; R_I32(c, o_cda_asks)[q] = 0; }
-      for (int q = tid; q < 2 * n * P.P; q += AIE_NT) {
+      for (int q = gtid; q < 2 * P.M; q += NT) { R_I32(c, o_cda_bids)[q] = 0; R_I32(c, o_cda_asks)[q] = 0; }
+      for (int q = gtid; q < 2 * n * P.P; q += NT) {
         R_U8(c, o_cda_bid_hist)[q] = 0; R_U8(c, o_cda_ask_hist)[q] = 0;
         R_F64(c, o_cda_price_history)[q] = 0;
       }
-      for (int q = tid; q < 2 * n; q += AIE_NT) R_I32(c, o_cda_n_orders)[q] = 0;
-      if (tid < 2) { R_I32(c, o_cda_n_bids)[tid] = 0; R_I32(c, o_cda_n_asks)[tid] = 0; }
-    }
-  }
-  __syncthreads();
-  build_src_list(c, arena);
-  if (P.regen_conv) {
+      for (int q = gtid; q < 2 * n; q += NT) R_I32(c, o_cda_n_orders)[q] = 0;
+      if (gtid < 2) { R_I32(c, o_cda_n_bids)[gtid] = 0; R_I32(c, o_cda_n_asks)[gtid] = 0; }
+    }
+  }
+  RS_SYNC();
+  if (wave == 0) RS_STAMP(2);
+  if (wave == w_side) build_src_list(c, arena);
+  if (P.regen_conv && wave >= regen_w0 && wave < regen_w0 + regen_nw) {
     const uint8_t* cb = reinterpret_cast<const uint8_t*>(R_CELLS(c));
-    for (int q = tid; q < AIE_N_RES * HW; q += AIE_NT) {
+    for (int q = (wave - regen_w0) * AIE_NT + tid; q < AIE_N_RES * HW; q += regen_nw * AIE_NT) {
       const int rs = q >= HW ? 1 : 0, cell = q - rs * HW, r0 = cell / P.W, c0 = cell - r0 * P.W;
       const int hw = P.c.regen_halfwidth[rs];
       const uint32_t bit = rs ? AIE_CELL_WOOD_SRC : AIE_CELL_STONE_SRC;
@@ -3306,104 +3329,22 @@
       R_U8(c, o_regen_count)[q] = (uint8_t)cnt;
     }
   }
-  rebuild_locmap(c);
-  *R_I32(c, o_timestep) = 0;
-  *R_I32(c, o_error_flags) = 0;
-  const int place_perm = P.c.reset_random_order ? rng_permutation(m, tid, n) : tid;
-  for (int k = 0; k < n; ++k) {
-    const int i = bcast(place_perm, k);
-    int r = (int)rng_interval(m, tid, (uint32_t)(P.H - 1)), col = (int)rng_interval(m, tid, (uint32_t)(P.W - 1)), tries = 0;
-    while (!can_agent_occupy(c, r, col, i)) {
-      r = (int)rng_interval(m, tid, (uint32_t)(P.H - 1));
-      col = (int)rng_interval(m, tid, (uint32_t)(P.W - 1));
-      if (++tries > 200) {
-        *R_I32(c, o_error_flags) |= AIE_ERR_RESET_PLACEMENT;
-        break;
-      }
-    }
-    R_I32(c, o_loc_r)[i] = r;
-    R_I32(c, o_loc_c)[i] = col;
-    c.locmap[r * P.W + col] = (uint8_t)(i + 1);
-  }
-  for (int k = 0; k < P.c.n_components; ++k) {
-    switch (P.c.components[k]) {
-      case AIE_COMP_BUILD:
-        for (int i = 0; i < n; ++i) {
-          double skill = 1, pay = 1;
-          const double pm = (double)c.R.c.build_payment_max_skill_multiplier;
-          if (P.c.build_skill_dist == AIE_SKILL_PARETO) {
-            skill = rng_pareto(m, tid, 4.0);
-            pay = (pm - 1) * skill + 1; if (pm < pay) pay = pm;
-          } else if (P.c.build_skill_dist == AIE_SKILL_LOGNORMAL) {
-            skill = rng_lognormal(c, m, -1.0, 0.5);
-            pay = (pm - 1) * skill + 1; if (pm < pay) pay = pm;
-          }
-          R_F64(c, o_build_payment)[i] = pay * (double)c.R.c.build_payment;
-          R_F64(c, o_build_skill)[i] = skill;
-        }
-        break;
-      case AIE_COMP_GATHER:
-        for (int i = 0; i < n; ++i) {
-          double b = 0.0;
-          if (P.c.gather_skill_dist == AIE_SKILL_PARETO) { b = rng_pareto(m, tid, 3.0); b = (b < 2 ? b : 2) / 2; }
-          else if (P.c.gather_skill_dist == AIE_SKILL_LOGNORMAL) { b = rng_lognormal(c, m, -2.022, 0.938); b = (b < 2 ? b : 2) / 2; }
-          R_F64(c, o_bonus_gather_prob)[i] = b;
-        }
-        break;
-      case AIE_COMP_TAX:
-        for (int b = 0; b < P.NB; ++b) R_I32(c, o_tax_rate_idx)[b] = 0;
-        *R_I32(c, o_tax_cycle_pos) = 1;
-        for (int i = 0; i < n; ++i) {
-          R_F64(c, o_tax_last_coin)[i] = R_F64(c, o_inv_coin)[i] + R_F64(c, o_esc_coin)[i];
-          R_F64(c, o_tax_last_income)[i] = 0;
-          R_F64(c, o_tax_last_marginal_rate)[i] = 0;
-        }
-        *R_F64(c, o_tax_total_collected) = 0;
-        if (P.c.tax_model == AIE_TAX_SAEZ) {
-          for (int b = 0; b < P.NB; ++b) R_F64(c, o_tax_saez_obs_rates)[b] = tax_rate(c, b);
-          AIE_WSYNC();
-          for (int b = 0; b < P.NB; ++b)
-            R_F64(c, o_tax_saez_rates)[b] = reinterpret_cast<const double*>(saez_block(c) + AIE_SAEZ_OFF_AVG)[b];
-        }
-        break;
-      default: break;
-    }
-  }
-  if (P.c.fixed_four_skill_and_loc) {
-    for (int i = 0; i < n; ++i) {
-      c.locmap[R_I32(c, o_loc_r)[i] * P.W + R_I32(c, o_loc_c)[i]] = 0;
-      R_I32(c, o_loc_r)[i] = -1;
-      R_I32(c, o_loc_c)[i] = -1;
-    }
-    const int perm = rng_permutation(m, tid, n);
+  if (wave == w_side) RS_STAMP(3);
+  if (wave == w_util) {
+    current_metrics(c);
+    AIE_WSYNC();
+    if (tid <= n) R_F64(c, o_util)[tid] = scr_part(c)[tid];
+    RS_STAMP(6);
+  }
+  if (wave == 0) {
+    *R_I32(c, o_timestep) = 0;
+    *R_I32(c, o_error_flags) = 0;
+    const int place_perm = P.c.reset_random_order ? rng_permutation(m, tid, n) : tid;
     for (int k = 0; k < n; ++k) {
-      const int i = bcast(perm, k);
-      const int r = c.R.c.ranked_locs[k][0], col = c.R.c.ranked_locs[k][1];
-      if (can_agent_occupy(c, r, col, i)) {
-        R_I32(c, o_loc_r)[i] = r;
-        R_I32(c, o_loc_c)[i] = col;
-        c.locmap[r * P.W + col] = (uint8_t)(i + 1);
-      }
-      R_F64(c, o_build_payment)[i] = c.R.c.avg_ranked_skill[k];
-    }
-  }
-  if (P.c.split_water_line > 0) {
-    for (int i = 0; i < n; ++i) {
-      c.locmap[R_I32(c, o_loc_r)[i] * P.W + R_I32(c, o_loc_c)[i]] = 0;
-      R_I32(c, o_loc_r)[i] = -1;
-      R_I32(c, o_loc_c)[i] = -1;
-    }
-    const int perm = rng_permutation(m, tid, n);
-    const int wl = P.c.split_water_line;
-    for (int k = 0; k < n; ++k) {
-      const int i = bcast(perm, k);
-      R_F64(c, o_build_payment)[i] = c.R.c.avg_ranked_skill[k];
-      const bool top = (c.R.c.split_top_ranks[k >> 5] >> (k & 31)) & 1u;
-      const int r_min = top ? 0 : wl + 1, r_max = top ? wl : P.H;
-      int r = r_min + (int)rng_interval(m, tid, (uint32_t)(r_max - r_min - 1));
-      int col = (int)rng_interval(m, tid, (uint32_t)(P.W - 1)), tries = 0;
+      const int i = bcast(place_perm, k);
+      int r = (int)rng_interval(m, tid, (uint32_t)(P.H - 1)), col = (int)rng_interval(m, tid, (uint32_t)(P.W - 1)), tries = 0;
       while (!can_agent_occupy(c, r, col, i)) {
-        r = r_min + (int)rng_interval(m, tid, (uint32_t)(r_max - r_min - 1));
+        r = (int)rng_interval(m, tid, (uint32_t)(P.H - 1));
         col = (int)rng_interval(m, tid, (uint32_t)(P.W - 1));
         if (++tries > 200) {
           *R_I32(c, o_error_flags) |= AIE_ERR_RESET_PLACEMENT;
@@ -3414,45 +3355,199 @@
       R_I32(c, o_loc_c)[i] = col;
       c.locmap[r * P.W + col] = (uint8_t)(i + 1);
     }
-  }
-  *R_I32(c, o_mt_pos) = m.pos;
-  mt_fast_detach(c, m);
+    RS_STAMP(4);
+  }
+  if (maps_early) RS_SYNC();
+  if (maps_early && maps_here) {
+    write_spatial_observations(c, arena, map_part, map_parts);
+    if (wave == w_side) RS_STAMP(8);
+  }
+  if (wave == 0) {
+    for (int k = 0; k < P.c.n_components; ++k) {
+      switch (P.c.components[k]) {
+        case AIE_COMP_BUILD:
+          for (int i = 0; i < n; ++i) {
+            double skill = 1, pay = 1;
+            const double pm = (double)c.R.c.build_payment_max_skill_multiplier;
+            if (P.c.build_skill_dist == AIE_SKILL_PARETO) {
+              skill = rng_pareto(m, tid, 4.0);
+              pay = (pm - 1) * skill + 1; if (pm < pay) pay = pm;
+            } else if (P.c.build_skill_dist == AIE_SKILL_LOGNORMAL) {
+              skill = rng_lognormal(c, m, -1.0, 0.5);
+              pay = (pm - 1) * skill + 1; if (pm < pay) pay = pm;
+            }
+            R_F64(c, o_build_payment)[i] = pay * (double)c.R.c.build_payment;
+            R_F64(c, o_build_skill)[i] = skill;
+          }
+          break;
+        case AIE_COMP_GATHER:
+          for (int i = 0; i < n; ++i) {
+            double b = 0.0;
+            if (P.c.gather_skill_dist == AIE_SKILL_PARETO) { b = rng_pareto(m, tid, 3.0); b = (b < 2 ? b : 2) / 2; }
+            else if (P.c.gather_skill_dist == AIE_SKILL_LOGNORMAL) { b = rng_lognormal(c, m, -2.022, 0.938); b = (b < 2 ? b : 2) / 2; }
+            R_F64(c, o_bonus_gather_prob)[i] = b;
+          }
+          break;
+        case AIE_COMP_TAX:
+          for (int b = 0; b < P.NB; ++b) R_I32(c, o_tax_rate_idx)[b] = 0;
+          *R_I32(c, o_tax_cycle_pos) = 1;
+          for (int i = 0; i < n; ++i) {
+            R_F64(c, o_tax_last_coin)[i] = R_F64(c, o_inv_coin)[i] + R_F64(c, o_esc_coin)[i];
+            R_F64(c, o_tax_last_income)[i] = 0;
+            R_F64(c, o_tax_last_marginal_rate)[i] = 0;
+          }
+          *R_F64(c, o_tax_total_collected) = 0;
+          if (P.c.tax_model == AIE_TAX_SAEZ) {
+            for (int b = 0; b < P.NB; ++b) R_F64(c, o_tax_saez_obs_rates)[b] = tax_rate(c, b);
+            AIE_WSYNC();
+            for (int b = 0; b < P.NB; ++b)
+              R_F64(c, o_tax_saez_rates)[b] = reinterpret_cast<const double*>(saez_block(c) + AIE_SAEZ_OFF_AVG)[b];
+          }
+          break;
+        default: break;
+      }
+    }
+    if (P.c.fixed_four_skill_and_loc) {
+      for (int i = 0; i < n; ++i) {
+        c.locmap[R_I32(c, o_loc_r)[i] * P.W + R_I32(c, o_loc_c)[i]] = 0;
+        R_I32(c, o_loc_r)[i] = -1;
+        R_I32(c, o_loc_c)[i] = -1;
+      }
+      const int perm = rng_permutation(m, tid, n);
+      for (int k = 0; k < n; ++k) {
+        const int i = bcast(perm, k);
+        const int r = c.R.c.ranked_locs[k][0], col = c.R.c.ranked_locs[k][1];
+        if (can_agent_occupy(c, r, col, i)) {
+          R_I32(c, o_loc_r)[i] = r;
+          R_I32(c, o_loc_c)[i] = col;
+          c.locmap[r * P.W + col] = (uint8_t)(i + 1);
+        }
+        R_F64(c, o_build_payment)[i] = c.R.c.avg_ranked_skill[k];
+      }
+    }
+    if (P.c.split_water_line > 0) {
+      for (int i = 0; i < n; ++i) {
+        c.locmap[R_I32(c, o_loc_r)[i] * P.W + R_I32(c, o_loc_c)[i]] = 0;
+        R_I32(c, o_loc_r)[i] = -1;
+        R_I32(c, o_loc_c)[i] = -1;
+      }
+      const int perm = rng_permutation(m, tid, n);
+      const int wl = P.c.split_water_line;
+      for (int k = 0; k < n; ++k) {
+        const int i = bcast(perm, k);
+        R_F64(c, o_build_payment)[i] = c.R.c.avg_ranked_skill[k];
+        const bool top = (c.R.c.split_top_ranks[k >> 5] >> (k & 31)) & 1u;
+        const int r_min = top ? 0 : wl + 1, r_max = top ? wl : P.H;
+        int r = r_min + (int)rng_interval(m, tid, (uint32_t)(r_max - r_min - 1));
+        int col = (int)rng_interval(m, tid, (uint32_t)(P.W - 1)), tries = 0;
+        while (!can_agent_occupy(c, r, col, i)) {
+          r = r_min + (int)rng_interval(m, tid, (uint32_t)(r_max - r_min - 1));
+          col = (int)rng_interval(m, tid, (uint32_t)(P.W - 1));
+          if (++tries > 200) {
+            *R_I32(c, o_error_flags) |= AIE_ERR_RESET_PLACEMENT;
+            break;
+          }
+        }
+        R_I32(c, o_loc_r)[i] = r;
+        R_I32(c, o_loc_c)[i] = col;
+        c.locmap[r * P.W + col] = (uint8_t)(i + 1);
+      }
+    }
+    *R_I32(c, o_mt_pos) = m.pos;
+    mt_fast_detach(c, m);
+    RS_STAMP(5);
+  }
+  RS_SYNC();
+  if (wave == 0) {
+    RS_STAMP(10);
+    write_flat_observations(c, arena);
+    RS_STAMP(9);
+  }
+  if (!maps_early && maps_here) {
+    write_spatial_observations(c, arena, map_part, map_parts);
+    if (wave == w_side) RS_STAMP(8);
+  }
+  if (latch) RS_SYNC();
+  if (wave == 0) {
+    if (tid == 0) *R_I32(c, o_obs_valid) = 1;
+    if (!keep_rewards) {
+      if (tid < n) reinterpret_cast<float*>(arena + R.a_rew_a)[(int64_t)e * n + tid] = 0.0f;
+      if (tid == 0) {
+        reinterpret_cast<float*>(arena + R.a_rew_p)[e] = 0.0f;
+        (arena + R.a_done)[e] = 0;
+      }
+    }
+  }
+  if (wave == w_side) {
+    AIE_WSYNC();
+    if (latch && tid == 0) *R_I32(c, o_tax_last_completions) = *R_I32(c, o_completions);
+    AIE_WSYNC();
+    write_action_masks(c, arena);
+    RS_STAMP(11);
+  }
+  RS_SYNC();
+  store_record(c, arena, m, wave, nwaves, 0);
+  if (wave == 0) RS_STAMP(7);
+}
+
+#define AIE_RESET_GROUP 8
+#define AIE_RESET_OCCUPANCY __attribute__((amdgpu_waves_per_eu(2)))
+#define AIE_RESET_DENSE_LDS_MAX 65536
+template <int SPEC, bool LAYOUT = true>
+__device__ __forceinline__ void reset_group(const aie_params* __restrict__ params, uint8_t* __restrict__ arena,
+                                            const uint8_t* mask, int keep_rewards, uint8_t* lds) {
+  const aie_params& P = aie_spec_params<SPEC>(params);
+  const bool grouped = mask && !(LAYOUT && P.c.layout_gen != AIE_LAYOUT_FIXED);
+  const int E = params->E, group = grouped ? AIE_RESET_GROUP : 1, groups = (E + group - 1) / group;
+  const int e0 = replica_of_block((int)blockIdx.x, groups) * group;
+  const int lane = (int)threadIdx.x & (AIE_NT - 1);
+  const bool in_group = lane < group && e0 + lane < E;
+  const bool set = in_group && (!mask || *const_cast<const volatile uint8_t*>(mask + e0 + lane) != 0);
+  uint32_t todo = (uint32_t)uni((int)(uint32_t)__ballot(set));
   __syncthreads();
-  current_metrics(c);
-  __syncthreads();
-  if (tid <= n) R_F64(c, o_util)[tid] = scr_part(c)[tid];
-  __syncthreads();
-  write_spatial_observations(c, arena);
-  if (tid == 0) *R_I32(c, o_obs_valid) = 1;
-  write_flat_observations(c, arena);
-  AIE_WSYNC();
-  if (P.has_tax && P.c.tax_annealing && tid == 0) *R_I32(c, o_tax_last_completions) = *R_I32(c, o_completions);
-  AIE_WSYNC();
-  write_action_masks(c, arena);
-  if (!keep_rewards) {
-    if (tid < n) reinterpret_cast<float*>(arena + R.a_rew_a)[(int64_t)e * n + tid] = 0.0f;
-    if (tid == 0) {
-      reinterpret_cast<float*>(arena + R.a_rew_p)[e] = 0.0f;
-      (arena + R.a_done)[e] = 0;
-    }
-  }
-  __syncthreads();
-  store_record(c, arena, m);
+  if constexpr (SPEC >= 0 || !LAYOUT) {
+    const size_t image = lds_bytes(P);
+    if (grouped && __popc(todo) >= 2 && image * LG_NW <= AIE_RESET_DENSE_LDS_MAX) {
+      const int wave = (int)threadIdx.x >> 6;
+      for (int at = 0; todo; ++at) {
+        const int k = __builtin_ctz(todo);
+        todo &= todo - 1u;
+        if ((at & (LG_NW - 1)) == wave) reset_body<SPEC, false, 1>(params, arena, keep_rewards, lds + wave * image, e0 + k);
+      }
+      return;
+    }
+  }
+  while (todo) {
+    const int k = __builtin_ctz(todo);
+    todo &= todo - 1u;
+    reset_body<SPEC, LAYOUT>(params, arena, keep_rewards, lds, e0 + k);
+    if (todo) __syncthreads();
+  }
+}
+template <int SPEC>
+__device__ __forceinline__ void reset_all(const aie_params* __restrict__ params, uint8_t* __restrict__ arena, int keep_rewards,
+                                          uint8_t* lds) {
+  if ((int)blockIdx.x < params->E)
+    reset_body<SPEC, false, 1>(params, arena, keep_rewards, lds, replica_of_block((int)blockIdx.x, params->E));
 }
 }
 
 #ifndef AIE_JIT
+extern "C" __global__ void __launch_bounds__(LG_NW * AIE_NT) AIE_RESET_OCCUPANCY
+aie_reset_kernel(const aie_params* __restrict__ params, uint8_t* __restrict__ arena, const uint8_t* mask, int keep_rewards) {
+  extern __shared__ __attribute__((aligned(16))) uint8_t lds[];
+  aie::reset_group<-1, false>(params, arena, mask, keep_rewards, lds);
+}
 extern "C" __global__ void __launch_bounds__(AIE_NT)
-aie_reset_kernel(const aie_params* __restrict__ params, uint8_t* __restrict__ arena,
-                 const uint8_t* __restrict__ mask, int keep_rewards) {
+aie_reset_all_kernel(const aie_params* __restrict__ params, uint8_t* __restrict__ arena, const uint8_t*, int keep_rewards) {
   extern __shared__ __attribute__((aligned(16))) uint8_t lds[];
-  aie::reset_body<-1, false>(params, arena, mask, keep_rewards, lds);
-}
-extern "C" __global__ void __launch_bounds__(LG_NW * AIE_NT)
-aie_reset_kernel_layout(const aie_params* __restrict__ params, uint8_t* __restrict__ arena,
-                        const uint8_t* __restrict__ mask, int keep_rewards) {
+  aie::reset_all<-1>(params, arena, keep_rewards, lds);
+}
+extern "C" __global__ void __launch_bounds__(LG_NW * AIE_NT) AIE_RESET_OCCUPANCY
+aie_reset_kernel_layout(const aie_params* __restrict__ params, uint8_t* __restrict__ arena, const uint8_t* mask,
+                        int keep_rewards) {
   extern __shared__ __attribute__((aligned(16))) uint8_t lds[];
-  aie::reset_body<-1, true>(params, arena, mask, keep_rewards, lds);
+  aie::reset_group<-1, true>(params, arena, mask, keep_rewards, lds);
 }
 extern "C" __global__ void aie_layout_decide_kernel(const aie_params* __restrict__ params, uint8_t* __restrict__ arena, int threshold) {
   int32_t* ctl = reinterpret_cast<int32_t*>(arena + params->a_layout_ctl);
@@ -3494,11 +3589,17 @@
   if (gtid == 0) tags[e] = tag;
 }
 template <int SPEC>
-__global__ void __launch_bounds__(LG_NW * AIE_NT)
-aie_reset_kernel_spec(const aie_params* __restrict__ params, uint8_t* __restrict__ arena,
-                      const uint8_t* __restrict__ mask, int keep_rewards) {
+__global__ void __launch_bounds__(LG_NW * AIE_NT) AIE_RESET_OCCUPANCY
+aie_reset_kernel_spec(const aie_params* __restrict__ params, uint8_t* __restrict__ arena, const uint8_t* mask,
+                      int keep_rewards) {
   extern __shared__ __attribute__((aligned(16))) uint8_t lds[];
-  aie::reset_body<SPEC>(params, arena, mask, keep_rewards, lds);
+  aie::reset_group<SPEC>(params, arena, mask, keep_rewards, lds);
+}
+template <int SPEC>
+__global__ void __launch_bounds__(AIE_NT)
+aie_reset_all_kernel_spec(const aie_params* __restrict__ params, uint8_t* __restrict__ arena, const uint8_t*, int keep_rewards) {
+  extern __shared__ __attribute__((aligned(16))) uint8_t lds[];
+  aie::reset_all<SPEC>(params, arena, keep_rewards, lds);
 }
 
 extern "C" __global__ void aie_seed_kernel(const aie_params P, uint8_t* __restrict__ arena, uint64_t base_seed) {
@@ -4311,10 +4412,9 @@
   extern __shared__ __attribute__((aligned(16))) uint8_t lds[];
   step_body<false, 0>(params, arena, act_a, act_p, lds, next);
 }
-extern "C" __global__ void __launch_bounds__(LG_NW * AIE_NT)
-aie_jit_reset(const aie_params* __restrict__ params, uint8_t* __restrict__ arena,
-              const uint8_t* __restrict__ mask, int keep_rewards) {
+extern "C" __global__ void __launch_bounds__(LG_NW * AIE_NT) AIE_RESET_OCCUPANCY
+aie_jit_reset(const aie_params* __restrict__ params, uint8_t* __restrict__ arena, const uint8_t* mask, int keep_rewards) {
   extern __shared__ __attribute__((aligned(16))) uint8_t lds[];
-  aie::reset_body<0>(params, arena, mask, keep_rewards, lds);
+  aie::reset_group<0>(params, arena, mask, keep_rewards, lds);
 }
 #endif
```

Result: no change. 737.4 million agent-steps/s (median of 6 runs) (+0.4%).
